# zkonduit/ezkl

Hardware: NVIDIA H100
Metric: prove_time_s (lower is better)
Workload: dtype u32 limbs (254-bit Montgomery integers mod BN254 r/p)

## Files before the change

### ezkl_b200/csrc/debug.cu

```cuda
#include "debug.h"
#include "ec_coop.cuh"
#include "msm.cuh"
#include "ntt.cuh"

namespace b200 {
template <class Tag>
HD Fp<Tag> dbg_field(int op, const Fp<Tag>& x, const Fp<Tag>& y) {
    switch (op) {
        case 0: return x + y;
        case 1: return x - y;
        case 2: return x * y;
        case 3: return fp_inv(x);
        case 4: return fp_from_mont(x);
        case 5: return fp_sqr(x);
        case 6: return fp_neg(x);
        case 7: return fp_dbl(x);
        default: return fp_to_mont(x);
    }
}
template <class Tag>
HD Fp<Tag> dbg_field4(int op, const Fp<Tag>& a, const Fp<Tag>& b, const Fp<Tag>& c, const Fp<Tag>& d) {
    return op == 0 ? fp_muladd2(a, b, c, d) : fp_mulsub2(a, b, c, d);
}
HD G1Affine dbg_g1(int op, const G1Affine& p, const G1Affine& q) {
    G1Xyzz r;
    if (op == 0) r = g1_add_mixed(g1_to_xyzz(p), q);
    else if (op == 1) r = g1_dbl(g1_to_xyzz(p));
    else if (op == 2) r = g1_mul_small(g1_to_xyzz(p), q.x.l[0]);
    else if (op == 3) r = g1_add(g1_to_xyzz(p), g1_dbl_affine(q));
    else r = g1_add_mixed(g1_to_xyzz(p), g1_neg(p));
    return g1_to_affine(r);
}
enum { DBG_XYZZ_COOP = 5 };
HD G1Xyzz dbg_xyzz(int op, const G1Xyzz& a, const G1Xyzz& b, uint32_t k) {
    switch (op) {
        case 0: return g1_add(a, b);
        case 1: return g1_dbl(a);
        case 2: { G1Affine q; q.x = b.x; q.y = b.y; return g1_add_mixed(a, q); }
        case 3: return g1_mul_small(a, k);
        default: {
            const G1Affine q = g1_to_affine(a);
            G1Xyzz r = g1_xyzz_identity(); r.x = q.x; r.y = q.y;
            return r;
        }
    }
}

template <class Tag>
__global__ void k_dbg_field(int op, const Fp<Tag>* a, const Fp<Tag>* b, Fp<Tag>* o, size_t n) {
    size_t i = (size_t)blockIdx.x * blockDim.x + threadIdx.x;
    if (i < n) fp_store(o + i, dbg_field(op, fp_load(a + i), fp_load(b + i)));
}
template <class Tag>
__global__ void k_dbg_field4(int op, const Fp<Tag>* a, const Fp<Tag>* b, const Fp<Tag>* c, const Fp<Tag>* d, Fp<Tag>* o, size_t n) {
    size_t i = (size_t)blockIdx.x * blockDim.x + threadIdx.x;
    if (i < n) fp_store(o + i, dbg_field4(op, fp_load(a + i), fp_load(b + i), fp_load(c + i), fp_load(d + i)));
}
__global__ void k_dbg_g1(int op, const G1Affine* a, const G1Affine* b, G1Affine* o, size_t n) {
    size_t i = (size_t)blockIdx.x * blockDim.x + threadIdx.x;
    if (i < n) o[i] = dbg_g1(op, a[i], b[i]);
}
__global__ void k_dbg_xyzz(int op, const G1Xyzz* a, const G1Xyzz* b, const uint32_t* k, G1Xyzz* o, size_t n) {
    const size_t t = (size_t)blockIdx.x * blockDim.x + threadIdx.x;
    if (op >= DBG_XYZZ_COOP) {
        const size_t i = t >> 2;
        if (i >= n) return;
        const G1Xyzz r = op == DBG_XYZZ_COOP ? g1_add_coop4(a[i], b[i]) : g1_dbl_coop4(a[i]);
        if ((t & 3) == 0) o[i] = r;
        return;
    }
    if (t < n) o[t] = dbg_xyzz(op, a[t], b[t], k[t]);
}
__global__ void k_dbg_xyzz_to_affine(const G1Xyzz* p, G1Affine* o, size_t n) {
    size_t i = (size_t)blockIdx.x * blockDim.x + threadIdx.x;
    if (i < n) o[i] = g1_to_affine(p[i]);
}
template <class Tag> static void host_field_op(int op, const b200_fr* a, const b200_fr* b, b200_fr* out, size_t n) {
    for (size_t i = 0; i < n; ++i) {
        Fp<Tag> x, y; memcpy(&x, &a[i], 32); memcpy(&y, &b[i], 32);
        const Fp<Tag> r = dbg_field(op, x, y); memcpy(&out[i], &r, 32);
    }
}
template <class Tag> static void host_field_op4(int op, const b200_fr* a, const b200_fr* b, const b200_fr* c, const b200_fr* d, b200_fr* out, size_t n) {
    for (size_t i = 0; i < n; ++i) {
        Fp<Tag> w, x, y, z; memcpy(&w, &a[i], 32); memcpy(&x, &b[i], 32); memcpy(&y, &c[i], 32); memcpy(&z, &d[i], 32);
        const Fp<Tag> r = dbg_field4(op, w, x, y, z); memcpy(&out[i], &r, 32);
    }
}
struct DbgStage {
    DevBuf bufs[6];
    int used = 0;
    template <class T> int in(const void* src, size_t bytes, T** d) {
        DevBuf& b = bufs[used++];
        if (b.ensure(bytes ? bytes : 1)) return -2;
        B200_CUDA(cudaMemcpy(b.p, src, bytes, cudaMemcpyHostToDevice));
        *d = b.as<T>();
        return 0;
    }
    template <class T> int out(size_t bytes, T** d) {
        DevBuf& b = bufs[used++];
        if (b.ensure(bytes ? bytes : 1)) return -2;
        *d = b.as<T>();
        return 0;
    }
    ~DbgStage() { for (DevBuf& b : bufs) b.release(); }
};
static Config g_dbg_cfg;
const Config& config() { return g_dbg_cfg; }
int sm_count() {
    int dev = 0, v = 0;
    if (cudaGetDevice(&dev) != cudaSuccess || cudaDeviceGetAttribute(&v, cudaDevAttrMultiProcessorCount, dev) != cudaSuccess || v <= 0) return 132;
    return v;
}
bool prof_enabled() { return false; }
void prof_mark(int, cudaStream_t, bool) {}
__global__ void k_dbg_digits(const Fr* s, int c, int W, int32_t* out, size_t n) {
    size_t i = (size_t)blockIdx.x * blockDim.x + threadIdx.x;
    if (i >= n) return;
    Fr v = fp_from_mont(fp_load(s + i));
    uint32_t carry = 0;
    for (int w = 0; w < W; ++w) out[i * W + w] = msm_next_digit(v.l, c, &carry);
}
template <int VARIANT>
__global__ void __launch_bounds__(256) k_bench_mul(Fq* out, int iters) {
    const uint32_t t = blockIdx.x * blockDim.x + threadIdx.x;
    Fq x = fp_one<FqTag>(), y = fp_one<FqTag>();
    x.l[0] ^= t; y.l[1] ^= (t * 2654435761u);
    if (VARIANT == 0) {
#pragma unroll 1
        for (int i = 0; i < iters; ++i) x = x * y;
    } else if (VARIANT == 1) {
        Fq z = y + y;
#pragma unroll 1
        for (int i = 0; i < iters; i += 2) { x = x * y; z = z * y; }
        x = x + z;
    } else if (VARIANT == 2) {
#pragma unroll 1
        for (int i = 0; i < iters; ++i) { Fq r; fp_mul_portable<FqTag>(r.l, x.l, y.l); x = r; }
    } else if (VARIANT == 3) {
        G1Affine g; g.x = x; g.y = y;
        G1Xyzz acc = g1_dbl_affine(g);
#pragma unroll 1
        for (int i = 0; i < iters; ++i) { acc = g1_add_mixed(acc, g); g.x.l[0] += 1; }
        x = acc.x + acc.y + acc.zz + acc.zzz;
    } else {
#pragma unroll 1
        for (int i = 0; i < iters; ++i) { x = x + y; y = y - x; }
    }
    fp_store(out + t, x);
}
template <int V>
__global__ void __launch_bounds__(256) k_bench_pipe(uint64_t* out, int iters) {
    const uint32_t t = blockIdx.x * blockDim.x + threadIdx.x;
    uint32_t a = t * 2654435761u + 12345u, b = t ^ 0x9e3779b9u;
    if (V == 0) {
        uint64_t c0 = t, c1 = t + 1, c2 = t + 2, c3 = t + 3, c4 = t + 4, c5 = t + 5, c6 = t + 6, c7 = t + 7;
#pragma unroll 1
        for (int i = 0; i < iters; ++i) {
            asm volatile("mad.wide.u32 %0, %8, %9, %0;\n\tmad.wide.u32 %1, %8, %9, %1;\n\tmad.wide.u32 %2, %8, %9, %2;\n\tmad.wide.u32 %3, %8, %9, %3;\n\t"
                         "mad.wide.u32 %4, %8, %9, %4;\n\tmad.wide.u32 %5, %8, %9, %5;\n\tmad.wide.u32 %6, %8, %9, %6;\n\tmad.wide.u32 %7, %8, %9, %7;"
                         : "+l"(c0), "+l"(c1), "+l"(c2), "+l"(c3), "+l"(c4), "+l"(c5), "+l"(c6), "+l"(c7) : "r"(a), "r"(b));
        }
        out[t] = c0 ^ c1 ^ c2 ^ c3 ^ c4 ^ c5 ^ c6 ^ c7;
    } else if (V == 1) {
        uint32_t e0 = t, e1 = 1, e2 = 2, e3 = 3, e4 = 4, e5 = 5, e6 = 6, e7 = 7, o0 = 8, o1 = 9, o2 = 10, o3 = 11, o4 = 12, o5 = 13, o6 = 14, o7 = 15;
#pragma unroll 1
        for (int i = 0; i < iters; ++i) {
            asm volatile("mad.lo.cc.u32 %0, %16, %17, %0;\n\tmadc.hi.cc.u32 %1, %16, %17, %1;\n\tmadc.lo.cc.u32 %2, %16, %17, %2;\n\tmadc.hi.cc.u32 %3, %16, %17, %3;\n\t"
                         "madc.lo.cc.u32 %4, %16, %17, %4;\n\tmadc.hi.cc.u32 %5, %16, %17, %5;\n\tmadc.lo.cc.u32 %6, %16, %17, %6;\n\tmadc.hi.u32 %7, %16, %17, %7;\n\t"
                         "mad.lo.cc.u32 %8, %16, %17, %8;\n\tmadc.hi.cc.u32 %9, %16, %17, %9;\n\tmadc.lo.cc.u32 %10, %16, %17, %10;\n\tmadc.hi.cc.u32 %11, %16, %17, %11;\n\t"
                         "madc.lo.cc.u32 %12, %16, %17, %12;\n\tmadc.hi.cc.u32 %13, %16, %17, %13;\n\tmadc.lo.cc.u32 %14, %16, %17, %14;\n\tmadc.hi.u32 %15, %16, %17, %15;"
                         : "+r"(e0), "+r"(e1), "+r"(e2), "+r"(e3), "+r"(e4), "+r"(e5), "+r"(e6), "+r"(e7), "+r"(o0), "+r"(o1), "+r"(o2), "+r"(o3), "+r"(o4), "+r"(o5), "+r"(o6), "+r"(o7)
                         : "r"(a), "r"(b));
        }
        out[t] = (uint64_t)(e0 ^ e1 ^ e2 ^ e3 ^ e4 ^ e5 ^ e6 ^ e7) << 32 | (o0 ^ o1 ^ o2 ^ o3 ^ o4 ^ o5 ^ o6 ^ o7);
    } else if (V == 2) {
        uint32_t c0 = t, c1 = 1, c2 = 2, c3 = 3, c4 = 4, c5 = 5, c6 = 6, c7 = 7;
#pragma unroll 1
        for (int i = 0; i < iters; ++i) {
            asm volatile("mad.lo.u32 %0, %8, %9, %0;\n\tmad.lo.u32 %1, %8, %9, %1;\n\tmad.lo.u32 %2, %8, %9, %2;\n\tmad.lo.u32 %3, %8, %9, %3;\n\t"
                         "mad.lo.u32 %4, %8, %9, %4;\n\tmad.lo.u32 %5, %8, %9, %5;\n\tmad.lo.u32 %6, %8, %9, %6;\n\tmad.lo.u32 %7, %8, %9, %7;"
                         : "+r"(c0), "+r"(c1), "+r"(c2), "+r"(c3), "+r"(c4), "+r"(c5), "+r"(c6), "+r"(c7) : "r"(a), "r"(b));
        }
        out[t] = c0 ^ c1 ^ c2 ^ c3 ^ c4 ^ c5 ^ c6 ^ c7;
    } else {
        double x = (double)a, y = 1.0 + 1e-9 * (double)(b & 1023), c0 = t, c1 = 1, c2 = 2, c3 = 3, c4 = 4, c5 = 5, c6 = 6, c7 = 7;
#pragma unroll 1
        for (int i = 0; i < iters; ++i) {
            c0 = fma(x, y, c0); c1 = fma(x, y, c1); c2 = fma(x, y, c2); c3 = fma(x, y, c3); c4 = fma(x, y, c4); c5 = fma(x, y, c5); c6 = fma(x, y, c6); c7 = fma(x, y, c7);
        }
        out[t] = (uint64_t)(c0 + c1 + c2 + c3 + c4 + c5 + c6 + c7);
    }
}
}
using namespace b200;

#pragma GCC visibility push(default)
extern "C" {
int b200_debug_field_op(int field, int op, const b200_fr* a, const b200_fr* b, b200_fr* out, size_t n) {
    if (n == 0) return 0;
    DbgStage st;
    Fr *da, *db, *dout;
    if (int rc = st.in(a, 32 * n, &da)) return rc;
    if (int rc = st.in(b, 32 * n, &db)) return rc;
    if (int rc = st.out(32 * n, &dout)) return rc;
    if (field == 0) k_dbg_field<FrTag><<<div_up(n, 128), 128>>>(op, da, db, dout, n);
    else k_dbg_field<FqTag><<<div_up(n, 128), 128>>>(op, (const Fq*)da, (const Fq*)db, (Fq*)dout, n);
    B200_CUDA(cudaGetLastError());
    B200_CUDA(cudaMemcpy(out, dout, 32 * n, cudaMemcpyDeviceToHost));
    return 0;
}
int b200_debug_field_op4(int field, int op, const b200_fr* a, const b200_fr* b, const b200_fr* c, const b200_fr* d, b200_fr* out, size_t n) {
    if (n == 0) return 0;
    DbgStage st;
    Fr *da, *db, *dc, *dd, *dout;
    if (int rc = st.in(a, 32 * n, &da)) return rc;
    if (int rc = st.in(b, 32 * n, &db)) return rc;
    if (int rc = st.in(c, 32 * n, &dc)) return rc;
    if (int rc = st.in(d, 32 * n, &dd)) return rc;
    if (int rc = st.out(32 * n, &dout)) return rc;
    if (field == 0) k_dbg_field4<FrTag><<<div_up(n, 128), 128>>>(op, da, db, dc, dd, dout, n);
    else k_dbg_field4<FqTag><<<div_up(n, 128), 128>>>(op, (const Fq*)da, (const Fq*)db, (const Fq*)dc, (const Fq*)dd, (Fq*)dout, n);
    B200_CUDA(cudaGetLastError());
    B200_CUDA(cudaMemcpy(out, dout, 32 * n, cudaMemcpyDeviceToHost));
    return 0;
}
int b200_debug_g1_op(int op, const b200_g1_affine* a, const b200_g1_affine* b, b200_g1_affine* out, size_t n) {
    if (n == 0) return 0;
    DbgStage st;
    G1Affine *da, *db, *dout;
    if (int rc = st.in(a, 64 * n, &da)) return rc;
    if (int rc = st.in(b, 64 * n, &db)) return rc;
    if (int rc = st.out(64 * n, &dout)) return rc;
    k_dbg_g1<<<div_up(n, 64), 64>>>(op, da, db, dout, n);
    B200_CUDA(cudaGetLastError());
    B200_CUDA(cudaMemcpy(out, dout, 64 * n, cudaMemcpyDeviceToHost));
    return 0;
}
int b200_debug_g1_xyzz_op(int op, const b200_g1_xyzz* a, const b200_g1_xyzz* b, const uint32_t* k, b200_g1_xyzz* out, size_t n) {
    if (op < 0 || op > DBG_XYZZ_COOP + 1) return -1;
    if (n == 0) return 0;
    DbgStage st;
    G1Xyzz *da, *db, *dout;
    uint32_t* dk;
    if (int rc = st.in(a, 128 * n, &da)) return rc;
    if (int rc = st.in(b, 128 * n, &db)) return rc;
    if (int rc = st.in(k, 4 * n, &dk)) return rc;
    if (int rc = st.out(128 * n, &dout)) return rc;
    const size_t threads = op >= DBG_XYZZ_COOP ? 4 * n : n;
    k_dbg_xyzz<<<div_up(threads, 64), 64>>>(op, da, db, dk, dout, n);
    B200_CUDA(cudaGetLastError());
    B200_CUDA(cudaMemcpy(out, dout, 128 * n, cudaMemcpyDeviceToHost));
    return 0;
}
int b200_debug_digits(const b200_fr* s, size_t n, int c, int32_t* out ) {
    const int W = (255 + c - 1) / c;
    void *ds, *dout;
    B200_CUDA(cudaMalloc(&ds, 32 * n)); B200_CUDA(cudaMalloc(&dout, 4 * n * W));
    B200_CUDA(cudaMemcpy(ds, s, 32 * n, cudaMemcpyHostToDevice));
    k_dbg_digits<<<div_up(n, 128), 128>>>((const Fr*)ds, c, W, (int32_t*)dout, n);
    B200_CUDA(cudaGetLastError());
    B200_CUDA(cudaMemcpy(out, dout, 4 * n * W, cudaMemcpyDeviceToHost));
    cudaFree(ds); cudaFree(dout);
    return 0;
}
int b200_debug_bench(int variant, int iters, int blocks, int threads, float* ms) {
    Fq* d; B200_CUDA(cudaMalloc(&d, sizeof(Fq) * (size_t)blocks * threads));
    cudaEvent_t e0, e1; cudaEventCreate(&e0); cudaEventCreate(&e1);
    for (int rep = 0; rep < 2; ++rep) {
        cudaEventRecord(e0);
        switch (variant) {
            case 0: k_bench_mul<0><<<blocks, threads>>>(d, iters); break;
            case 1: k_bench_mul<1><<<blocks, threads>>>(d, iters); break;
            case 2: k_bench_mul<2><<<blocks, threads>>>(d, iters); break;
            case 3: k_bench_mul<3><<<blocks, threads>>>(d, iters); break;
            default: k_bench_mul<4><<<blocks, threads>>>(d, iters); break;
        }
        cudaEventRecord(e1);
        B200_CUDA(cudaEventSynchronize(e1));
    }
    B200_CUDA(cudaEventElapsedTime(ms, e0, e1));
    cudaFree(d); cudaEventDestroy(e0); cudaEventDestroy(e1);
    return 0;
}
int b200_debug_bench_pipe(int variant, int iters, int blocks, int threads, float* ms) {
    uint64_t* d; B200_CUDA(cudaMalloc(&d, 8 * (size_t)blocks * threads));
    cudaEvent_t e0, e1; cudaEventCreate(&e0); cudaEventCreate(&e1);
    for (int rep = 0; rep < 2; ++rep) {
        cudaEventRecord(e0);
        switch (variant) {
            case 0: k_bench_pipe<0><<<blocks, threads>>>(d, iters); break;
            case 1: k_bench_pipe<1><<<blocks, threads>>>(d, iters); break;
            case 2: k_bench_pipe<2><<<blocks, threads>>>(d, iters); break;
            default: k_bench_pipe<3><<<blocks, threads>>>(d, iters); break;
        }
        cudaEventRecord(e1);
        B200_CUDA(cudaEventSynchronize(e1));
    }
    B200_CUDA(cudaEventElapsedTime(ms, e0, e1));
    cudaFree(d); cudaEventDestroy(e0); cudaEventDestroy(e1);
    return 0;
}
int b200_debug_digits_host(const b200_fr* s_canonical, size_t n, int c, int32_t* out) {
    const int W = (255 + c - 1) / c;
    for (size_t i = 0; i < n; ++i) {
        uint32_t v[8]; memcpy(v, &s_canonical[i], 32);
        uint32_t carry = 0;
        for (int w = 0; w < W; ++w) out[i * W + w] = msm_next_digit(v, c, &carry);
    }
    return 0;
}
int b200_debug_digit_slots_host(const b200_fr* s_canonical, size_t n, int c, int wpl, int32_t* out) {
    const int W = (255 + c - 1) / c;
    for (size_t i = 0; i < n; ++i) {
        uint32_t v[8]; memcpy(v, &s_canonical[i], 32);
        uint32_t carry = 0;
        MsmWindowSlot slot;
        for (int w = 0; w < W; ++w) {
            const int32_t d = msm_next_digit(v, c, &carry);
            int32_t* o = out + ((size_t)i * W + w) * 4;
            o[0] = (int32_t)slot.level; o[1] = slot.r;
            o[2] = d ? (int32_t)(slot.set_off + (uint32_t)(d < 0 ? -d : d) - 1u) : -1;
            o[3] = d < 0 ? -1 : (d > 0 ? 1 : 0);
            slot.next(c, wpl);
        }
    }
    return 0;
}
int b200_debug_msm_pick_levels(size_t n, int c, size_t max_table_bytes, int* s, int* L) {
    msm_pick_levels(n, c, max_table_bytes, s, L);
    return 0;
}
int b200_debug_msm_recode_plan(size_t n, int batch, uint32_t nbuckets, int W, int sm_count, uint32_t* out ) {
    const MsmRecodePlan p = msm_pick_recode(n, batch, nbuckets, W, sm_count);
    out[0] = p.tile; out[1] = p.tiles;
    return 0;
}
int b200_debug_msm_base_off(const b200_fr* scalars, size_t n, int batch, const b200_g1_affine* bases, size_t table_n, int c,
                            size_t max_table_bytes, size_t base_off, b200_g1_affine* out) {
    if (n == 0 || batch < 1 || batch > 4096 || base_off + n > table_n || c < 4 || c > 22) return -1;
    MsmTable t;
    MsmWorkspace ws;
    void *d_sc = nullptr, *d_xyzz = nullptr, *d_aff = nullptr;
    auto run = [&]() -> int {
        if (int rc = msm_table_alloc(&t, table_n, c, max_table_bytes ? max_table_bytes : ~(size_t)0)) return rc;
        B200_CUDA(cudaMemcpy(t.d_table, bases, sizeof(G1Affine) * table_n, cudaMemcpyHostToDevice));
        if (int rc = msm_table_build(&t, nullptr, 0)) return rc;
        B200_CUDA(cudaMalloc(&d_sc, sizeof(Fr) * n * batch));
        B200_CUDA(cudaMalloc(&d_xyzz, sizeof(G1Xyzz) * batch));
        B200_CUDA(cudaMalloc(&d_aff, sizeof(G1Affine) * batch));
        B200_CUDA(cudaMemcpy(d_sc, scalars, sizeof(Fr) * n * batch, cudaMemcpyHostToDevice));
        if (int rc = msm_run(t, (const Fr*)d_sc, n, n, batch, (G1Xyzz*)d_xyzz, ws, 0, base_off)) return rc;
        k_dbg_xyzz_to_affine<<<div_up(batch, 32), 32>>>((const G1Xyzz*)d_xyzz, (G1Affine*)d_aff, (size_t)batch);
        B200_CUDA(cudaGetLastError());
        B200_CUDA(cudaMemcpy(out, d_aff, sizeof(G1Affine) * batch, cudaMemcpyDeviceToHost));
        return 0;
    };
    const int rc = run();
    DevBuf* bufs[] = {&ws.counts, &ws.offs, &ws.ents, &ws.subs, &ws.sums, &ws.misc, &ws.tile_counts};
    for (DevBuf* b : bufs) b->release();
    msm_table_free(&t);
    if (d_sc) cudaFree(d_sc);
    if (d_xyzz) cudaFree(d_xyzz);
    if (d_aff) cudaFree(d_aff);
    return rc;
}
int b200_debug_ntt_plan_host(uint32_t log_n, int batch, int sm_count, int64_t* out ) {
    if (log_n < 1 || log_n > 28 || batch < 1 || batch > 65535 || sm_count < 1) return -1;
    int npass, logm[3];
    ntt_choose_passes(log_n, &npass, logm);
    for (int i = 0; i < npass; ++i) {
        const NttPassShape sh = ntt_pass_shape(npass, logm, i);
        const NttPassGeom g = ntt_pass_geometry((uint32_t)logm[i], sh.inner_cnt, sh.lines, batch, sm_count);
        int64_t* o = out + 7 * i;
        o[0] = g.kernel; o[1] = logm[i]; o[2] = g.log_g; o[3] = g.threads; o[4] = (int64_t)g.smem; o[5] = (int64_t)g.grid_x;
        o[6] = i == npass - 1 ? 0 : (g.kernel == 2 && ntt_full_table(log_n, npass) ? 1 : 2);
    }
    return npass;
}
int b200_debug_host_g1_op(int op, const b200_g1_affine* a, const b200_g1_affine* b, b200_g1_affine* out, size_t n) {
    for (size_t i = 0; i < n; ++i) {
        G1Affine p, q; memcpy(&p, &a[i], 64); memcpy(&q, &b[i], 64);
        const G1Affine o = dbg_g1(op, p, q); memcpy(&out[i], &o, 64);
    }
    return 0;
}
int b200_debug_host_g1_xyzz_op(int op, const b200_g1_xyzz* a, const b200_g1_xyzz* b, const uint32_t* k, b200_g1_xyzz* out, size_t n) {
    if (op < 0 || op >= DBG_XYZZ_COOP) return -1;
    for (size_t i = 0; i < n; ++i) {
        G1Xyzz p, q; memcpy(&p, &a[i], 128); memcpy(&q, &b[i], 128);
        const G1Xyzz o = dbg_xyzz(op, p, q, k[i]); memcpy(&out[i], &o, 128);
    }
    return 0;
}
int b200_debug_host_field_op(int field, int op, const b200_fr* a, const b200_fr* b, b200_fr* out, size_t n) {
    if (field == 0) host_field_op<FrTag>(op, a, b, out, n); else host_field_op<FqTag>(op, a, b, out, n);
    return 0;
}
int b200_debug_host_field_op4(int field, int op, const b200_fr* a, const b200_fr* b, const b200_fr* c, const b200_fr* d, b200_fr* out, size_t n) {
    if (field == 0) host_field_op4<FrTag>(op, a, b, c, d, out, n); else host_field_op4<FqTag>(op, a, b, c, d, out, n);
    return 0;
}
}
#pragma GCC visibility pop
```

### ezkl_b200/csrc/ec.cuh

```cuda
#pragma once
#include "field.cuh"

namespace b200 {

struct alignas(16) G1Affine { Fq x, y; };
struct alignas(16) G1Xyzz { Fq x, y, zz, zzz; };
struct alignas(16) G1Jac { Fq x, y, z; };

HD bool g1_is_identity(const G1Affine& p) { return fp_is_zero(p.x) && fp_is_zero(p.y); }
HD bool g1_is_identity(const G1Xyzz& p) { return fp_is_zero(p.zz); }
HD G1Xyzz g1_xyzz_identity() {
    G1Xyzz r; r.x = fp_zero<FqTag>(); r.y = fp_zero<FqTag>(); r.zz = fp_zero<FqTag>(); r.zzz = fp_zero<FqTag>();
    return r;
}
HD G1Xyzz g1_to_xyzz(const G1Affine& p) {
    G1Xyzz r;
    if (g1_is_identity(p)) return g1_xyzz_identity();
    r.x = p.x; r.y = p.y; r.zz = fp_one<FqTag>(); r.zzz = fp_one<FqTag>();
    return r;
}
HD G1Affine g1_neg(const G1Affine& p) {
    G1Affine r; r.x = p.x; r.y = fp_neg(p.y);
    return r;
}
HD G1Xyzz g1_dbl_affine(const G1Affine& p) {
    if (g1_is_identity(p)) return g1_xyzz_identity();
    G1Xyzz r;
    Fq u = fp_dbl(p.y), v = fp_sqr(u), w = u * v, s = p.x * v;
    Fq xx = fp_sqr(p.x), m = fp_dbl(xx) + xx;
    r.x = fp_sqr(m) - fp_dbl(s);
    r.y = fp_mulsub2(m, s - r.x, w, p.y);
    r.zz = v; r.zzz = w;
    return r;
}
HD G1Xyzz g1_dbl(const G1Xyzz& p) {
    if (g1_is_identity(p)) return p;
    G1Xyzz r;
    Fq u = fp_dbl(p.y), v = fp_sqr(u), w = u * v, s = p.x * v;
    Fq xx = fp_sqr(p.x), m = fp_dbl(xx) + xx;
    r.x = fp_sqr(m) - fp_dbl(s);
    r.y = fp_mulsub2(m, s - r.x, w, p.y);
    r.zz = v * p.zz; r.zzz = w * p.zzz;
    return r;
}
HD G1Xyzz g1_add_mixed(const G1Xyzz& a, const G1Affine& q) {
    if (g1_is_identity(q)) return a;
    if (g1_is_identity(a)) return g1_to_xyzz(q);
    Fq u2 = q.x * a.zz, s2 = q.y * a.zzz;
    Fq p = u2 - a.x, r = s2 - a.y;
    if (fp_is_zero(p)) {
        if (fp_is_zero(r)) return g1_dbl_affine(q);
        return g1_xyzz_identity();
    }
    G1Xyzz o;
    Fq pp = fp_sqr(p), ppp = p * pp, qq = a.x * pp;
    o.x = fp_sqr(r) - ppp - fp_dbl(qq);
    o.y = fp_mulsub2(r, qq - o.x, a.y, ppp);
    o.zz = a.zz * pp; o.zzz = a.zzz * ppp;
    return o;
}
HD G1Xyzz g1_add(const G1Xyzz& a, const G1Xyzz& b) {
    if (g1_is_identity(a)) return b;
    if (g1_is_identity(b)) return a;
    Fq u1 = a.x * b.zz, u2 = b.x * a.zz, s1 = a.y * b.zzz, s2 = b.y * a.zzz;
    Fq p = u2 - u1, r = s2 - s1;
    if (fp_is_zero(p)) {
        if (fp_is_zero(r)) return g1_dbl(a);
        return g1_xyzz_identity();
    }
    G1Xyzz o;
    Fq pp = fp_sqr(p), ppp = p * pp, qq = u1 * pp;
    o.x = fp_sqr(r) - ppp - fp_dbl(qq);
    o.y = fp_mulsub2(r, qq - o.x, s1, ppp);
    o.zz = a.zz * b.zz * pp; o.zzz = a.zzz * b.zzz * ppp;
    return o;
}
HD G1Affine g1_to_affine(const G1Xyzz& p) {
    G1Affine r;
    if (g1_is_identity(p)) { r.x = fp_zero<FqTag>(); r.y = fp_zero<FqTag>(); return r; }
    Fq zzz_inv = fp_inv(p.zzz);
    Fq zinv = p.zz * zzz_inv;
    Fq zinv2 = fp_sqr(zinv);
    r.x = p.x * zinv2;
    r.y = p.y * (zinv2 * zinv);
    return r;
}
HD G1Jac g1_affine_to_jac(const G1Affine& p) {
    G1Jac r;
    if (g1_is_identity(p)) { r.x = fp_zero<FqTag>(); r.y = fp_one<FqTag>(); r.z = fp_zero<FqTag>(); return r; }
    r.x = p.x; r.y = p.y; r.z = fp_one<FqTag>();
    return r;
}
HD bool g1_is_on_curve(const G1Affine& p) {
    if (g1_is_identity(p)) return true;
    Fq one = fp_one<FqTag>();
    Fq three = one + one + one;
    return fp_eq(fp_sqr(p.y), fp_sqr(p.x) * p.x + three);
}
HD G1Xyzz g1_mul_small(const G1Xyzz& p, uint32_t k) {
    if (k == 0) return g1_xyzz_identity();
    const G1Xyzz p2 = g1_dbl(p), p3 = g1_add(p2, p);
    int top = 30;
    while (top > 0 && !((k >> top) & 3u)) top -= 2;
    uint32_t d = (k >> top) & 3u;
    G1Xyzz acc = d == 1 ? p : (d == 2 ? p2 : p3);
#pragma unroll 1
    for (int i = top - 2; i >= 0; i -= 2) {
        acc = g1_dbl(g1_dbl(acc));
        d = (k >> i) & 3u;
        if (d) acc = g1_add(acc, d == 1 ? p : (d == 2 ? p2 : p3));
    }
    return acc;
}

}
```

### ezkl_b200/csrc/field.cuh

```cuda
#pragma once
#include <stdint.h>
#include "fp_ptx.cuh"

#if defined(__CUDACC__)
#define HD __host__ __device__ __forceinline__
#define DEV __device__ __forceinline__
#else
#define HD inline
#define DEV inline
#endif

namespace b200 {

struct FrTag {
    static constexpr uint32_t INV = 0xefffffffu;
    HD static uint32_t mod(int i) {
        constexpr uint32_t M[8] = {0xf0000001u, 0x43e1f593u, 0x79b97091u, 0x2833e848u, 0x8181585du, 0xb85045b6u, 0xe131a029u, 0x30644e72u};
        return M[i];
    }
    HD static uint32_t one(int i) {
        constexpr uint32_t V[8] = {0x4ffffffbu, 0xac96341cu, 0x9f60cd29u, 0x36fc7695u, 0x7879462eu, 0x666ea36fu, 0x9a07df2fu, 0x0e0a77c1u};
        return V[i];
    }
    HD static uint32_t r2(int i) {
        constexpr uint32_t V[8] = {0xae216da7u, 0x1bb8e645u, 0xe35c59e3u, 0x53fe3ab1u, 0x53bb8085u, 0x8c49833du, 0x7f4e44a5u, 0x0216d0b1u};
        return V[i];
    }
};
struct FqTag {
    static constexpr uint32_t INV = 0xe4866389u;
    HD static uint32_t mod(int i) {
        constexpr uint32_t M[8] = {0xd87cfd47u, 0x3c208c16u, 0x6871ca8du, 0x97816a91u, 0x8181585du, 0xb85045b6u, 0xe131a029u, 0x30644e72u};
        return M[i];
    }
    HD static uint32_t one(int i) {
        constexpr uint32_t V[8] = {0xc58f0d9du, 0xd35d438du, 0xf5c70b3du, 0x0a78eb28u, 0x7879462cu, 0x666ea36fu, 0x9a07df2fu, 0x0e0a77c1u};
        return V[i];
    }
    HD static uint32_t r2(int i) {
        constexpr uint32_t V[8] = {0x538afa89u, 0xf32cfc5bu, 0xd44501fbu, 0xb5e71911u, 0x0a417ff6u, 0x47ab1effu, 0xcab8351fu, 0x06d89f71u};
        return V[i];
    }
};

template <class Tag>
struct alignas(16) Fp {
    uint32_t l[8];
};
using Fr = Fp<FrTag>;
using Fq = Fp<FqTag>;

template <class Tag>
HD void fp_mul_portable(uint32_t* r, const uint32_t* a, const uint32_t* b) {
    uint32_t t[10];
#pragma unroll
    for (int i = 0; i < 10; ++i) t[i] = 0;
#pragma unroll
    for (int i = 0; i < 8; ++i) {
        uint64_t c = 0, s;
#pragma unroll
        for (int j = 0; j < 8; ++j) { s = (uint64_t)a[j] * b[i] + t[j] + c; t[j] = (uint32_t)s; c = s >> 32; }
        s = (uint64_t)t[8] + c; t[8] = (uint32_t)s; t[9] = (uint32_t)(s >> 32);
        uint32_t m = t[0] * Tag::INV;
        c = ((uint64_t)m * Tag::mod(0) + t[0]) >> 32;
#pragma unroll
        for (int j = 1; j < 8; ++j) { s = (uint64_t)m * Tag::mod(j) + t[j] + c; t[j - 1] = (uint32_t)s; c = s >> 32; }
        s = (uint64_t)t[8] + c; t[7] = (uint32_t)s; t[8] = t[9] + (uint32_t)(s >> 32);
    }
    uint32_t d[8]; uint64_t br = 0;
#pragma unroll
    for (int j = 0; j < 8; ++j) { uint64_t s = (uint64_t)t[j] - Tag::mod(j) - br; d[j] = (uint32_t)s; br = (s >> 32) & 1; }
    bool ge = (t[8] != 0) || (br == 0);
#pragma unroll
    for (int j = 0; j < 8; ++j) r[j] = ge ? d[j] : t[j];
}
template <class Tag>
HD void fp_add_portable(uint32_t* r, const uint32_t* a, const uint32_t* b) {
    uint32_t t[8], d[8]; uint64_t c = 0, br = 0;
#pragma unroll
    for (int j = 0; j < 8; ++j) { uint64_t s = (uint64_t)a[j] + b[j] + c; t[j] = (uint32_t)s; c = s >> 32; }
#pragma unroll
    for (int j = 0; j < 8; ++j) { uint64_t s = (uint64_t)t[j] - Tag::mod(j) - br; d[j] = (uint32_t)s; br = (s >> 32) & 1; }
    bool ge = (br == 0);
#pragma unroll
    for (int j = 0; j < 8; ++j) r[j] = ge ? d[j] : t[j];
}
template <class Tag>
HD void fp_sub_portable(uint32_t* r, const uint32_t* a, const uint32_t* b) {
    uint32_t t[8]; uint64_t br = 0, c = 0;
#pragma unroll
    for (int j = 0; j < 8; ++j) { uint64_t s = (uint64_t)a[j] - b[j] - br; t[j] = (uint32_t)s; br = (s >> 32) & 1; }
    uint32_t mask = br ? 0xffffffffu : 0u;
#pragma unroll
    for (int j = 0; j < 8; ++j) { uint64_t s = (uint64_t)t[j] + (Tag::mod(j) & mask) + c; r[j] = (uint32_t)s; c = s >> 32; }
}

template <class Tag> struct PtxOps;
#if defined(__CUDA_ARCH__)
template <> struct PtxOps<FrTag> {
    DEV static void mul(uint32_t* r, const uint32_t* a, const uint32_t* b) { fr_mul_ptx(r, a, b); }
    DEV static void add(uint32_t* r, const uint32_t* a, const uint32_t* b) { fr_add_ptx(r, a, b); }
    DEV static void sub(uint32_t* r, const uint32_t* a, const uint32_t* b) { fr_sub_ptx(r, a, b); }
    DEV static void mul2(uint32_t* r, const uint32_t* a, const uint32_t* b, const uint32_t* c, const uint32_t* d) { fr_mul2_ptx(r, a, b, c, d); }
    DEV static void sqr(uint32_t* r, const uint32_t* a) { fr_sqr_ptx(r, a); }
};
template <> struct PtxOps<FqTag> {
    DEV static void mul(uint32_t* r, const uint32_t* a, const uint32_t* b) { fq_mul_ptx(r, a, b); }
    DEV static void add(uint32_t* r, const uint32_t* a, const uint32_t* b) { fq_add_ptx(r, a, b); }
    DEV static void sub(uint32_t* r, const uint32_t* a, const uint32_t* b) { fq_sub_ptx(r, a, b); }
    DEV static void mul2(uint32_t* r, const uint32_t* a, const uint32_t* b, const uint32_t* c, const uint32_t* d) { fq_mul2_ptx(r, a, b, c, d); }
    DEV static void sqr(uint32_t* r, const uint32_t* a) { fq_sqr_ptx(r, a); }
};
#endif

template <class Tag> HD Fp<Tag> operator*(const Fp<Tag>& a, const Fp<Tag>& b) {
    Fp<Tag> r;
#if defined(__CUDA_ARCH__)
    PtxOps<Tag>::mul(r.l, a.l, b.l);
#else
    fp_mul_portable<Tag>(r.l, a.l, b.l);
#endif
    return r;
}
template <class Tag> HD Fp<Tag> operator+(const Fp<Tag>& a, const Fp<Tag>& b) {
    Fp<Tag> r;
#if defined(__CUDA_ARCH__)
    PtxOps<Tag>::add(r.l, a.l, b.l);
#else
    fp_add_portable<Tag>(r.l, a.l, b.l);
#endif
    return r;
}
template <class Tag> HD Fp<Tag> operator-(const Fp<Tag>& a, const Fp<Tag>& b) {
    Fp<Tag> r;
#if defined(__CUDA_ARCH__)
    PtxOps<Tag>::sub(r.l, a.l, b.l);
#else
    fp_sub_portable<Tag>(r.l, a.l, b.l);
#endif
    return r;
}
template <class Tag> HD Fp<Tag> fp_sqr(const Fp<Tag>& a) {
#if defined(__CUDA_ARCH__)
    Fp<Tag> r;
    PtxOps<Tag>::sqr(r.l, a.l);
    return r;
#else
    return a * a;
#endif
}
template <class Tag> HD Fp<Tag> fp_dbl(const Fp<Tag>& a) { return a + a; }
template <class Tag> HD Fp<Tag> fp_zero() {
    Fp<Tag> r;
#pragma unroll
    for (int i = 0; i < 8; ++i) r.l[i] = 0;
    return r;
}
template <class Tag> HD Fp<Tag> fp_one() {
    Fp<Tag> r;
#pragma unroll
    for (int i = 0; i < 8; ++i) r.l[i] = Tag::one(i);
    return r;
}
template <class Tag> HD bool fp_is_zero(const Fp<Tag>& a) {
    uint32_t o = 0;
#pragma unroll
    for (int i = 0; i < 8; ++i) o |= a.l[i];
    return o == 0;
}
template <class Tag> HD bool fp_eq(const Fp<Tag>& a, const Fp<Tag>& b) {
    uint32_t o = 0;
#pragma unroll
    for (int i = 0; i < 8; ++i) o |= a.l[i] ^ b.l[i];
    return o == 0;
}
template <class Tag> HD Fp<Tag> fp_neg(const Fp<Tag>& a) { return fp_zero<Tag>() - a; }
template <class Tag> HD Fp<Tag> fp_muladd2(const Fp<Tag>& a, const Fp<Tag>& b, const Fp<Tag>& c, const Fp<Tag>& d) {
#if defined(__CUDA_ARCH__)
    Fp<Tag> r;
    PtxOps<Tag>::mul2(r.l, a.l, b.l, c.l, d.l);
    return r;
#else
    return a * b + c * d;
#endif
}
template <class Tag> HD Fp<Tag> fp_mulsub2(const Fp<Tag>& a, const Fp<Tag>& b, const Fp<Tag>& c, const Fp<Tag>& d) {
#if defined(__CUDA_ARCH__)
    return fp_muladd2(a, b, fp_neg(c), d);
#else
    return a * b - c * d;
#endif
}
template <class Tag> HD Fp<Tag> fp_from_mont(const Fp<Tag>& a) {
    Fp<Tag> one_c = fp_zero<Tag>(); one_c.l[0] = 1;
    return a * one_c;
}
template <class Tag> HD Fp<Tag> fp_to_mont(const Fp<Tag>& a) {
    Fp<Tag> r2;
#pragma unroll
    for (int i = 0; i < 8; ++i) r2.l[i] = Tag::r2(i);
    return a * r2;
}
template <class Tag> HD Fp<Tag> fp_inv(const Fp<Tag>& a) {
    uint32_t e[8];
    {
        uint64_t br = 2;
        for (int i = 0; i < 8; ++i) { uint64_t s = (uint64_t)Tag::mod(i) - br; e[i] = (uint32_t)s; br = (s >> 32) & 1; }
    }
    Fp<Tag> acc = fp_one<Tag>();
#pragma unroll 1
    for (int i = 253; i >= 0; --i) {
        acc = acc * acc;
        if ((e[i >> 5] >> (i & 31)) & 1) acc = acc * a;
    }
    return acc;
}
template <class Tag> HD Fp<Tag> fp_pow_u64(const Fp<Tag>& a, uint64_t e) {
    Fp<Tag> acc = fp_one<Tag>();
#pragma unroll 1
    for (int i = 63; i >= 0; --i) {
        acc = acc * acc;
        if ((e >> i) & 1) acc = acc * a;
    }
    return acc;
}

#if defined(__CUDACC__)
template <class Tag> DEV Fp<Tag> fp_load(const Fp<Tag>* p) {
    Fp<Tag> r;
    const uint4* q = reinterpret_cast<const uint4*>(p);
    uint4 lo = q[0], hi = q[1];
    r.l[0] = lo.x; r.l[1] = lo.y; r.l[2] = lo.z; r.l[3] = lo.w;
    r.l[4] = hi.x; r.l[5] = hi.y; r.l[6] = hi.z; r.l[7] = hi.w;
    return r;
}
template <class Tag> DEV void fp_store(Fp<Tag>* p, const Fp<Tag>& v) {
    uint4* q = reinterpret_cast<uint4*>(p);
    q[0] = make_uint4(v.l[0], v.l[1], v.l[2], v.l[3]);
    q[1] = make_uint4(v.l[4], v.l[5], v.l[6], v.l[7]);
}
#endif

}
```

### ezkl_b200/csrc/fp_gen.py

```python
#!/usr/bin/env python
import random
import sys

M32 = 0xFFFFFFFF
FIELDS = {
    "fr": 0x30644e72e131a029b85045b68181585d2833e84879b9709143e1f593f0000001,
    "fq": 0x30644e72e131a029b85045b68181585d97816a916871ca8d3c208c16d87cfd47,
}


def limbs(x, n=8):
    return [(x >> (32 * i)) & M32 for i in range(n)]


def gen_mul(mod):
    Ml = limbs(mod)
    inv = (-pow(mod, -1, 1 << 32)) & M32
    ins = []
    X = ["x%d" % i for i in range(8)]
    Y = ["y%d" % i for i in range(8)]
    A = ["a%d" % i for i in range(8)]
    B = ["b%d" % i for i in range(8)]

    def imm(v):
        return "0x%08x" % v

    def reduce_row(E, O):
        ins.append(("mul.lo.u32", "m", E[0], imm(inv)))
        for j in range(4):
            ins.append((("mad.lo.cc.u32" if j == 0 else "madc.lo.cc.u32"), O[2 * j], "m", imm(Ml[2 * j + 1]), O[2 * j]))
            ins.append(("madc.hi.cc.u32", O[2 * j + 1], "m", imm(Ml[2 * j + 1]), O[2 * j + 1]))
        for j in range(4):
            ins.append((("mad.lo.cc.u32" if j == 0 else "madc.lo.cc.u32"), E[2 * j], "m", imm(Ml[2 * j]), E[2 * j]))
            ins.append(("madc.hi.cc.u32", E[2 * j + 1], "m", imm(Ml[2 * j]), E[2 * j + 1]))
        ins.append(("addc.u32", O[7], O[7], "0"))

    for j in range(4):
        ins.append(("mul.lo.u32", X[2 * j], A[2 * j], B[0]))
        ins.append(("mul.hi.u32", X[2 * j + 1], A[2 * j], B[0]))
    for j in range(4):
        ins.append(("mul.lo.u32", Y[2 * j], A[2 * j + 1], B[0]))
        ins.append(("mul.hi.u32", Y[2 * j + 1], A[2 * j + 1], B[0]))
    E, O = X, Y
    reduce_row(E, O)
    for i in range(1, 8):
        nE, nO = O, E
        ins.append(("add.cc.u32", nE[0], nE[0], nO[1]))
        for j in range(4):
            c_lo = nO[2 * j + 2] if 2 * j + 2 < 8 else "0"
            c_hi = nO[2 * j + 3] if 2 * j + 3 < 8 else "0"
            ins.append(("madc.lo.cc.u32", nO[2 * j], A[2 * j + 1], B[i], c_lo))
            ins.append(("madc.hi.cc.u32", nO[2 * j + 1], A[2 * j + 1], B[i], c_hi))
        for j in range(4):
            ins.append((("mad.lo.cc.u32" if j == 0 else "madc.lo.cc.u32"), nE[2 * j], A[2 * j], B[i], nE[2 * j]))
            ins.append(("madc.hi.cc.u32", nE[2 * j + 1], A[2 * j], B[i], nE[2 * j + 1]))
        ins.append(("addc.u32", nO[7], nO[7], "0"))
        E, O = nE, nO
        reduce_row(E, O)
    T = ["t%d" % i for i in range(8)]
    for j in range(7):
        ins.append((("add.cc.u32" if j == 0 else "addc.cc.u32"), T[j], O[j], E[j + 1]))
    ins.append(("addc.u32", T[7], O[7], "0"))
    ins += final_sub(T, Ml)
    return ins


def gen_mul2(mod):
    Ml = limbs(mod)
    inv = (-pow(mod, -1, 1 << 32)) & M32
    ins = []
    X = ["x%d" % i for i in range(8)]
    Y = ["y%d" % i for i in range(8)]
    A = ["a%d" % i for i in range(8)]
    B = ["b%d" % i for i in range(8)]
    Cc = ["c%d" % i for i in range(8)]
    D = ["d%d" % i for i in range(8)]

    def imm(v):
        return "0x%08x" % v

    def acc_rows(E, O, P, q):
        def pair(p):
            return (q, p) if p.startswith("0x") else (p, q)
        for j in range(4):
            ins.append((("mad.lo.cc.u32" if j == 0 else "madc.lo.cc.u32"), O[2 * j]) + pair(P[2 * j + 1]) + (O[2 * j],))
            ins.append(("madc.hi.cc.u32", O[2 * j + 1]) + pair(P[2 * j + 1]) + (O[2 * j + 1],))
        for j in range(4):
            ins.append((("mad.lo.cc.u32" if j == 0 else "madc.lo.cc.u32"), E[2 * j]) + pair(P[2 * j]) + (E[2 * j],))
            ins.append(("madc.hi.cc.u32", E[2 * j + 1]) + pair(P[2 * j]) + (E[2 * j + 1],))
        ins.append(("addc.u32", O[7], O[7], "0"))

    def reduce_row(E, O):
        ins.append(("mul.lo.u32", "m", E[0], imm(inv)))
        acc_rows(E, O, [imm(v) for v in Ml], "m")

    for j in range(4):
        ins.append(("mul.lo.u32", X[2 * j], A[2 * j], B[0]))
        ins.append(("mul.hi.u32", X[2 * j + 1], A[2 * j], B[0]))
    for j in range(4):
        ins.append(("mul.lo.u32", Y[2 * j], A[2 * j + 1], B[0]))
        ins.append(("mul.hi.u32", Y[2 * j + 1], A[2 * j + 1], B[0]))
    E, O = X, Y
    acc_rows(E, O, Cc, D[0])
    reduce_row(E, O)
    for i in range(1, 8):
        nE, nO = O, E
        ins.append(("add.cc.u32", nE[0], nE[0], nO[1]))
        for j in range(4):
            c_lo = nO[2 * j + 2] if 2 * j + 2 < 8 else "0"
            c_hi = nO[2 * j + 3] if 2 * j + 3 < 8 else "0"
            ins.append(("madc.lo.cc.u32", nO[2 * j], A[2 * j + 1], B[i], c_lo))
            ins.append(("madc.hi.cc.u32", nO[2 * j + 1], A[2 * j + 1], B[i], c_hi))
        for j in range(4):
            ins.append((("mad.lo.cc.u32" if j == 0 else "madc.lo.cc.u32"), nE[2 * j], A[2 * j], B[i], nE[2 * j]))
            ins.append(("madc.hi.cc.u32", nE[2 * j + 1], A[2 * j], B[i], nE[2 * j + 1]))
        ins.append(("addc.u32", nO[7], nO[7], "0"))
        E, O = nE, nO
        acc_rows(E, O, Cc, D[i])
        reduce_row(E, O)
    T = ["t%d" % i for i in range(8)]
    for j in range(7):
        ins.append((("add.cc.u32" if j == 0 else "addc.cc.u32"), T[j], O[j], E[j + 1]))
    ins.append(("addc.u32", T[7], O[7], "0"))
    ins += final_sub(T, Ml)
    return ins


def gen_sqr(mod):
    Ml = limbs(mod)
    inv = (-pow(mod, -1, 1 << 32)) & M32
    ins = []
    X = ["x%d" % i for i in range(8)]
    Y = ["y%d" % i for i in range(8)]
    A = ["a%d" % i for i in range(8)]
    U = ["u%d" % i for i in range(8)]
    Wl = ["w%d" % i for i in range(8)]

    def imm(v):
        return "0x%08x" % v

    for j in range(1, 8):
        ins.append(("shl.b32", Wl[j], A[j], "1"))
    for j in range(2, 8):
        ins.append(("shf.l.clamp.b32", U[j], A[j - 1], A[j], "1"))

    def operand(i, j):
        return A[j] if j == i else (Wl[j] if j == i + 1 else U[j])

    def reduce_row(E, O):
        ins.append(("mul.lo.u32", "m", E[0], imm(inv)))
        for j in range(4):
            ins.append((("mad.lo.cc.u32" if j == 0 else "madc.lo.cc.u32"), O[2 * j], "m", imm(Ml[2 * j + 1]), O[2 * j]))
            ins.append(("madc.hi.cc.u32", O[2 * j + 1], "m", imm(Ml[2 * j + 1]), O[2 * j + 1]))
        for j in range(4):
            ins.append((("mad.lo.cc.u32" if j == 0 else "madc.lo.cc.u32"), E[2 * j], "m", imm(Ml[2 * j]), E[2 * j]))
            ins.append(("madc.hi.cc.u32", E[2 * j + 1], "m", imm(Ml[2 * j]), E[2 * j + 1]))
        ins.append(("addc.u32", O[7], O[7], "0"))

    for j in range(4):
        ins.append(("mul.lo.u32", X[2 * j], operand(0, 2 * j), A[0]))
        ins.append(("mul.hi.u32", X[2 * j + 1], operand(0, 2 * j), A[0]))
    for j in range(4):
        ins.append(("mul.lo.u32", Y[2 * j], operand(0, 2 * j + 1), A[0]))
        ins.append(("mul.hi.u32", Y[2 * j + 1], operand(0, 2 * j + 1), A[0]))
    E, O = X, Y
    reduce_row(E, O)
    for i in range(1, 8):
        nE, nO = O, E
        ins.append(("add.cc.u32", nE[0], nE[0], nO[1]))
        for j in range(4):
            c_lo = nO[2 * j + 2] if 2 * j + 2 < 8 else "0"
            c_hi = nO[2 * j + 3] if 2 * j + 3 < 8 else "0"
            if 2 * j + 1 >= i:
                ins.append(("madc.lo.cc.u32", nO[2 * j], operand(i, 2 * j + 1), A[i], c_lo))
                ins.append(("madc.hi.cc.u32", nO[2 * j + 1], operand(i, 2 * j + 1), A[i], c_hi))
            else:
                ins.append(("addc.cc.u32", nO[2 * j], c_lo, "0"))
                ins.append(("addc.cc.u32", nO[2 * j + 1], c_hi, "0"))
        first = True
        for j in range(4):
            if 2 * j < i:
                continue
            ins.append((("mad.lo.cc.u32" if first else "madc.lo.cc.u32"), nE[2 * j], operand(i, 2 * j), A[i], nE[2 * j]))
            ins.append(("madc.hi.cc.u32", nE[2 * j + 1], operand(i, 2 * j), A[i], nE[2 * j + 1]))
            first = False
        if not first:
            ins.append(("addc.u32", nO[7], nO[7], "0"))
        E, O = nE, nO
        reduce_row(E, O)
    T = ["t%d" % i for i in range(8)]
    for j in range(7):
        ins.append((("add.cc.u32" if j == 0 else "addc.cc.u32"), T[j], O[j], E[j + 1]))
    ins.append(("addc.u32", T[7], O[7], "0"))
    ins += final_sub(T, Ml)
    return ins


def final_sub(T, Ml, out=None):
    out = out or ["r%d" % i for i in range(8)]
    ins = []
    S = ["s%d" % i for i in range(8)]
    for j in range(8):
        ins.append((("sub.cc.u32" if j == 0 else "subc.cc.u32"), S[j], T[j], "0x%08x" % Ml[j]))
    ins.append(("subc.u32", "brw", "0", "0"))
    ins.append(("setp.eq.u32", "p", "brw", "0"))
    for j in range(8):
        ins.append(("selp.u32", out[j], S[j], T[j], "p"))
    return ins


def gen_add(mod):
    Ml = limbs(mod)
    ins = []
    T = ["t%d" % i for i in range(8)]
    for j in range(8):
        op = "add.cc.u32" if j == 0 else ("addc.cc.u32" if j < 7 else "addc.u32")
        ins.append((op, T[j], "a%d" % j, "b%d" % j))
    return ins + final_sub(T, Ml)


def gen_sub(mod):
    Ml = limbs(mod)
    ins = []
    T = ["t%d" % i for i in range(8)]
    for j in range(8):
        ins.append((("sub.cc.u32" if j == 0 else "subc.cc.u32"), T[j], "a%d" % j, "b%d" % j))
    ins.append(("subc.u32", "brw", "0", "0"))
    for j in range(8):
        ins.append(("and.b32", "s%d" % j, "brw", "0x%08x" % Ml[j]))
    for j in range(8):
        op = "add.cc.u32" if j == 0 else ("addc.cc.u32" if j < 7 else "addc.u32")
        ins.append((op, "r%d" % j, T[j], "s%d" % j))
    return ins


def run(ins, regs):
    cc = 0
    pred = {}

    def val(x):
        if x in regs:
            return regs[x]
        return int(x, 0)

    for it in ins:
        op, d = it[0], it[1]
        s = [val(x) if x not in pred else x for x in it[2:]]
        if op == "mul.lo.u32":
            regs[d] = (s[0] * s[1]) & M32
        elif op == "mul.hi.u32":
            regs[d] = (s[0] * s[1]) >> 32
        elif op in ("mad.lo.cc.u32", "madc.lo.cc.u32", "madc.hi.cc.u32", "mad.hi.cc.u32"):
            p = s[0] * s[1]
            p = (p & M32) if ".lo" in op else (p >> 32)
            t = p + s[2] + (cc if op.startswith("madc") else 0)
            regs[d], cc = t & M32, t >> 32
        elif op in ("add.cc.u32", "addc.cc.u32", "addc.u32"):
            t = s[0] + s[1] + (cc if op.startswith("addc") else 0)
            regs[d] = t & M32
            if ".cc" in op:
                cc = t >> 32
        elif op in ("sub.cc.u32", "subc.cc.u32", "subc.u32"):
            t = s[0] - s[1] - (cc if op.startswith("subc") else 0)
            regs[d] = t & M32
            if ".cc" in op:
                cc = 1 if t < 0 else 0
        elif op == "and.b32":
            regs[d] = s[0] & s[1]
        elif op == "shl.b32":
            regs[d] = (s[0] << s[1]) & M32
        elif op == "shf.l.clamp.b32":
            regs[d] = ((((s[1] << 32) | s[0]) << min(s[2], 32)) >> 32) & M32
        elif op == "setp.eq.u32":
            pred[d] = (s[0] == s[1])
        elif op == "selp.u32":
            regs[d] = s[0] if pred[it[4]] else s[1]
        else:
            raise ValueError(op)
        assert 0 <= regs.get(d, 0) <= M32
    return regs


def check(name, mod, trials=3000):
    rng = random.Random(hash(name) & 0xFFFF)
    mul, add, sub = gen_mul(mod), gen_add(mod), gen_sub(mod)
    Rinv = pow(1 << 256, -1, mod)
    edge = [0, 1, 2, mod - 1, mod - 2, (1 << 254) % mod, (1 << 253), mod >> 1, 0xFFFFFFFF, (1 << 128) - 1]
    pairs = [(x, y) for x in edge for y in edge] + [(rng.randrange(mod), rng.randrange(mod)) for _ in range(trials)]
    for a, b in pairs:
        regs = {}
        for i, v in enumerate(limbs(a)):
            regs["a%d" % i] = v
        for i, v in enumerate(limbs(b)):
            regs["b%d" % i] = v
        for ins, exp in ((mul, a * b * Rinv % mod), (add, (a + b) % mod), (sub, (a - b) % mod)):
            out = run(ins, dict(regs))
            got = sum(out["r%d" % i] << (32 * i) for i in range(8))
            assert got == exp, (name, hex(a), hex(b), hex(got), hex(exp))
    mul2 = gen_mul2(mod)
    edge2 = [0, 1, mod - 1, mod, (1 << 254) % mod, 0xFFFFFFFF, mod >> 1]
    quads = [(a, b, c, d) for a in edge2 for b in edge2 for c in edge2 for d in edge2]
    quads += [tuple(rng.randrange(mod) for _ in range(4)) for _ in range(trials)]
    for a, b, c, d in quads:
        regs = {}
        for nm, v in (("a", a), ("b", b), ("c", c), ("d", d)):
            for i, w in enumerate(limbs(v)):
                regs["%s%d" % (nm, i)] = w
        out = run(mul2, regs)
        got = sum(out["r%d" % i] << (32 * i) for i in range(8))
        exp = (a * b + c * d) * Rinv % mod
        assert got == exp, (name, "mul2", hex(a), hex(b), hex(c), hex(d), hex(got), hex(exp))
    sqr = gen_sqr(mod)
    for a in edge + [mod, (1 << 254) - 1 if (1 << 254) - 1 < mod else mod - 3, 0x80000000, 0xFFFFFFFF << 32, int("80000000" * 8, 16) % mod,
                     int("ffffffff" * 7, 16)] + [rng.randrange(mod) for _ in range(trials)]:
        regs = {"a%d" % i: v for i, v in enumerate(limbs(a))}
        out = run(sqr, regs)
        got = sum(out["r%d" % i] << (32 * i) for i in range(8))
        assert got == a * a * Rinv % mod, (name, "sqr", hex(a), hex(got))
    return len(mul), len(add), len(sub), len(mul2), len(sqr)


def emit_fn(fname, ins, n_in):
    tmp = sorted({x for it in ins for x in it[1:] if x[0] in "xytsmuw" and not x.startswith("0x")} | {"brw"})
    tmp = [t for t in tmp if t != "p"]
    lines = ["    .reg .u32 %s;" % ", ".join(tmp), "    .reg .pred p;"]

    def opnd(x):
        if x[0] == "r" and x[1:].isdigit():
            return "%%%d" % int(x[1:])
        if x[0] == "a" and x[1:].isdigit():
            return "%%%d" % (8 + int(x[1:]))
        if x[0] == "b" and x[1:].isdigit() and x != "brw":
            return "%%%d" % (16 + int(x[1:]))
        if x[0] == "c" and x[1:].isdigit():
            return "%%%d" % (24 + int(x[1:]))
        if x[0] == "d" and x[1:].isdigit():
            return "%%%d" % (32 + int(x[1:]))
        return x

    for it in ins:
        lines.append("    %s %s;" % (it[0], ", ".join(opnd(x) for x in it[1:])))
    body = "\n".join('        "%s\\n\\t"' % ln.strip() for ln in ["{"] + lines + ["}"])
    outs = ", ".join('"=r"(r[%d])' % i for i in range(8))
    inps = ", ".join('"r"(a[%d])' % i for i in range(8))
    args = "uint32_t* r, const uint32_t* a"
    if n_in >= 2:
        inps += ", " + ", ".join('"r"(b[%d])' % i for i in range(8))
        args += ", const uint32_t* b"
    if n_in == 4:
        inps += ", " + ", ".join('"r"(c[%d])' % i for i in range(8)) + ", " + ", ".join('"r"(d[%d])' % i for i in range(8))
        args += ", const uint32_t* c, const uint32_t* d"
    return ("__device__ __forceinline__ void %s(%s) {\n    asm(\n%s\n        : %s\n        : %s);\n}\n"
            % (fname, args, body, outs, inps))


def main():
    out = ["// GENERATED by fp_gen.py -- do not edit.  Every instruction list below was executed by the generator's",
           "// PTX interpreter against Python bigints (edge + random operands) before this file was written.",
           "#pragma once", "#include <stdint.h>", "#if defined(__CUDA_ARCH__)", ""]
    for name, mod in FIELDS.items():
        n = check(name, mod)
        print("%s: verified; instruction counts mul/add/sub/mul2/sqr = %s" % (name, n))
        out.append(emit_fn("%s_mul_ptx" % name, gen_mul(mod), 2))
        out.append(emit_fn("%s_add_ptx" % name, gen_add(mod), 2))
        out.append(emit_fn("%s_sub_ptx" % name, gen_sub(mod), 2))
        out.append(emit_fn("%s_mul2_ptx" % name, gen_mul2(mod), 4))
        out.append(emit_fn("%s_sqr_ptx" % name, gen_sqr(mod), 1))
    out.append("#endif  // __CUDA_ARCH__")
    if "--check" not in sys.argv:
        import os
        with open(os.path.join(os.path.dirname(os.path.abspath(__file__)), "fp_ptx.cuh"), "w") as f:
            f.write("\n".join(out) + "\n")


if __name__ == "__main__":
    main()
```

### ezkl_b200/csrc/fp_ptx.cuh

```cuda
#pragma once
#include <stdint.h>
#if defined(__CUDA_ARCH__)

__device__ __forceinline__ void fr_mul_ptx(uint32_t* r, const uint32_t* a, const uint32_t* b) {
    asm(
        "{\n\t"
        ".reg .u32 brw, m, s0, s1, s2, s3, s4, s5, s6, s7, t0, t1, t2, t3, t4, t5, t6, t7, x0, x1, x2, x3, x4, x5, x6, x7, y0, y1, y2, y3, y4, y5, y6, y7;\n\t"
        ".reg .pred p;\n\t"
        "mul.lo.u32 x0, %8, %16;\n\t"
        "mul.hi.u32 x1, %8, %16;\n\t"
        "mul.lo.u32 x2, %10, %16;\n\t"
        "mul.hi.u32 x3, %10, %16;\n\t"
        "mul.lo.u32 x4, %12, %16;\n\t"
        "mul.hi.u32 x5, %12, %16;\n\t"
        "mul.lo.u32 x6, %14, %16;\n\t"
        "mul.hi.u32 x7, %14, %16;\n\t"
        "mul.lo.u32 y0, %9, %16;\n\t"
        "mul.hi.u32 y1, %9, %16;\n\t"
        "mul.lo.u32 y2, %11, %16;\n\t"
        "mul.hi.u32 y3, %11, %16;\n\t"
        "mul.lo.u32 y4, %13, %16;\n\t"
        "mul.hi.u32 y5, %13, %16;\n\t"
        "mul.lo.u32 y6, %15, %16;\n\t"
        "mul.hi.u32 y7, %15, %16;\n\t"
// ... 1982 lines not shown

__device__ __forceinline__ void fq_sqr_ptx(uint32_t* r, const uint32_t* a) {
    asm(
        "{\n\t"
        ".reg .u32 brw, m, s0, s1, s2, s3, s4, s5, s6, s7, t0, t1, t2, t3, t4, t5, t6, t7, u2, u3, u4, u5, u6, u7, w1, w2, w3, w4, w5, w6, w7, x0, x1, x2, x3, x4, x5, x6, x7, y0, y1, y2, y3, y4, y5, y6, y7;\n\t"
        ".reg .pred p;\n\t"
        "shl.b32 w1, %9, 1;\n\t"
        "shl.b32 w2, %10, 1;\n\t"
        "shl.b32 w3, %11, 1;\n\t"
        "shl.b32 w4, %12, 1;\n\t"
        "shl.b32 w5, %13, 1;\n\t"
        "shl.b32 w6, %14, 1;\n\t"
        "shl.b32 w7, %15, 1;\n\t"
        "shf.l.clamp.b32 u2, %9, %10, 1;\n\t"
        "shf.l.clamp.b32 u3, %10, %11, 1;\n\t"
        "shf.l.clamp.b32 u4, %11, %12, 1;\n\t"
        "shf.l.clamp.b32 u5, %12, %13, 1;\n\t"
        "shf.l.clamp.b32 u6, %13, %14, 1;\n\t"
        "shf.l.clamp.b32 u7, %14, %15, 1;\n\t"
        "mul.lo.u32 x0, %8, %8;\n\t"
        "mul.hi.u32 x1, %8, %8;\n\t"
        "mul.lo.u32 x2, u2, %8;\n\t"
        "mul.hi.u32 x3, u2, %8;\n\t"
        "mul.lo.u32 x4, u4, %8;\n\t"
        "mul.hi.u32 x5, u4, %8;\n\t"
        "mul.lo.u32 x6, u6, %8;\n\t"
        "mul.hi.u32 x7, u6, %8;\n\t"
        "mul.lo.u32 y0, w1, %8;\n\t"
        "mul.hi.u32 y1, w1, %8;\n\t"
        "mul.lo.u32 y2, u3, %8;\n\t"
        "mul.hi.u32 y3, u3, %8;\n\t"
        "mul.lo.u32 y4, u5, %8;\n\t"
        "mul.hi.u32 y5, u5, %8;\n\t"
        "mul.lo.u32 y6, u7, %8;\n\t"
        "mul.hi.u32 y7, u7, %8;\n\t"
        "mul.lo.u32 m, x0, 0xe4866389;\n\t"
        "mad.lo.cc.u32 y0, m, 0x3c208c16, y0;\n\t"
        "madc.hi.cc.u32 y1, m, 0x3c208c16, y1;\n\t"
        "madc.lo.cc.u32 y2, m, 0x97816a91, y2;\n\t"
        "madc.hi.cc.u32 y3, m, 0x97816a91, y3;\n\t"
        "madc.lo.cc.u32 y4, m, 0xb85045b6, y4;\n\t"
        "madc.hi.cc.u32 y5, m, 0xb85045b6, y5;\n\t"
        "madc.lo.cc.u32 y6, m, 0x30644e72, y6;\n\t"
        "madc.hi.cc.u32 y7, m, 0x30644e72, y7;\n\t"
        "mad.lo.cc.u32 x0, m, 0xd87cfd47, x0;\n\t"
        "madc.hi.cc.u32 x1, m, 0xd87cfd47, x1;\n\t"
        "madc.lo.cc.u32 x2, m, 0x6871ca8d, x2;\n\t"
        "madc.hi.cc.u32 x3, m, 0x6871ca8d, x3;\n\t"
        "madc.lo.cc.u32 x4, m, 0x8181585d, x4;\n\t"
        "madc.hi.cc.u32 x5, m, 0x8181585d, x5;\n\t"
        "madc.lo.cc.u32 x6, m, 0xe131a029, x6;\n\t"
        "madc.hi.cc.u32 x7, m, 0xe131a029, x7;\n\t"
        "addc.u32 y7, y7, 0;\n\t"
        "add.cc.u32 y0, y0, x1;\n\t"
        "madc.lo.cc.u32 x0, %9, %9, x2;\n\t"
        "madc.hi.cc.u32 x1, %9, %9, x3;\n\t"
        "madc.lo.cc.u32 x2, u3, %9, x4;\n\t"
        "madc.hi.cc.u32 x3, u3, %9, x5;\n\t"
        "madc.lo.cc.u32 x4, u5, %9, x6;\n\t"
        "madc.hi.cc.u32 x5, u5, %9, x7;\n\t"
        "madc.lo.cc.u32 x6, u7, %9, 0;\n\t"
        "madc.hi.cc.u32 x7, u7, %9, 0;\n\t"
        "mad.lo.cc.u32 y2, w2, %9, y2;\n\t"
        "madc.hi.cc.u32 y3, w2, %9, y3;\n\t"
        "madc.lo.cc.u32 y4, u4, %9, y4;\n\t"
        "madc.hi.cc.u32 y5, u4, %9, y5;\n\t"
        "madc.lo.cc.u32 y6, u6, %9, y6;\n\t"
        "madc.hi.cc.u32 y7, u6, %9, y7;\n\t"
        "addc.u32 x7, x7, 0;\n\t"
        "mul.lo.u32 m, y0, 0xe4866389;\n\t"
        "mad.lo.cc.u32 x0, m, 0x3c208c16, x0;\n\t"
        "madc.hi.cc.u32 x1, m, 0x3c208c16, x1;\n\t"
        "madc.lo.cc.u32 x2, m, 0x97816a91, x2;\n\t"
        "madc.hi.cc.u32 x3, m, 0x97816a91, x3;\n\t"
        "madc.lo.cc.u32 x4, m, 0xb85045b6, x4;\n\t"
        "madc.hi.cc.u32 x5, m, 0xb85045b6, x5;\n\t"
        "madc.lo.cc.u32 x6, m, 0x30644e72, x6;\n\t"
        "madc.hi.cc.u32 x7, m, 0x30644e72, x7;\n\t"
        "mad.lo.cc.u32 y0, m, 0xd87cfd47, y0;\n\t"
        "madc.hi.cc.u32 y1, m, 0xd87cfd47, y1;\n\t"
        "madc.lo.cc.u32 y2, m, 0x6871ca8d, y2;\n\t"
        "madc.hi.cc.u32 y3, m, 0x6871ca8d, y3;\n\t"
        "madc.lo.cc.u32 y4, m, 0x8181585d, y4;\n\t"
        "madc.hi.cc.u32 y5, m, 0x8181585d, y5;\n\t"
        "madc.lo.cc.u32 y6, m, 0xe131a029, y6;\n\t"
        "madc.hi.cc.u32 y7, m, 0xe131a029, y7;\n\t"
        "addc.u32 x7, x7, 0;\n\t"
        "add.cc.u32 x0, x0, y1;\n\t"
        "addc.cc.u32 y0, y2, 0;\n\t"
        "addc.cc.u32 y1, y3, 0;\n\t"
        "madc.lo.cc.u32 y2, w3, %10, y4;\n\t"
        "madc.hi.cc.u32 y3, w3, %10, y5;\n\t"
        "madc.lo.cc.u32 y4, u5, %10, y6;\n\t"
        "madc.hi.cc.u32 y5, u5, %10, y7;\n\t"
        "madc.lo.cc.u32 y6, u7, %10, 0;\n\t"
        "madc.hi.cc.u32 y7, u7, %10, 0;\n\t"
        "mad.lo.cc.u32 x2, %10, %10, x2;\n\t"
        "madc.hi.cc.u32 x3, %10, %10, x3;\n\t"
        "madc.lo.cc.u32 x4, u4, %10, x4;\n\t"
        "madc.hi.cc.u32 x5, u4, %10, x5;\n\t"
        "madc.lo.cc.u32 x6, u6, %10, x6;\n\t"
        "madc.hi.cc.u32 x7, u6, %10, x7;\n\t"
        "addc.u32 y7, y7, 0;\n\t"
        "mul.lo.u32 m, x0, 0xe4866389;\n\t"
        "mad.lo.cc.u32 y0, m, 0x3c208c16, y0;\n\t"
        "madc.hi.cc.u32 y1, m, 0x3c208c16, y1;\n\t"
        "madc.lo.cc.u32 y2, m, 0x97816a91, y2;\n\t"
        "madc.hi.cc.u32 y3, m, 0x97816a91, y3;\n\t"
        "madc.lo.cc.u32 y4, m, 0xb85045b6, y4;\n\t"
        "madc.hi.cc.u32 y5, m, 0xb85045b6, y5;\n\t"
        "madc.lo.cc.u32 y6, m, 0x30644e72, y6;\n\t"
        "madc.hi.cc.u32 y7, m, 0x30644e72, y7;\n\t"
        "mad.lo.cc.u32 x0, m, 0xd87cfd47, x0;\n\t"
        "madc.hi.cc.u32 x1, m, 0xd87cfd47, x1;\n\t"
        "madc.lo.cc.u32 x2, m, 0x6871ca8d, x2;\n\t"
        "madc.hi.cc.u32 x3, m, 0x6871ca8d, x3;\n\t"
        "madc.lo.cc.u32 x4, m, 0x8181585d, x4;\n\t"
        "madc.hi.cc.u32 x5, m, 0x8181585d, x5;\n\t"
        "madc.lo.cc.u32 x6, m, 0xe131a029, x6;\n\t"
        "madc.hi.cc.u32 x7, m, 0xe131a029, x7;\n\t"
        "addc.u32 y7, y7, 0;\n\t"
        "add.cc.u32 y0, y0, x1;\n\t"
        "addc.cc.u32 x0, x2, 0;\n\t"
        "addc.cc.u32 x1, x3, 0;\n\t"
        "madc.lo.cc.u32 x2, %11, %11, x4;\n\t"
        "madc.hi.cc.u32 x3, %11, %11, x5;\n\t"
        "madc.lo.cc.u32 x4, u5, %11, x6;\n\t"
        "madc.hi.cc.u32 x5, u5, %11, x7;\n\t"
        "madc.lo.cc.u32 x6, u7, %11, 0;\n\t"
        "madc.hi.cc.u32 x7, u7, %11, 0;\n\t"
        "mad.lo.cc.u32 y4, w4, %11, y4;\n\t"
        "madc.hi.cc.u32 y5, w4, %11, y5;\n\t"
        "madc.lo.cc.u32 y6, u6, %11, y6;\n\t"
        "madc.hi.cc.u32 y7, u6, %11, y7;\n\t"
        "addc.u32 x7, x7, 0;\n\t"
        "mul.lo.u32 m, y0, 0xe4866389;\n\t"
        "mad.lo.cc.u32 x0, m, 0x3c208c16, x0;\n\t"
        "madc.hi.cc.u32 x1, m, 0x3c208c16, x1;\n\t"
        "madc.lo.cc.u32 x2, m, 0x97816a91, x2;\n\t"
        "madc.hi.cc.u32 x3, m, 0x97816a91, x3;\n\t"
        "madc.lo.cc.u32 x4, m, 0xb85045b6, x4;\n\t"
        "madc.hi.cc.u32 x5, m, 0xb85045b6, x5;\n\t"
        "madc.lo.cc.u32 x6, m, 0x30644e72, x6;\n\t"
        "madc.hi.cc.u32 x7, m, 0x30644e72, x7;\n\t"
        "mad.lo.cc.u32 y0, m, 0xd87cfd47, y0;\n\t"
        "madc.hi.cc.u32 y1, m, 0xd87cfd47, y1;\n\t"
        "madc.lo.cc.u32 y2, m, 0x6871ca8d, y2;\n\t"
        "madc.hi.cc.u32 y3, m, 0x6871ca8d, y3;\n\t"
        "madc.lo.cc.u32 y4, m, 0x8181585d, y4;\n\t"
        "madc.hi.cc.u32 y5, m, 0x8181585d, y5;\n\t"
        "madc.lo.cc.u32 y6, m, 0xe131a029, y6;\n\t"
        "madc.hi.cc.u32 y7, m, 0xe131a029, y7;\n\t"
        "addc.u32 x7, x7, 0;\n\t"
        "add.cc.u32 x0, x0, y1;\n\t"
        "addc.cc.u32 y0, y2, 0;\n\t"
        "addc.cc.u32 y1, y3, 0;\n\t"
        "addc.cc.u32 y2, y4, 0;\n\t"
        "addc.cc.u32 y3, y5, 0;\n\t"
        "madc.lo.cc.u32 y4, w5, %12, y6;\n\t"
        "madc.hi.cc.u32 y5, w5, %12, y7;\n\t"
        "madc.lo.cc.u32 y6, u7, %12, 0;\n\t"
        "madc.hi.cc.u32 y7, u7, %12, 0;\n\t"
        "mad.lo.cc.u32 x4, %12, %12, x4;\n\t"
        "madc.hi.cc.u32 x5, %12, %12, x5;\n\t"
        "madc.lo.cc.u32 x6, u6, %12, x6;\n\t"
        "madc.hi.cc.u32 x7, u6, %12, x7;\n\t"
        "addc.u32 y7, y7, 0;\n\t"
        "mul.lo.u32 m, x0, 0xe4866389;\n\t"
        "mad.lo.cc.u32 y0, m, 0x3c208c16, y0;\n\t"
        "madc.hi.cc.u32 y1, m, 0x3c208c16, y1;\n\t"
        "madc.lo.cc.u32 y2, m, 0x97816a91, y2;\n\t"
        "madc.hi.cc.u32 y3, m, 0x97816a91, y3;\n\t"
        "madc.lo.cc.u32 y4, m, 0xb85045b6, y4;\n\t"
        "madc.hi.cc.u32 y5, m, 0xb85045b6, y5;\n\t"
        "madc.lo.cc.u32 y6, m, 0x30644e72, y6;\n\t"
        "madc.hi.cc.u32 y7, m, 0x30644e72, y7;\n\t"
        "mad.lo.cc.u32 x0, m, 0xd87cfd47, x0;\n\t"
        "madc.hi.cc.u32 x1, m, 0xd87cfd47, x1;\n\t"
        "madc.lo.cc.u32 x2, m, 0x6871ca8d, x2;\n\t"
        "madc.hi.cc.u32 x3, m, 0x6871ca8d, x3;\n\t"
        "madc.lo.cc.u32 x4, m, 0x8181585d, x4;\n\t"
        "madc.hi.cc.u32 x5, m, 0x8181585d, x5;\n\t"
        "madc.lo.cc.u32 x6, m, 0xe131a029, x6;\n\t"
        "madc.hi.cc.u32 x7, m, 0xe131a029, x7;\n\t"
        "addc.u32 y7, y7, 0;\n\t"
        "add.cc.u32 y0, y0, x1;\n\t"
        "addc.cc.u32 x0, x2, 0;\n\t"
        "addc.cc.u32 x1, x3, 0;\n\t"
        "addc.cc.u32 x2, x4, 0;\n\t"
        "addc.cc.u32 x3, x5, 0;\n\t"
        "madc.lo.cc.u32 x4, %13, %13, x6;\n\t"
        "madc.hi.cc.u32 x5, %13, %13, x7;\n\t"
        "madc.lo.cc.u32 x6, u7, %13, 0;\n\t"
        "madc.hi.cc.u32 x7, u7, %13, 0;\n\t"
        "mad.lo.cc.u32 y6, w6, %13, y6;\n\t"
        "madc.hi.cc.u32 y7, w6, %13, y7;\n\t"
        "addc.u32 x7, x7, 0;\n\t"
        "mul.lo.u32 m, y0, 0xe4866389;\n\t"
        "mad.lo.cc.u32 x0, m, 0x3c208c16, x0;\n\t"
        "madc.hi.cc.u32 x1, m, 0x3c208c16, x1;\n\t"
        "madc.lo.cc.u32 x2, m, 0x97816a91, x2;\n\t"
        "madc.hi.cc.u32 x3, m, 0x97816a91, x3;\n\t"
        "madc.lo.cc.u32 x4, m, 0xb85045b6, x4;\n\t"
        "madc.hi.cc.u32 x5, m, 0xb85045b6, x5;\n\t"
        "madc.lo.cc.u32 x6, m, 0x30644e72, x6;\n\t"
        "madc.hi.cc.u32 x7, m, 0x30644e72, x7;\n\t"
        "mad.lo.cc.u32 y0, m, 0xd87cfd47, y0;\n\t"
        "madc.hi.cc.u32 y1, m, 0xd87cfd47, y1;\n\t"
        "madc.lo.cc.u32 y2, m, 0x6871ca8d, y2;\n\t"
        "madc.hi.cc.u32 y3, m, 0x6871ca8d, y3;\n\t"
        "madc.lo.cc.u32 y4, m, 0x8181585d, y4;\n\t"
        "madc.hi.cc.u32 y5, m, 0x8181585d, y5;\n\t"
        "madc.lo.cc.u32 y6, m, 0xe131a029, y6;\n\t"
        "madc.hi.cc.u32 y7, m, 0xe131a029, y7;\n\t"
        "addc.u32 x7, x7, 0;\n\t"
        "add.cc.u32 x0, x0, y1;\n\t"
        "addc.cc.u32 y0, y2, 0;\n\t"
        "addc.cc.u32 y1, y3, 0;\n\t"
        "addc.cc.u32 y2, y4, 0;\n\t"
        "addc.cc.u32 y3, y5, 0;\n\t"
        "addc.cc.u32 y4, y6, 0;\n\t"
        "addc.cc.u32 y5, y7, 0;\n\t"
        "madc.lo.cc.u32 y6, w7, %14, 0;\n\t"
        "madc.hi.cc.u32 y7, w7, %14, 0;\n\t"
        "mad.lo.cc.u32 x6, %14, %14, x6;\n\t"
        "madc.hi.cc.u32 x7, %14, %14, x7;\n\t"
        "addc.u32 y7, y7, 0;\n\t"
        "mul.lo.u32 m, x0, 0xe4866389;\n\t"
        "mad.lo.cc.u32 y0, m, 0x3c208c16, y0;\n\t"
        "madc.hi.cc.u32 y1, m, 0x3c208c16, y1;\n\t"
        "madc.lo.cc.u32 y2, m, 0x97816a91, y2;\n\t"
        "madc.hi.cc.u32 y3, m, 0x97816a91, y3;\n\t"
        "madc.lo.cc.u32 y4, m, 0xb85045b6, y4;\n\t"
        "madc.hi.cc.u32 y5, m, 0xb85045b6, y5;\n\t"
        "madc.lo.cc.u32 y6, m, 0x30644e72, y6;\n\t"
        "madc.hi.cc.u32 y7, m, 0x30644e72, y7;\n\t"
        "mad.lo.cc.u32 x0, m, 0xd87cfd47, x0;\n\t"
        "madc.hi.cc.u32 x1, m, 0xd87cfd47, x1;\n\t"
        "madc.lo.cc.u32 x2, m, 0x6871ca8d, x2;\n\t"
        "madc.hi.cc.u32 x3, m, 0x6871ca8d, x3;\n\t"
        "madc.lo.cc.u32 x4, m, 0x8181585d, x4;\n\t"
        "madc.hi.cc.u32 x5, m, 0x8181585d, x5;\n\t"
        "madc.lo.cc.u32 x6, m, 0xe131a029, x6;\n\t"
        "madc.hi.cc.u32 x7, m, 0xe131a029, x7;\n\t"
        "addc.u32 y7, y7, 0;\n\t"
        "add.cc.u32 y0, y0, x1;\n\t"
        "addc.cc.u32 x0, x2, 0;\n\t"
        "addc.cc.u32 x1, x3, 0;\n\t"
        "addc.cc.u32 x2, x4, 0;\n\t"
        "addc.cc.u32 x3, x5, 0;\n\t"
        "addc.cc.u32 x4, x6, 0;\n\t"
        "addc.cc.u32 x5, x7, 0;\n\t"
        "madc.lo.cc.u32 x6, %15, %15, 0;\n\t"
        "madc.hi.cc.u32 x7, %15, %15, 0;\n\t"
        "mul.lo.u32 m, y0, 0xe4866389;\n\t"
        "mad.lo.cc.u32 x0, m, 0x3c208c16, x0;\n\t"
        "madc.hi.cc.u32 x1, m, 0x3c208c16, x1;\n\t"
        "madc.lo.cc.u32 x2, m, 0x97816a91, x2;\n\t"
        "madc.hi.cc.u32 x3, m, 0x97816a91, x3;\n\t"
        "madc.lo.cc.u32 x4, m, 0xb85045b6, x4;\n\t"
        "madc.hi.cc.u32 x5, m, 0xb85045b6, x5;\n\t"
        "madc.lo.cc.u32 x6, m, 0x30644e72, x6;\n\t"
        "madc.hi.cc.u32 x7, m, 0x30644e72, x7;\n\t"
        "mad.lo.cc.u32 y0, m, 0xd87cfd47, y0;\n\t"
        "madc.hi.cc.u32 y1, m, 0xd87cfd47, y1;\n\t"
        "madc.lo.cc.u32 y2, m, 0x6871ca8d, y2;\n\t"
        "madc.hi.cc.u32 y3, m, 0x6871ca8d, y3;\n\t"
        "madc.lo.cc.u32 y4, m, 0x8181585d, y4;\n\t"
        "madc.hi.cc.u32 y5, m, 0x8181585d, y5;\n\t"
        "madc.lo.cc.u32 y6, m, 0xe131a029, y6;\n\t"
        "madc.hi.cc.u32 y7, m, 0xe131a029, y7;\n\t"
        "addc.u32 x7, x7, 0;\n\t"
        "add.cc.u32 t0, x0, y1;\n\t"
        "addc.cc.u32 t1, x1, y2;\n\t"
        "addc.cc.u32 t2, x2, y3;\n\t"
        "addc.cc.u32 t3, x3, y4;\n\t"
        "addc.cc.u32 t4, x4, y5;\n\t"
        "addc.cc.u32 t5, x5, y6;\n\t"
        "addc.cc.u32 t6, x6, y7;\n\t"
        "addc.u32 t7, x7, 0;\n\t"
        "sub.cc.u32 s0, t0, 0xd87cfd47;\n\t"
        "subc.cc.u32 s1, t1, 0x3c208c16;\n\t"
        "subc.cc.u32 s2, t2, 0x6871ca8d;\n\t"
        "subc.cc.u32 s3, t3, 0x97816a91;\n\t"
        "subc.cc.u32 s4, t4, 0x8181585d;\n\t"
        "subc.cc.u32 s5, t5, 0xb85045b6;\n\t"
        "subc.cc.u32 s6, t6, 0xe131a029;\n\t"
        "subc.cc.u32 s7, t7, 0x30644e72;\n\t"
        "subc.u32 brw, 0, 0;\n\t"
        "setp.eq.u32 p, brw, 0;\n\t"
        "selp.u32 %0, s0, t0, p;\n\t"
        "selp.u32 %1, s1, t1, p;\n\t"
        "selp.u32 %2, s2, t2, p;\n\t"
        "selp.u32 %3, s3, t3, p;\n\t"
        "selp.u32 %4, s4, t4, p;\n\t"
        "selp.u32 %5, s5, t5, p;\n\t"
        "selp.u32 %6, s6, t6, p;\n\t"
        "selp.u32 %7, s7, t7, p;\n\t"
        "}\n\t"
        : "=r"(r[0]), "=r"(r[1]), "=r"(r[2]), "=r"(r[3]), "=r"(r[4]), "=r"(r[5]), "=r"(r[6]), "=r"(r[7])
        : "r"(a[0]), "r"(a[1]), "r"(a[2]), "r"(a[3]), "r"(a[4]), "r"(a[5]), "r"(a[6]), "r"(a[7]));
}

#endif
```

### ezkl_b200/csrc/msm.cu

```cuda
#include "msm.cuh"
#include "ec_coop.cuh"

namespace b200 {

static constexpr int HEAVY_CHUNKS = 32;
static constexpr int REDUCE_M_MAX = 32;
static constexpr int TREE_THREADS = 256;

int msm_default_window(size_t n) {
    int k = 0;
    while (((size_t)1 << (k + 1)) <= n) ++k;
    int c = k <= 10 ? 8 : (k <= 13 ? k - 2 : (k <= 17 ? k - 1 : (k <= 19 ? 17 : (k <= 21 ? 18 : 20))));
    if (c < 4) c = 4;
    if (c > 22) c = 22;
    return c;
}

__global__ void __launch_bounds__(128) k_table_next_level(const G1Affine* __restrict__ prev, G1Affine* __restrict__ next, size_t n, int c) {
    size_t i = (size_t)blockIdx.x * blockDim.x + threadIdx.x;
    if (i >= n) return;
    G1Affine p = prev[i];
    G1Xyzz a = g1_dbl_affine(p);
#pragma unroll 1
    for (int j = 1; j < c; ++j) a = g1_dbl(a);
    next[i] = g1_to_affine(a);
}

int msm_table_alloc(MsmTable* t, size_t n, int c, size_t max_table_bytes) {
    B200_CHECK(n > 0, -1, "msm_table_build: empty base vector");
    if (c <= 0) c = msm_default_window(n);
    int W = (255 + c - 1) / c, s = 1, L = W;
    msm_pick_levels(n, c, max_table_bytes, &s, &L);
    B200_CHECK((size_t)L * n < ((size_t)1 << 31), -1, "msm_table_build: L*n = %zu exceeds the 31-bit entry index", (size_t)L * n);
    t->n = n; t->c = c; t->W = W; t->s = s; t->L = L;
    B200_CUDA(cudaGetDevice(&t->device));
    const cudaError_t e = cudaMalloc(&t->d_table, t->bytes());
    if (e != cudaSuccess) {
        cudaGetLastError();
        t->d_table = nullptr;
        set_error("msm_table_build: %zu MiB table (%d levels of %zu points): %s", t->bytes() >> 20, L, n, cudaGetErrorString(e));
        return -2;
    }
    return 0;
}

int msm_table_build(MsmTable* t, const G1Affine* d_bases, cudaStream_t st) {
    const size_t n = t->n;
    if (d_bases) B200_CUDA(cudaMemcpyAsync(t->d_table, d_bases, sizeof(G1Affine) * n, cudaMemcpyDeviceToDevice, st));
    for (int j = 1; j < t->L; ++j) {
        k_table_next_level<<<div_up(n, 128), 128, 0, st>>>(t->d_table + (size_t)(j - 1) * n, t->d_table + (size_t)j * n, n, t->c * t->s); count_launch();
    }
    B200_CUDA(cudaGetLastError());
    return 0;
}
void msm_table_free(MsmTable* t) {
    if (t->d_table) cudaFree(t->d_table);
    t->d_table = nullptr;
}

template <bool SCATTER, bool SUBWIN>
__global__ void __launch_bounds__(256) k_digits(const Fr* __restrict__ scalars, size_t stride, uint32_t n, uint32_t table_n, uint32_t base_off, int c, int W,
                                                 uint32_t nbuckets, uint32_t* __restrict__ counters ,
                                                 const uint32_t* __restrict__ offs , uint32_t* __restrict__ ents, size_t ent_stride,
                                                 const uint32_t* __restrict__ skew, int wpl) {
    const uint32_t col = blockIdx.y;
    const bool aggregate = !SCATTER || skew[col] != 0;
    const Fr* sc = scalars + (size_t)col * stride;
    uint32_t* cnt = counters + (size_t)col * nbuckets;
    const uint32_t* off = SCATTER ? offs + (size_t)col * (nbuckets + 1) : nullptr;
    uint32_t* ent = SCATTER ? ents + (size_t)col * ent_stride : nullptr;
    const unsigned lane = threadIdx.x & 31;
    const uint32_t n_up = (n + 31u) & ~31u;
    for (uint32_t i = blockIdx.x * blockDim.x + threadIdx.x; i < n_up; i += gridDim.x * blockDim.x) {
        const bool valid = i < n;
        Fr s = fp_zero<FrTag>();
        if (valid) s = fp_from_mont(fp_load(sc + i));
        uint32_t carry = 0;
        MsmWindowSlot slot;
#pragma unroll 1
        for (int w = 0; w < W; ++w) {
            int32_t d = msm_next_digit(s.l, c, &carry);
            const uint32_t j = SUBWIN ? slot.level : (uint32_t)w;
            const bool nz = d != 0;
            const unsigned act = __ballot_sync(0xffffffffu, nz);
            if (nz && !aggregate) {
                const uint32_t bucket = (SUBWIN ? slot.set_off : 0u) + (uint32_t)(d < 0 ? -d : d) - 1u;
                ent[off[bucket] + atomicAdd(&cnt[bucket], 1u)] = (j * table_n + base_off + i) | (d < 0 ? 0x80000000u : 0u);
            } else if (nz) {
                const uint32_t bucket = (SUBWIN ? slot.set_off : 0u) + (uint32_t)(d < 0 ? -d : d) - 1u;
                const unsigned peers = __match_any_sync(act, bucket);
                const int leader = __ffs(peers) - 1;
                uint32_t base = 0;
                if ((int)lane == leader) base = atomicAdd(&cnt[bucket], (uint32_t)__popc(peers));
                if (SCATTER) {
                    base = __shfl_sync(peers, base, leader);
                    const uint32_t rank = __popc(peers & ((1u << lane) - 1u));
                    ent[off[bucket] + base + rank] = (j * table_n + base_off + i) | (d < 0 ? 0x80000000u : 0u);
                }
            }
            if (SUBWIN) slot.next(c, wpl);
        }
    }
}

template <bool SCATTER, bool SUBWIN>
__global__ void __launch_bounds__(MSM_TILE_THREADS, 1) k_digits_tile(const Fr* __restrict__ scalars, size_t stride, uint32_t n, uint32_t table_n, uint32_t base_off,
                                                                     int c, int W, uint32_t nbuckets, uint32_t tile, uint32_t* __restrict__ tile_counts ,
                                                                     const uint32_t* __restrict__ offs , uint32_t* __restrict__ ents, size_t ent_stride, int wpl) {
    extern __shared__ uint32_t sh_cnt[];
    const uint32_t col = blockIdx.y;
    const Fr* sc = scalars + (size_t)col * stride;
    uint32_t* tc = tile_counts + ((size_t)col * gridDim.x + blockIdx.x) * nbuckets;
    if (SCATTER) {
        const uint32_t* off = offs + (size_t)col * (nbuckets + 1);
        for (uint32_t b = threadIdx.x; b < nbuckets; b += blockDim.x) sh_cnt[b] = off[b] + tc[b];
    } else {
        for (uint32_t b = threadIdx.x; b < nbuckets; b += blockDim.x) sh_cnt[b] = 0;
    }
    __syncthreads();
    uint32_t* ent = SCATTER ? ents + (size_t)col * ent_stride : nullptr;
    const uint32_t lo = blockIdx.x * tile, hi = min(lo + tile, n);
    for (uint32_t i = lo + threadIdx.x; i < hi; i += blockDim.x) {
        Fr s = fp_from_mont(fp_load(sc + i));
        uint32_t carry = 0;
        MsmWindowSlot slot;
#pragma unroll 1
        for (int w = 0; w < W; ++w) {
            const int32_t d = msm_next_digit(s.l, c, &carry);
            if (d != 0) {
                const uint32_t bucket = (SUBWIN ? slot.set_off : 0u) + (uint32_t)(d < 0 ? -d : d) - 1u;
                const uint32_t pos = atomicAdd(&sh_cnt[bucket], 1u);
                if (SCATTER) ent[pos] = ((SUBWIN ? slot.level : (uint32_t)w) * table_n + base_off + i) | (d < 0 ? 0x80000000u : 0u);
            }
            if (SUBWIN) slot.next(c, wpl);
        }
    }
    if (!SCATTER) {
        __syncthreads();
        for (uint32_t b = threadIdx.x; b < nbuckets; b += blockDim.x) tc[b] = sh_cnt[b];
    }
}

__global__ void __launch_bounds__(256) k_tile_prefix(uint32_t* __restrict__ tile_counts, uint32_t tiles, uint32_t nbuckets, uint32_t* __restrict__ hist) {
    const uint32_t col = blockIdx.y;
    const uint32_t b = blockIdx.x * blockDim.x + threadIdx.x;
    if (b >= nbuckets) return;
    uint32_t* tc = tile_counts + (size_t)col * tiles * nbuckets + b;
    uint32_t acc = 0;
    for (uint32_t t0 = 0; t0 < tiles; t0 += 8) {
        uint32_t v[8];
#pragma unroll
        for (int j = 0; j < 8; ++j) v[j] = t0 + j < tiles ? tc[(size_t)(t0 + j) * nbuckets] : 0u;
#pragma unroll
        for (int j = 0; j < 8; ++j) {
            if (t0 + j < tiles) tc[(size_t)(t0 + j) * nbuckets] = acc;
            acc += v[j];
        }
    }
    hist[(size_t)col * nbuckets + b] = acc;
}

__global__ void __launch_bounds__(1024) k_scan_buckets(const uint32_t* __restrict__ counts, uint32_t* __restrict__ offs, uint32_t* __restrict__ chunk_offs,
                                                        uint32_t nbuckets, uint32_t cap, uint32_t* __restrict__ skew ) {
    __shared__ uint32_t sh_max;
    if (threadIdx.x == 0) sh_max = 0;
    __syncthreads();
    const uint32_t col = blockIdx.x;
    const uint32_t lc = 31u - (uint32_t)__clz(cap);
    const uint32_t* cnt = counts + (size_t)col * nbuckets;
    uint32_t* off = offs + (size_t)col * (nbuckets + 1);
    uint32_t* coff = chunk_offs + (size_t)col * (nbuckets + 1);
    const uint32_t ipt = (nbuckets + blockDim.x - 1) / blockDim.x;
    const uint32_t lo = threadIdx.x * ipt, hi = min(lo + ipt, nbuckets);
    uint32_t s = 0, cs = 0;
    uint32_t mx = 0;
    const bool vec = (ipt & 3u) == 0 && lo + ipt <= nbuckets;
    if (vec) {
        const uint4* c4 = reinterpret_cast<const uint4*>(cnt + lo);
#pragma unroll 4
        for (uint32_t q = 0; q < (ipt >> 2); ++q) {
            const uint4 v = c4[q];
            s += v.x + v.y + v.z + v.w;
            cs += ((v.x + cap - 1) >> lc) + ((v.y + cap - 1) >> lc) + ((v.z + cap - 1) >> lc) + ((v.w + cap - 1) >> lc);
            mx = max(max(mx, v.x), max(max(v.y, v.z), v.w));
        }
    } else {
        for (uint32_t b = lo; b < hi; ++b) { uint32_t v = cnt[b]; s += v; cs += ((v + cap - 1) >> lc); mx = max(mx, v); }
    }
    if (mx) atomicMax(&sh_max, mx);
    uint32_t tot, ctot;
    uint32_t ex = block_exclusive_scan(s, &tot);
    uint32_t cex = block_exclusive_scan(cs, &ctot);
    if (vec) {
        const uint4* c4 = reinterpret_cast<const uint4*>(cnt + lo);
#pragma unroll 4
        for (uint32_t q = 0; q < (ipt >> 2); ++q) {
            const uint4 v = c4[q];
            const uint32_t b = lo + 4 * q;
            off[b] = ex; coff[b] = cex; ex += v.x; cex += ((v.x + cap - 1) >> lc);
            off[b + 1] = ex; coff[b + 1] = cex; ex += v.y; cex += ((v.y + cap - 1) >> lc);
            off[b + 2] = ex; coff[b + 2] = cex; ex += v.z; cex += ((v.z + cap - 1) >> lc);
            off[b + 3] = ex; coff[b + 3] = cex; ex += v.w; cex += ((v.w + cap - 1) >> lc);
        }
    } else {
        for (uint32_t b = lo; b < hi; ++b) { uint32_t v = cnt[b]; off[b] = ex; coff[b] = cex; ex += v; cex += ((v + cap - 1) >> lc); }
    }
    if (threadIdx.x == 0) {
        off[nbuckets] = tot; coff[nbuckets] = ctot;
        skew[col] = sh_max > 16u * (tot / nbuckets + 1u) ? 1u : 0u;
    }
}

__global__ void __launch_bounds__(256) k_fill_chunks(const uint32_t* __restrict__ offs, const uint32_t* __restrict__ chunk_offs, uint32_t nbuckets, uint32_t cap,
                                                      uint32_t* __restrict__ chunk_start, uint32_t* __restrict__ chunk_len, size_t chunk_stride,
                                                      uint32_t* __restrict__ len_hist , uint32_t* __restrict__ heavy , uint32_t heavy_stride) {
    extern __shared__ uint32_t sh_hist[];
    const uint32_t col = blockIdx.y;
    for (uint32_t j = threadIdx.x; j <= cap; j += blockDim.x) sh_hist[j] = 0;
    __syncthreads();
    const uint32_t* off = offs + (size_t)col * (nbuckets + 1);
    const uint32_t* coff = chunk_offs + (size_t)col * (nbuckets + 1);
    uint32_t* cs = chunk_start + (size_t)col * chunk_stride;
    uint32_t* cl = chunk_len + (size_t)col * chunk_stride;
    const uint32_t b = blockIdx.x * blockDim.x + threadIdx.x;
    if (b < nbuckets) {
        const uint32_t start = off[b], size = off[b + 1] - start, c0 = coff[b], nch = coff[b + 1] - c0;
        for (uint32_t j = 0; j < nch; ++j) {
            const uint32_t len = min(cap, size - j * cap);
            cs[c0 + j] = start + j * cap;
            cl[c0 + j] = len;
            if (j + 1 == nch) atomicAdd(&sh_hist[len], 1u);
        }
        if (nch > 1) atomicAdd(&sh_hist[cap], nch - 1);
        if (nch > (uint32_t)HEAVY_CHUNKS) {
            uint32_t* hv = heavy + (size_t)col * heavy_stride;
            uint32_t slot = atomicAdd(&hv[0], 1u);
            if (slot + 1 < heavy_stride) hv[1 + slot] = b;
        }
    }
    __syncthreads();
    uint32_t* gh = len_hist + (size_t)col * (cap + 1);
    for (uint32_t j = threadIdx.x; j <= cap; j += blockDim.x) if (sh_hist[j]) atomicAdd(&gh[j], sh_hist[j]);
}

__global__ void k_len_offsets(const uint32_t* __restrict__ len_hist, uint32_t* __restrict__ len_offs, uint32_t cap) {
    const uint32_t col = blockIdx.x;
    if (threadIdx.x != 0) return;
    const uint32_t* h = len_hist + (size_t)col * (cap + 1);
    uint32_t* o = len_offs + (size_t)col * (cap + 1);
    uint32_t acc = 0;
    for (int l = (int)cap; l >= 0; --l) { o[l] = acc; acc += h[l]; }
}

__global__ void __launch_bounds__(256) k_order_chunks(const uint32_t* __restrict__ chunk_len, size_t chunk_stride, const uint32_t* __restrict__ chunk_offs, uint32_t nbuckets,
                                                       const uint32_t* __restrict__ len_offs, uint32_t* __restrict__ len_cursor, uint32_t cap, uint32_t* __restrict__ order) {
    const uint32_t col = blockIdx.y;
    const uint32_t nchunks = chunk_offs[(size_t)col * (nbuckets + 1) + nbuckets];
    const uint32_t* cl = chunk_len + (size_t)col * chunk_stride;
    uint32_t* ord = order + (size_t)col * chunk_stride;
    const uint32_t* lo = len_offs + (size_t)col * (cap + 1);
    uint32_t* lc = len_cursor + (size_t)col * (cap + 1);
    const unsigned lane = threadIdx.x & 31;
    const uint32_t n_up = (nchunks + 31u) & ~31u;
    for (uint32_t i = blockIdx.x * blockDim.x + threadIdx.x; i < n_up; i += gridDim.x * blockDim.x) {
        const bool valid = i < nchunks;
        const uint32_t len = valid ? cl[i] : 0;
        const unsigned act = __ballot_sync(0xffffffffu, valid);
        if (valid) {
            const unsigned peers = __match_any_sync(act, len);
            const int leader = __ffs(peers) - 1;
            uint32_t base = 0;
            if ((int)lane == leader) base = atomicAdd(&lc[len], (uint32_t)__popc(peers));
            base = __shfl_sync(peers, base, leader);
            ord[lo[len] + base + __popc(peers & ((1u << lane) - 1u))] = i;
        }
    }
}

DEV G1Affine load_base(const G1Affine* __restrict__ table, uint32_t e) {
    const uint4* q = reinterpret_cast<const uint4*>(table + (e & 0x7fffffffu));
    uint4 a = __ldg(q), b = __ldg(q + 1), c = __ldg(q + 2), d = __ldg(q + 3);
    G1Affine p;
    p.x.l[0] = a.x; p.x.l[1] = a.y; p.x.l[2] = a.z; p.x.l[3] = a.w; p.x.l[4] = b.x; p.x.l[5] = b.y; p.x.l[6] = b.z; p.x.l[7] = b.w;
    p.y.l[0] = c.x; p.y.l[1] = c.y; p.y.l[2] = c.z; p.y.l[3] = c.w; p.y.l[4] = d.x; p.y.l[5] = d.y; p.y.l[6] = d.z; p.y.l[7] = d.w;
    return p;
}
__global__ void __launch_bounds__(128, 4) k_accumulate(const G1Affine* __restrict__ table, const uint32_t* __restrict__ ents, size_t ent_stride,
                                                        const uint32_t* __restrict__ chunk_start, const uint32_t* __restrict__ chunk_len, const uint32_t* __restrict__ order,
                                                        size_t chunk_stride, const uint32_t* __restrict__ chunk_offs, uint32_t nbuckets, G1Xyzz* __restrict__ chunk_sums) {
    const uint32_t col = blockIdx.y;
    const uint32_t nchunks = chunk_offs[(size_t)col * (nbuckets + 1) + nbuckets];
    const uint32_t* ent = ents + (size_t)col * ent_stride;
    for (uint32_t t = blockIdx.x * blockDim.x + threadIdx.x; t < nchunks; t += gridDim.x * blockDim.x) {
        const uint32_t ch = order[(size_t)col * chunk_stride + t];
        const uint32_t start = chunk_start[(size_t)col * chunk_stride + ch], len = chunk_len[(size_t)col * chunk_stride + ch];
        uint32_t e = ent[start];
        G1Affine p = load_base(table, e);
        if (e >> 31) p = g1_neg(p);
        G1Xyzz acc = g1_to_xyzz(p);
        if (len > 1) {
            uint32_t e_next = ent[start + 1];
            G1Affine nx = load_base(table, e_next);
#pragma unroll 1
            for (uint32_t j = 1; j < len; ++j) {
                p = nx; e = e_next;
                if (j + 1 < len) { e_next = ent[start + j + 1]; nx = load_base(table, e_next); }
                if (e >> 31) p = g1_neg(p);
                acc = g1_add_mixed(acc, p);
            }
        }
        chunk_sums[(size_t)col * chunk_stride + ch] = acc;
    }
}

DEV G1Xyzz block_sum(G1Xyzz v, G1Xyzz* sh) {
    sh[threadIdx.x] = v;
    __syncthreads();
#pragma unroll 1
    for (unsigned s = blockDim.x / 2; s > 0; s >>= 1) {
        if (threadIdx.x < s) { v = g1_add(v, sh[threadIdx.x + s]); sh[threadIdx.x] = v; }
        __syncthreads();
    }
    return v;
}

__global__ void __launch_bounds__(128) k_combine(const uint32_t* __restrict__ chunk_offs, uint32_t nbuckets, const G1Xyzz* __restrict__ chunk_sums, size_t chunk_stride,
                                                  G1Xyzz* __restrict__ bucket_sums) {
    const uint32_t col = blockIdx.y;
    const uint32_t b = blockIdx.x * blockDim.x + threadIdx.x;
    if (b >= nbuckets) return;
    const uint32_t* coff = chunk_offs + (size_t)col * (nbuckets + 1);
    const uint32_t c0 = coff[b], nch = coff[b + 1] - c0;
    if (nch > (uint32_t)HEAVY_CHUNKS) return;
    const G1Xyzz* cs = chunk_sums + (size_t)col * chunk_stride;
    G1Xyzz acc = g1_xyzz_identity();
    if (nch > 0) acc = cs[c0];
#pragma unroll 1
    for (uint32_t j = 1; j < nch; ++j) acc = g1_add(acc, cs[c0 + j]);
    bucket_sums[(size_t)col * nbuckets + b] = acc;
}
__global__ void __launch_bounds__(TREE_THREADS) k_combine_heavy(const uint32_t* __restrict__ heavy, uint32_t heavy_stride, const uint32_t* __restrict__ chunk_offs, uint32_t nbuckets,
                                                                 const G1Xyzz* __restrict__ chunk_sums, size_t chunk_stride, G1Xyzz* __restrict__ bucket_sums) {
    __shared__ G1Xyzz sh[TREE_THREADS];
    const uint32_t col = blockIdx.y;
    const uint32_t* hv = heavy + (size_t)col * heavy_stride;
    const uint32_t nheavy = min(hv[0], heavy_stride - 1);
    const uint32_t* coff = chunk_offs + (size_t)col * (nbuckets + 1);
    const G1Xyzz* cs = chunk_sums + (size_t)col * chunk_stride;
    for (uint32_t h = blockIdx.x; h < nheavy; h += gridDim.x) {
        const uint32_t b = hv[1 + h];
        const uint32_t c0 = coff[b], nch = coff[b + 1] - c0;
        G1Xyzz acc = g1_xyzz_identity();
#pragma unroll 1
        for (uint32_t j = threadIdx.x; j < nch; j += TREE_THREADS) acc = g1_add(acc, cs[c0 + j]);
        acc = block_sum(acc, sh);
        if (threadIdx.x == 0) bucket_sums[(size_t)col * nbuckets + b] = acc;
        __syncthreads();
    }
}

template <int MIN_CTAS>
__global__ void __launch_bounds__(TREE_THREADS, MIN_CTAS) k_reduce(const G1Xyzz* __restrict__ bucket_sums, uint32_t nbuckets, G1Xyzz* __restrict__ partials, uint32_t nparts, uint32_t per_thread) {
    __shared__ G1Xyzz sh[TREE_THREADS];
    const uint32_t col = blockIdx.y;
    const G1Xyzz* bs = bucket_sums + (size_t)col * nbuckets;
    const uint32_t t = blockIdx.x * blockDim.x + threadIdx.x;
    const uint32_t lo = t * per_thread;
    G1Xyzz run = g1_xyzz_identity(), acc = g1_xyzz_identity();
    if (lo < nbuckets) {
        const uint32_t hi = min(lo + per_thread, nbuckets);
#pragma unroll 1
        for (uint32_t b = hi; b-- > lo;) {
            run = g1_add(run, bs[b]);
            acc = g1_add(acc, run);
        }
        if (lo > 0) acc = g1_add(acc, g1_mul_small(run, lo));
    }
    acc = block_sum(acc, sh);
    if (threadIdx.x == 0) partials[(size_t)col * nparts + blockIdx.x] = acc;
}
__global__ void __launch_bounds__(TREE_THREADS) k_final(const G1Xyzz* __restrict__ partials, uint32_t nparts, G1Xyzz* __restrict__ out) {
    __shared__ G1Xyzz sh[TREE_THREADS];
    const uint32_t col = blockIdx.x;
    G1Xyzz acc = g1_xyzz_identity();
#pragma unroll 1
    for (uint32_t j = threadIdx.x; j < nparts; j += blockDim.x) acc = g1_add(acc, partials[(size_t)col * nparts + j]);
    acc = block_sum(acc, sh);
    if (threadIdx.x == 0) out[col] = acc;
}

static constexpr int COOP_LT = TREE_THREADS / 4;
DEV G1Xyzz block_sum_coop(G1Xyzz v, G1Xyzz* sh) {
    const unsigned lt = threadIdx.x >> 2, q = threadIdx.x & 3;
    if (q == 0) sh[lt] = v;
    __syncthreads();
#pragma unroll 1
    for (unsigned s = COOP_LT / 2; s > 0; s >>= 1) {
        if (lt < s) { v = g1_add_coop4(v, sh[lt + s]); if (q == 0) sh[lt] = v; }
        __syncthreads();
    }
    return v;
}
__global__ void __launch_bounds__(TREE_THREADS) k_final_coop(const G1Xyzz* __restrict__ partials, uint32_t nparts, G1Xyzz* __restrict__ out) {
    __shared__ G1Xyzz sh[COOP_LT];
    const uint32_t col = blockIdx.x;
    G1Xyzz acc = g1_xyzz_identity();
#pragma unroll 1
    for (uint32_t j = threadIdx.x >> 2; j < nparts; j += COOP_LT) acc = g1_add_coop4(acc, partials[(size_t)col * nparts + j]);
    acc = block_sum_coop(acc, sh);
    if (threadIdx.x == 0) out[col] = acc;
}

__global__ void __launch_bounds__(32) k_subwindow_fold(const G1Xyzz* __restrict__ set_sums , int s, int c, uint32_t batch, G1Xyzz* __restrict__ out) {
    const uint32_t col = blockIdx.x * blockDim.x + threadIdx.x;
    if (col >= batch) return;
    const G1Xyzz* rs = set_sums + (size_t)col * s;
    G1Xyzz acc = rs[s - 1];
#pragma unroll 1
    for (int r = s - 2; r >= 0; --r) {
#pragma unroll 1
        for (int k = 0; k < c; ++k) acc = g1_dbl(acc);
        acc = g1_add(acc, rs[r]);
    }
    out[col] = acc;
}

__global__ void __launch_bounds__(128) k_g1_generate(uint64_t seed, size_t n, G1Affine* __restrict__ out) {
    const size_t i = (size_t)blockIdx.x * blockDim.x + threadIdx.x;
    if (i >= n) return;
    uint32_t s[8];
    uint64_t z = seed + 0x9e3779b97f4a7c15ull * (uint64_t)(i + 1);
#pragma unroll
    for (int w = 0; w < 4; ++w) {
        z += 0x9e3779b97f4a7c15ull;
        uint64_t x = z; x = (x ^ (x >> 30)) * 0xbf58476d1ce4e5b9ull; x = (x ^ (x >> 27)) * 0x94d049bb133111ebull; x ^= x >> 31;
        s[2 * w] = (uint32_t)x; s[2 * w + 1] = (uint32_t)(x >> 32);
    }
    s[7] &= 0x0fffffffu;
    G1Affine g; g.x = fp_one<FqTag>(); g.y = fp_one<FqTag>() + fp_one<FqTag>();
    G1Xyzz acc = g1_xyzz_identity();
#pragma unroll 1
    for (int b = 251; b >= 0; --b) {
        acc = g1_dbl(acc);
        if ((s[b >> 5] >> (b & 31)) & 1) acc = g1_add_mixed(acc, g);
    }
    out[i] = g1_to_affine(acc);
}
int g1_generate_run(uint64_t seed, size_t n, G1Affine* d_out, cudaStream_t st) {
    if (n == 0) return 0;
    k_g1_generate<<<div_up(n, 128), 128, 0, st>>>(seed, n, d_out); count_launch();
    B200_CUDA(cudaGetLastError());
    return 0;
}

__global__ void __launch_bounds__(128) k_g1_fixed_base_mul(const Fr* __restrict__ scalars, size_t n, G1Affine base, G1Affine* __restrict__ out) {
    const size_t i = (size_t)blockIdx.x * blockDim.x + threadIdx.x;
    if (i >= n) return;
    const Fr s = fp_from_mont(fp_load(scalars + i));
    G1Xyzz acc = g1_xyzz_identity();
#pragma unroll 1
    for (int b = 253; b >= 0; --b) {
        acc = g1_dbl(acc);
        if ((s.l[b >> 5] >> (b & 31)) & 1) acc = g1_add_mixed(acc, base);
    }
    out[i] = g1_to_affine(acc);
}
int g1_fixed_base_mul_run(const Fr* d_scalars, size_t n, const G1Affine& base, G1Affine* d_out, cudaStream_t st) {
    if (n == 0) return 0;
    k_g1_fixed_base_mul<<<div_up(n, 128), 128, 0, st>>>(d_scalars, n, base, d_out); count_launch();
    B200_CUDA(cudaGetLastError());
    return 0;
}

int g1_sum_run(const G1Xyzz* d_points, size_t groups, size_t count, G1Xyzz* d_out, cudaStream_t st) {
    if (groups == 0) return 0;
    B200_CHECK(groups <= 0x7fffffffu && count <= 0xffffffffu, -1, "g1_sum: sizes out of range");
    k_final_coop<<<(unsigned)groups, TREE_THREADS, 0, st>>>(d_points, (uint32_t)count, d_out); count_launch();
    B200_CUDA(cudaGetLastError());
    return 0;
}

static uint32_t pick_cap(size_t total_entries) {
    size_t target = total_entries / ((size_t)sm_count() * 512 * 4);
    uint32_t cap = 16;
    while (cap < 512 && cap < target) cap <<= 1;
    return cap;
}

size_t msm_workspace_per_column(const MsmTable& t, size_t n) {
    const size_t nb = (size_t)t.s << (t.c - 1), ents = n * t.W;
    const size_t chunk_stride = nb + ents / 16 + 1;
    const size_t tile_counts = nb <= MSM_TILE_MAX_BUCKETS ? (ents + nb) * 4 : 0;
    return ents * 4 + chunk_stride * (12 + sizeof(G1Xyzz)) + nb * (sizeof(G1Xyzz) + 24) + 65536 * (size_t)t.s + tile_counts;
}

int msm_run(const MsmTable& t, const Fr* d_scalars, size_t n, size_t stride, int batch, G1Xyzz* d_out, MsmWorkspace& ws, cudaStream_t st, size_t base_off) {
    B200_CHECK(base_off + n <= t.n, -1, "msm: pairs [%zu, %zu) but only %zu bases registered", base_off, base_off + n, t.n);
    B200_CHECK(batch > 0 && batch <= 65535, -1, "msm: batch %d out of range", batch);
    if (n == 0) {
        B200_CUDA(cudaMemsetAsync(d_out, 0, sizeof(G1Xyzz) * batch, st));
        return 0;
    }
    const int c = t.c, W = t.W, s = t.s;
    B200_CHECK((size_t)batch * s <= 65535, -1, "msm: batch %d x %d bucket sets out of range", batch, s);
    const uint32_t half = 1u << (c - 1), nb = half * (uint32_t)s;
    const int vcols = batch * s;
    const size_t ent_stride = (size_t)n * W;
    B200_CHECK(ent_stride < ((size_t)1 << 32), -1, "msm: n*W too large");
    const Config& cfg = config();
    const uint32_t cap = pick_cap(ent_stride * batch);
    const size_t chunk_stride = (size_t)nb + ent_stride / cap + 1;
    const uint32_t heavy_stride = (uint32_t)(ent_stride / ((size_t)cap * HEAVY_CHUNKS)) + 2;
    const size_t all_buckets = (size_t)batch * nb;
    uint32_t reduce_m = REDUCE_M_MAX, reduce_threads = TREE_THREADS;
    if (all_buckets <= ((size_t)1 << 15)) { reduce_m = 4; reduce_threads = 128; }
    else if (all_buckets <= ((size_t)1 << 18)) { reduce_m = 8; reduce_threads = 128; }
    else if (all_buckets <= ((size_t)5 << 17)) { reduce_m = 16; reduce_threads = 256; }
    else if (all_buckets < ((size_t)37 << 15)) { reduce_m = 32; reduce_threads = 128; }
    while (reduce_m > 1 && reduce_m > half) reduce_m >>= 1;
    if (cfg.msm_reduce_m >= 1 && cfg.msm_reduce_m <= 4096) reduce_m = (uint32_t)cfg.msm_reduce_m;
    if (cfg.msm_reduce_threads == 32 || cfg.msm_reduce_threads == 64 || cfg.msm_reduce_threads == 128 || cfg.msm_reduce_threads == 256) reduce_threads = (uint32_t)cfg.msm_reduce_threads;
    const uint32_t nparts = div_up(div_up(half, reduce_m), reduce_threads);
    uint32_t final_threads = 32;
    while (final_threads < (uint32_t)TREE_THREADS && final_threads < nparts) final_threads <<= 1;

    const unsigned sms = (unsigned)sm_count();
    const MsmRecodePlan rp = msm_pick_recode(n, batch, nb, W, (int)sms);
    const size_t n_hist = (size_t)batch * nb, n_len = (size_t)batch * (cap + 1), n_heavy = (size_t)batch * heavy_stride;
    const size_t counts_words = 2 * n_hist + 2 * n_len + n_heavy;
    if (ws.counts.ensure(counts_words * 4)) return -2;
    uint32_t* hist = ws.counts.as<uint32_t>();
    uint32_t* cursor = hist + n_hist;
    uint32_t* len_hist = cursor + n_hist;
    uint32_t* len_cursor = len_hist + n_len;
    uint32_t* heavy = len_cursor + n_len;
    uint32_t* zero_from = rp.tile ? len_hist : hist;
    const size_t zero_words = counts_words - (size_t)(zero_from - hist);
    uint32_t* tile_counts = nullptr;
    const size_t tile_smem = (size_t)nb * 4;
    auto* count_k = s == 1 ? k_digits_tile<false, false> : k_digits_tile<false, true>;
    auto* place_k = s == 1 ? k_digits_tile<true, false> : k_digits_tile<true, true>;
    if (rp.tile) {
        if (ws.tile_counts.ensure((size_t)batch * rp.tiles * nb * 4)) return -2;
        tile_counts = ws.tile_counts.as<uint32_t>();
        const int smem_limit = (int)(MSM_TILE_MAX_BUCKETS * 4);
        B200_CUDA(cudaFuncSetAttribute(count_k, cudaFuncAttributeMaxDynamicSharedMemorySize, smem_limit));
        B200_CUDA(cudaFuncSetAttribute(place_k, cudaFuncAttributeMaxDynamicSharedMemorySize, smem_limit));
    }
    const size_t n_off = (size_t)batch * (nb + 1);
    if (ws.offs.ensure((2 * n_off + n_len + (size_t)batch) * 4)) return -2;
    uint32_t* offs = ws.offs.as<uint32_t>();
    uint32_t* chunk_offs = offs + n_off;
    uint32_t* len_offs = chunk_offs + n_off;
    uint32_t* skew = len_offs + n_len;
    if (ws.ents.ensure((size_t)batch * ent_stride * 4)) return -2;
    uint32_t* ents = ws.ents.as<uint32_t>();
    if (ws.subs.ensure((size_t)batch * chunk_stride * 4 * 3)) return -2;
    uint32_t* chunk_start = ws.subs.as<uint32_t>();
    uint32_t* chunk_len = chunk_start + (size_t)batch * chunk_stride;
    uint32_t* order = chunk_len + (size_t)batch * chunk_stride;
    const size_t n_set = s > 1 ? (size_t)vcols : 0;
    if (ws.sums.ensure(sizeof(G1Xyzz) * ((size_t)batch * chunk_stride + (size_t)batch * nb + (size_t)vcols * nparts + n_set))) return -2;
    G1Xyzz* chunk_sums = ws.sums.as<G1Xyzz>();
    G1Xyzz* bucket_sums = chunk_sums + (size_t)batch * chunk_stride;
    G1Xyzz* partials = bucket_sums + (size_t)batch * nb;
    G1Xyzz* reduced = s > 1 ? partials + (size_t)vcols * nparts : d_out;

    ProfScope ps_total(PROF_MSM_TOTAL, st);
    B200_CUDA(cudaMemsetAsync(zero_from, 0, zero_words * 4, st));
    if (prof_enabled()) prof_mark(PROF_MSM_RECODE, st, true);
    const unsigned dig_blocks = min(div_up(n, 256), sms * 8u);
    const dim3 gd(dig_blocks, batch), gt(rp.tiles, batch);
    if (rp.tile) {
        count_k<<<gt, MSM_TILE_THREADS, tile_smem, st>>>(d_scalars, stride, (uint32_t)n, (uint32_t)t.n, (uint32_t)base_off, c, W, nb, rp.tile, tile_counts, nullptr, nullptr, 0, s);
        count_launch();
        k_tile_prefix<<<dim3(div_up(nb, 256), batch), 256, 0, st>>>(tile_counts, rp.tiles, nb, hist); count_launch();
    } else {
        if (s == 1) k_digits<false, false><<<gd, 256, 0, st>>>(d_scalars, stride, (uint32_t)n, (uint32_t)t.n, (uint32_t)base_off, c, W, nb, hist, nullptr, nullptr, 0, nullptr, 1);
        else k_digits<false, true><<<gd, 256, 0, st>>>(d_scalars, stride, (uint32_t)n, (uint32_t)t.n, (uint32_t)base_off, c, W, nb, hist, nullptr, nullptr, 0, nullptr, s);
        count_launch();
    }
    {
        ProfScope ps(PROF_MSM_SCAN, st);
        k_scan_buckets<<<batch, 1024, 0, st>>>(hist, offs, chunk_offs, nb, cap, skew); count_launch();
    }
    if (rp.tile) {
        place_k<<<gt, MSM_TILE_THREADS, tile_smem, st>>>(d_scalars, stride, (uint32_t)n, (uint32_t)t.n, (uint32_t)base_off, c, W, nb, rp.tile, tile_counts, offs, ents, ent_stride, s);
    } else if (s == 1) {
        k_digits<true, false><<<gd, 256, 0, st>>>(d_scalars, stride, (uint32_t)n, (uint32_t)t.n, (uint32_t)base_off, c, W, nb, cursor, offs, ents, ent_stride, skew, 1);
    } else {
        k_digits<true, true><<<gd, 256, 0, st>>>(d_scalars, stride, (uint32_t)n, (uint32_t)t.n, (uint32_t)base_off, c, W, nb, cursor, offs, ents, ent_stride, skew, s);
    }
    count_launch();
    k_fill_chunks<<<dim3(div_up(nb, 256), batch), 256, (cap + 1) * 4, st>>>(offs, chunk_offs, nb, cap, chunk_start, chunk_len, chunk_stride, len_hist, heavy, heavy_stride); count_launch();
    k_len_offsets<<<batch, 32, 0, st>>>(len_hist, len_offs, cap); count_launch();
    const unsigned ch_blocks = min(div_up(chunk_stride, 256), sms * 8u);
    k_order_chunks<<<dim3(ch_blocks, batch), 256, 0, st>>>(chunk_len, chunk_stride, chunk_offs, nb, len_offs, len_cursor, cap, order); count_launch();
    if (prof_enabled()) prof_mark(PROF_MSM_RECODE, st, false);
    const unsigned acc_blocks = min(div_up(chunk_stride, 128), sms * 16u);
    {
        ProfScope ps(PROF_MSM_ACCUMULATE, st);
        k_accumulate<<<dim3(acc_blocks, batch), 128, 0, st>>>(t.d_table, ents, ent_stride, chunk_start, chunk_len, order, chunk_stride, chunk_offs, nb, chunk_sums); count_launch();
    }
    ProfScope ps_tail(PROF_MSM_TAIL, st);
    k_combine<<<dim3(div_up(nb, 128), batch), 128, 0, st>>>(chunk_offs, nb, chunk_sums, chunk_stride, bucket_sums); count_launch();
    k_combine_heavy<<<dim3(32, batch), TREE_THREADS, 0, st>>>(heavy, heavy_stride, chunk_offs, nb, chunk_sums, chunk_stride, bucket_sums); count_launch();
    {
        ProfScope ps(PROF_MSM_REDUCE, st);
        k_reduce<1><<<dim3(nparts, vcols), reduce_threads, 0, st>>>(bucket_sums, half, partials, nparts, reduce_m); count_launch();
        k_final<<<vcols, final_threads, 0, st>>>(partials, nparts, reduced); count_launch();
    }
    if (s > 1) {
        ProfScope ps(PROF_MSM_FOLD, st);
        k_subwindow_fold<<<div_up((size_t)batch, 32), 32, 0, st>>>(reduced, s, c, (uint32_t)batch, d_out); count_launch();
    }
    B200_CUDA(cudaGetLastError());
    return 0;
}

}
```

Before: 0.08525.

## Use lazy-reduced Fq arithmetic in MSM bucket accumulation and reduction loops

Adds Fq Montgomery multiply, square, add and subtract variants whose results stay in [0, 2p), dropping the final conditional subtraction, plus a reduce helper and lazy XYZZ point additions. The MSM chunk accumulation loop and the bucket running-sum reduction now use these lazy additions and reduce only when storing the result. The aim is to cut per-operation instruction count in the hot elliptic-curve loops. In exchange, correctness depends on the [0, 2p) bounds holding through mul2 and the zero checks, and the debug and benchmark paths gain new ops for testing this.

```diff
diff --git a/ezkl_b200/csrc/debug.cu b/ezkl_b200/csrc/debug.cu
--- a/ezkl_b200/csrc/debug.cu
+++ b/ezkl_b200/csrc/debug.cu
@@ -4,6 +4,18 @@
 #include "ntt.cuh"
 
 namespace b200 {
+template <class Tag> HD Fp<Tag> dbg_field_lazy(int, const Fp<Tag>& x, const Fp<Tag>&) { return x; }
+HD Fq dbg_field_lazy(int op, const Fq& x, const Fq& y) {
+    switch (op) {
+        case 9: return fq_mul_lazy(x, y);
+        case 10: return fq_sqr_lazy(x);
+        case 11: return fq_add_lazy(x, y);
+        case 12: return fq_sub_lazy(x, y);
+        case 13: return fq_reduce(x);
+        case 14: return fq_mulsub2_lazy(x, y, x, x);
+        default: { Fq r = fp_zero<FqTag>(); r.l[0] = fq_is_zero_lazy(x) ? 1u : 0u; return r; }
+    }
+}
 template <class Tag>
 HD Fp<Tag> dbg_field(int op, const Fp<Tag>& x, const Fp<Tag>& y) {
     switch (op) {
@@ -15,7 +27,8 @@
         case 5: return fp_sqr(x);
         case 6: return fp_neg(x);
         case 7: return fp_dbl(x);
-        default: return fp_to_mont(x);
+        case 8: return fp_to_mont(x);
+        default: return dbg_field_lazy(op, x, y);
     }
 }
 template <class Tag>
@@ -31,13 +44,15 @@
     else r = g1_add_mixed(g1_to_xyzz(p), g1_neg(p));
     return g1_to_affine(r);
 }
-enum { DBG_XYZZ_COOP = 5 };
+enum { DBG_XYZZ_COOP = 5, DBG_XYZZ_LAZY = 7 };
 HD G1Xyzz dbg_xyzz(int op, const G1Xyzz& a, const G1Xyzz& b, uint32_t k) {
     switch (op) {
         case 0: return g1_add(a, b);
         case 1: return g1_dbl(a);
         case 2: { G1Affine q; q.x = b.x; q.y = b.y; return g1_add_mixed(a, q); }
         case 3: return g1_mul_small(a, k);
+        case DBG_XYZZ_LAZY: { G1Affine q; q.x = b.x; q.y = b.y; return g1_add_mixed_lazy(a, q); }
+        case DBG_XYZZ_LAZY + 1: return g1_add_lazy(a, b);
         default: {
             const G1Affine q = g1_to_affine(a);
             G1Xyzz r = g1_xyzz_identity(); r.x = q.x; r.y = q.y;
@@ -62,7 +77,7 @@
 }
 __global__ void k_dbg_xyzz(int op, const G1Xyzz* a, const G1Xyzz* b, const uint32_t* k, G1Xyzz* o, size_t n) {
     const size_t t = (size_t)blockIdx.x * blockDim.x + threadIdx.x;
-    if (op >= DBG_XYZZ_COOP) {
+    if (op == DBG_XYZZ_COOP || op == DBG_XYZZ_COOP + 1) {
         const size_t i = t >> 2;
         if (i >= n) return;
         const G1Xyzz r = op == DBG_XYZZ_COOP ? g1_add_coop4(a[i], b[i]) : g1_dbl_coop4(a[i]);
@@ -137,11 +152,12 @@
     } else if (VARIANT == 2) {
 #pragma unroll 1
         for (int i = 0; i < iters; ++i) { Fq r; fp_mul_portable<FqTag>(r.l, x.l, y.l); x = r; }
-    } else if (VARIANT == 3) {
+    } else if (VARIANT == 3 || VARIANT == 5) {
         G1Affine g; g.x = x; g.y = y;
         G1Xyzz acc = g1_dbl_affine(g);
 #pragma unroll 1
-        for (int i = 0; i < iters; ++i) { acc = g1_add_mixed(acc, g); g.x.l[0] += 1; }
+        for (int i = 0; i < iters; ++i) { acc = VARIANT == 3 ? g1_add_mixed(acc, g) : g1_add_mixed_lazy(acc, g); g.x.l[0] += 1; }
+        acc = g1_reduce(acc);
         x = acc.x + acc.y + acc.zz + acc.zzz;
     } else {
 #pragma unroll 1
@@ -238,7 +254,7 @@
     return 0;
 }
 int b200_debug_g1_xyzz_op(int op, const b200_g1_xyzz* a, const b200_g1_xyzz* b, const uint32_t* k, b200_g1_xyzz* out, size_t n) {
-    if (op < 0 || op > DBG_XYZZ_COOP + 1) return -1;
+    if (op < 0 || op > DBG_XYZZ_LAZY + 1) return -1;
     if (n == 0) return 0;
     DbgStage st;
     G1Xyzz *da, *db, *dout;
@@ -247,7 +263,7 @@
     if (int rc = st.in(b, 128 * n, &db)) return rc;
     if (int rc = st.in(k, 4 * n, &dk)) return rc;
     if (int rc = st.out(128 * n, &dout)) return rc;
-    const size_t threads = op >= DBG_XYZZ_COOP ? 4 * n : n;
+    const size_t threads = op == DBG_XYZZ_COOP || op == DBG_XYZZ_COOP + 1 ? 4 * n : n;
     k_dbg_xyzz<<<div_up(threads, 64), 64>>>(op, da, db, dk, dout, n);
     B200_CUDA(cudaGetLastError());
     B200_CUDA(cudaMemcpy(out, dout, 128 * n, cudaMemcpyDeviceToHost));
@@ -274,6 +290,7 @@
             case 1: k_bench_mul<1><<<blocks, threads>>>(d, iters); break;
             case 2: k_bench_mul<2><<<blocks, threads>>>(d, iters); break;
             case 3: k_bench_mul<3><<<blocks, threads>>>(d, iters); break;
+            case 5: k_bench_mul<5><<<blocks, threads>>>(d, iters); break;
             default: k_bench_mul<4><<<blocks, threads>>>(d, iters); break;
         }
         cudaEventRecord(e1);
@@ -386,7 +403,7 @@
     return 0;
 }
 int b200_debug_host_g1_xyzz_op(int op, const b200_g1_xyzz* a, const b200_g1_xyzz* b, const uint32_t* k, b200_g1_xyzz* out, size_t n) {
-    if (op < 0 || op >= DBG_XYZZ_COOP) return -1;
+    if (op < 0 || op > DBG_XYZZ_LAZY + 1 || op == DBG_XYZZ_COOP || op == DBG_XYZZ_COOP + 1) return -1;
     for (size_t i = 0; i < n; ++i) {
         G1Xyzz p, q; memcpy(&p, &a[i], 128); memcpy(&q, &b[i], 128);
         const G1Xyzz o = dbg_xyzz(op, p, q, k[i]); memcpy(&out[i], &o, 128);
diff --git a/ezkl_b200/csrc/ec.cuh b/ezkl_b200/csrc/ec.cuh
--- a/ezkl_b200/csrc/ec.cuh
+++ b/ezkl_b200/csrc/ec.cuh
@@ -59,6 +59,26 @@
     o.zz = a.zz * pp; o.zzz = a.zzz * ppp;
     return o;
 }
+HD G1Xyzz g1_add_mixed_lazy(const G1Xyzz& a, const G1Affine& q) {
+    if (g1_is_identity(q)) return a;
+    if (g1_is_identity(a)) return g1_to_xyzz(q);
+    Fq u2 = fq_mul_lazy(q.x, a.zz), s2 = fq_mul_lazy(q.y, a.zzz);
+    Fq p = fq_sub_lazy(u2, a.x), r = fq_sub_lazy(s2, a.y);
+    if (fq_is_zero_lazy(p)) {
+        if (fq_is_zero_lazy(r)) return g1_dbl_affine(q);
+        return g1_xyzz_identity();
+    }
+    G1Xyzz o;
+    Fq pp = fq_sqr_lazy(p), ppp = fq_mul_lazy(p, pp), qq = fq_mul_lazy(a.x, pp);
+    o.x = fq_sub_lazy(fq_sub_lazy(fq_sqr_lazy(r), ppp), fq_add_lazy(qq, qq));
+    o.y = fq_mulsub2_lazy(r, fq_sub_lazy(qq, o.x), a.y, ppp);
+    o.zz = fq_mul_lazy(a.zz, pp); o.zzz = fq_mul_lazy(a.zzz, ppp);
+    return o;
+}
+HD G1Xyzz g1_reduce(const G1Xyzz& a) {
+    G1Xyzz r; r.x = fq_reduce(a.x); r.y = fq_reduce(a.y); r.zz = fq_reduce(a.zz); r.zzz = fq_reduce(a.zzz);
+    return r;
+}
 HD G1Xyzz g1_add(const G1Xyzz& a, const G1Xyzz& b) {
     if (g1_is_identity(a)) return b;
     if (g1_is_identity(b)) return a;
@@ -73,6 +93,22 @@
     o.x = fp_sqr(r) - ppp - fp_dbl(qq);
     o.y = fp_mulsub2(r, qq - o.x, s1, ppp);
     o.zz = a.zz * b.zz * pp; o.zzz = a.zzz * b.zzz * ppp;
+    return o;
+}
+HD G1Xyzz g1_add_lazy(const G1Xyzz& a, const G1Xyzz& b) {
+    if (g1_is_identity(a)) return b;
+    if (g1_is_identity(b)) return a;
+    Fq u1 = fq_mul_lazy(a.x, b.zz), u2 = fq_mul_lazy(b.x, a.zz), s1 = fq_mul_lazy(a.y, b.zzz), s2 = fq_mul_lazy(b.y, a.zzz);
+    Fq p = fq_sub_lazy(u2, u1), r = fq_sub_lazy(s2, s1);
+    if (fq_is_zero_lazy(p)) {
+        if (fq_is_zero_lazy(r)) return g1_dbl(g1_reduce(a));
+        return g1_xyzz_identity();
+    }
+    G1Xyzz o;
+    Fq pp = fq_sqr_lazy(p), ppp = fq_mul_lazy(p, pp), qq = fq_mul_lazy(u1, pp);
+    o.x = fq_sub_lazy(fq_sub_lazy(fq_sqr_lazy(r), ppp), fq_add_lazy(qq, qq));
+    o.y = fq_mulsub2_lazy(r, fq_sub_lazy(qq, o.x), s1, ppp);
+    o.zz = fq_mul_lazy(fq_mul_lazy(a.zz, b.zz), pp); o.zzz = fq_mul_lazy(fq_mul_lazy(a.zzz, b.zzz), ppp);
     return o;
 }
 HD G1Affine g1_to_affine(const G1Xyzz& p) {
diff --git a/ezkl_b200/csrc/field.cuh b/ezkl_b200/csrc/field.cuh
--- a/ezkl_b200/csrc/field.cuh
+++ b/ezkl_b200/csrc/field.cuh
@@ -191,6 +191,42 @@
     return a * b - c * d;
 #endif
 }
+HD Fq fq_reduce(const Fq& a) {
+    Fq r;
+#if defined(__CUDA_ARCH__)
+    fq_reduce_ptx(r.l, a.l);
+#else
+    uint32_t d[8]; uint64_t br = 0;
+    for (int j = 0; j < 8; ++j) { uint64_t s = (uint64_t)a.l[j] - FqTag::mod(j) - br; d[j] = (uint32_t)s; br = (s >> 32) & 1; }
+    for (int j = 0; j < 8; ++j) r.l[j] = br ? a.l[j] : d[j];
+#endif
+    return r;
+}
+HD bool fq_is_zero_lazy(const Fq& a) {
+    uint32_t z = 0, e = 0;
+#pragma unroll
+    for (int i = 0; i < 8; ++i) { z |= a.l[i]; e |= a.l[i] ^ FqTag::mod(i); }
+    return z == 0 || e == 0;
+}
+#if defined(__CUDA_ARCH__)
+DEV Fq fq_mul_lazy(const Fq& a, const Fq& b) { Fq r; fq_mul_lazy_ptx(r.l, a.l, b.l); return r; }
+DEV Fq fq_sqr_lazy(const Fq& a) { Fq r; fq_sqr_lazy_ptx(r.l, a.l); return r; }
+DEV Fq fq_add_lazy(const Fq& a, const Fq& b) { Fq r; fq_add_lazy_ptx(r.l, a.l, b.l); return r; }
+DEV Fq fq_sub_lazy(const Fq& a, const Fq& b) { Fq r; fq_sub_lazy_ptx(r.l, a.l, b.l); return r; }
+DEV Fq fq_mulsub2_lazy(const Fq& a, const Fq& b, const Fq& c, const Fq& d) {
+    const Fq nc = fq_sub_lazy(fp_zero<FqTag>(), c);
+    Fq r;
+    fq_mul2_ptx(r.l, a.l, b.l, nc.l, d.l);
+    return r;
+}
+#else
+HD Fq fq_mul_lazy(const Fq& a, const Fq& b) { return fq_reduce(a) * fq_reduce(b); }
+HD Fq fq_sqr_lazy(const Fq& a) { return fq_reduce(a) * fq_reduce(a); }
+HD Fq fq_add_lazy(const Fq& a, const Fq& b) { return fq_reduce(a) + fq_reduce(b); }
+HD Fq fq_sub_lazy(const Fq& a, const Fq& b) { return fq_reduce(a) - fq_reduce(b); }
+HD Fq fq_mulsub2_lazy(const Fq& a, const Fq& b, const Fq& c, const Fq& d) { return fq_reduce(a) * fq_reduce(b) - fq_reduce(c) * fq_reduce(d); }
+#endif
+
 template <class Tag> HD Fp<Tag> fp_from_mont(const Fp<Tag>& a) {
     Fp<Tag> one_c = fp_zero<Tag>(); one_c.l[0] = 1;
     return a * one_c;
diff --git a/ezkl_b200/csrc/fp_gen.py b/ezkl_b200/csrc/fp_gen.py
--- a/ezkl_b200/csrc/fp_gen.py
+++ b/ezkl_b200/csrc/fp_gen.py
@@ -13,7 +13,7 @@
     return [(x >> (32 * i)) & M32 for i in range(n)]
 
 
-def gen_mul(mod):
+def gen_mul(mod, lazy=False):
     Ml = limbs(mod)
     inv = (-pow(mod, -1, 1 << 32)) & M32
     ins = []
@@ -57,11 +57,12 @@
         ins.append(("addc.u32", nO[7], nO[7], "0"))
         E, O = nE, nO
         reduce_row(E, O)
-    T = ["t%d" % i for i in range(8)]
+    T = ["%s%d" % ("r" if lazy else "t", i) for i in range(8)]
     for j in range(7):
         ins.append((("add.cc.u32" if j == 0 else "addc.cc.u32"), T[j], O[j], E[j + 1]))
     ins.append(("addc.u32", T[7], O[7], "0"))
-    ins += final_sub(T, Ml)
+    if not lazy:
+        ins += final_sub(T, Ml)
     return ins
 
 
@@ -126,7 +127,7 @@
     return ins
 
 
-def gen_sqr(mod):
+def gen_sqr(mod, lazy=False):
     Ml = limbs(mod)
     inv = (-pow(mod, -1, 1 << 32)) & M32
     ins = []
@@ -188,11 +189,12 @@
             ins.append(("addc.u32", nO[7], nO[7], "0"))
         E, O = nE, nO
         reduce_row(E, O)
-    T = ["t%d" % i for i in range(8)]
+    T = ["%s%d" % ("r" if lazy else "t", i) for i in range(8)]
     for j in range(7):
         ins.append((("add.cc.u32" if j == 0 else "addc.cc.u32"), T[j], O[j], E[j + 1]))
     ins.append(("addc.u32", T[7], O[7], "0"))
-    ins += final_sub(T, Ml)
+    if not lazy:
+        ins += final_sub(T, Ml)
     return ins
 
 
@@ -209,8 +211,8 @@
     return ins
 
 
-def gen_add(mod):
-    Ml = limbs(mod)
+def gen_add(mod, lazy=False):
+    Ml = limbs(2 * mod if lazy else mod)
     ins = []
     T = ["t%d" % i for i in range(8)]
     for j in range(8):
@@ -219,8 +221,8 @@
     return ins + final_sub(T, Ml)
 
 
-def gen_sub(mod):
-    Ml = limbs(mod)
+def gen_sub(mod, lazy=False):
+    Ml = limbs(2 * mod if lazy else mod)
     ins = []
     T = ["t%d" % i for i in range(8)]
     for j in range(8):
@@ -232,6 +234,10 @@
         op = "add.cc.u32" if j == 0 else ("addc.cc.u32" if j < 7 else "addc.u32")
         ins.append((op, "r%d" % j, T[j], "s%d" % j))
     return ins
+
+
+def gen_reduce(mod):
+    return final_sub(["a%d" % i for i in range(8)], limbs(mod))
 
 
 def run(ins, regs):
@@ -320,6 +326,43 @@
     return len(mul), len(add), len(sub), len(mul2), len(sqr)
 
 
+def check_lazy(name, mod, trials=3000):
+    rng = random.Random(hash(name + "lazy") & 0xFFFF)
+    mul, sqr, add, sub, red = gen_mul(mod, True), gen_sqr(mod, True), gen_add(mod, True), gen_sub(mod, True), gen_reduce(mod)
+    mul2 = gen_mul2(mod)
+    Rinv = pow(1 << 256, -1, mod)
+    edge = [0, 1, mod - 1, mod, mod + 1, 2 * mod - 2, 2 * mod - 1, mod >> 1, mod + (mod >> 1), 0xFFFFFFFF, (1 << 254) - 1,
+            2 * mod - (1 << 128)]
+    vals = edge + [rng.randrange(mod, 2 * mod) for _ in range(trials)] + [rng.randrange(2 * mod) for _ in range(trials)]
+
+    def regs_of(**kw):
+        return {"%s%d" % (nm, i): w for nm, v in kw.items() for i, w in enumerate(limbs(v))}
+
+    def result(ins, regs, what, exp, *ops):
+        out = run(ins, regs)
+        got = sum(out["r%d" % i] << (32 * i) for i in range(8))
+        assert got < 2 * mod and got % mod == exp % mod, (name, what) + tuple(hex(x) for x in ops) + (hex(got),)
+        return got
+
+    pairs = [(x, y) for x in edge for y in edge] + [(vals[rng.randrange(len(vals))], vals[rng.randrange(len(vals))]) for _ in range(trials)]
+    for a, b in pairs:
+        regs = regs_of(a=a, b=b)
+        result(mul, dict(regs), "mul_lazy", a * b * Rinv, a, b)
+        result(add, dict(regs), "add_lazy", a + b, a, b)
+        result(sub, dict(regs), "sub_lazy", a - b, a, b)
+    for a in vals:
+        regs = regs_of(a=a)
+        result(sqr, dict(regs), "sqr_lazy", a * a * Rinv, a)
+        got = result(red, dict(regs), "reduce", a, a)
+        assert got == a % mod, (name, "reduce", hex(a), hex(got))
+    edge2 = [0, 1, mod - 1, mod, 2 * mod - 1, mod + (mod >> 1)]
+    quads = [(a, b, c, d) for a in edge2 for b in edge2 for c in edge2 for d in edge2]
+    quads += [tuple(vals[rng.randrange(len(vals))] for _ in range(4)) for _ in range(trials)]
+    for a, b, c, d in quads:
+        result(mul2, regs_of(a=a, b=b, c=c, d=d), "mul2 on [0, 2M)", (a * b + c * d) * Rinv, a, b, c, d)
+    return len(mul), len(sqr), len(add), len(sub), len(red)
+
+
 def emit_fn(fname, ins, n_in):
     tmp = sorted({x for it in ins for x in it[1:] if x[0] in "xytsmuw" and not x.startswith("0x")} | {"brw"})
     tmp = [t for t in tmp if t != "p"]
@@ -366,6 +409,14 @@
         out.append(emit_fn("%s_sub_ptx" % name, gen_sub(mod), 2))
         out.append(emit_fn("%s_mul2_ptx" % name, gen_mul2(mod), 4))
         out.append(emit_fn("%s_sqr_ptx" % name, gen_sqr(mod), 1))
+        if name == "fq":
+            n = check_lazy(name, mod)
+            print("%s: verified on [0, 2p); instruction counts mul_lazy/sqr_lazy/add_lazy/sub_lazy/reduce = %s" % (name, n))
+            out.append(emit_fn("%s_mul_lazy_ptx" % name, gen_mul(mod, True), 2))
+            out.append(emit_fn("%s_sqr_lazy_ptx" % name, gen_sqr(mod, True), 1))
+            out.append(emit_fn("%s_add_lazy_ptx" % name, gen_add(mod, True), 2))
+            out.append(emit_fn("%s_sub_lazy_ptx" % name, gen_sub(mod, True), 2))
+            out.append(emit_fn("%s_reduce_ptx" % name, gen_reduce(mod), 1))
     out.append("#endif  // __CUDA_ARCH__")
     if "--check" not in sys.argv:
         import os
diff --git a/ezkl_b200/csrc/fp_ptx.cuh b/ezkl_b200/csrc/fp_ptx.cuh
--- a/ezkl_b200/csrc/fp_ptx.cuh
+++ b/ezkl_b200/csrc/fp_ptx.cuh
@@ -2308,4 +2308,691 @@
         : "r"(a[0]), "r"(a[1]), "r"(a[2]), "r"(a[3]), "r"(a[4]), "r"(a[5]), "r"(a[6]), "r"(a[7]));
 }
 
+__device__ __forceinline__ void fq_mul_lazy_ptx(uint32_t* r, const uint32_t* a, const uint32_t* b) {
+    asm(
+        "{\n\t"
+        ".reg .u32 brw, m, x0, x1, x2, x3, x4, x5, x6, x7, y0, y1, y2, y3, y4, y5, y6, y7;\n\t"
+        ".reg .pred p;\n\t"
+        "mul.lo.u32 x0, %8, %16;\n\t"
+        "mul.hi.u32 x1, %8, %16;\n\t"
+        "mul.lo.u32 x2, %10, %16;\n\t"
+        "mul.hi.u32 x3, %10, %16;\n\t"
+        "mul.lo.u32 x4, %12, %16;\n\t"
+        "mul.hi.u32 x5, %12, %16;\n\t"
+        "mul.lo.u32 x6, %14, %16;\n\t"
+        "mul.hi.u32 x7, %14, %16;\n\t"
+        "mul.lo.u32 y0, %9, %16;\n\t"
+        "mul.hi.u32 y1, %9, %16;\n\t"
+        "mul.lo.u32 y2, %11, %16;\n\t"
+        "mul.hi.u32 y3, %11, %16;\n\t"
+        "mul.lo.u32 y4, %13, %16;\n\t"
+        "mul.hi.u32 y5, %13, %16;\n\t"
+        "mul.lo.u32 y6, %15, %16;\n\t"
+        "mul.hi.u32 y7, %15, %16;\n\t"
+        "mul.lo.u32 m, x0, 0xe4866389;\n\t"
+        "mad.lo.cc.u32 y0, m, 0x3c208c16, y0;\n\t"
+        "madc.hi.cc.u32 y1, m, 0x3c208c16, y1;\n\t"
+        "madc.lo.cc.u32 y2, m, 0x97816a91, y2;\n\t"
+        "madc.hi.cc.u32 y3, m, 0x97816a91, y3;\n\t"
+        "madc.lo.cc.u32 y4, m, 0xb85045b6, y4;\n\t"
+        "madc.hi.cc.u32 y5, m, 0xb85045b6, y5;\n\t"
+        "madc.lo.cc.u32 y6, m, 0x30644e72, y6;\n\t"
+        "madc.hi.cc.u32 y7, m, 0x30644e72, y7;\n\t"
+        "mad.lo.cc.u32 x0, m, 0xd87cfd47, x0;\n\t"
+        "madc.hi.cc.u32 x1, m, 0xd87cfd47, x1;\n\t"
+        "madc.lo.cc.u32 x2, m, 0x6871ca8d, x2;\n\t"
+        "madc.hi.cc.u32 x3, m, 0x6871ca8d, x3;\n\t"
+        "madc.lo.cc.u32 x4, m, 0x8181585d, x4;\n\t"
+        "madc.hi.cc.u32 x5, m, 0x8181585d, x5;\n\t"
+        "madc.lo.cc.u32 x6, m, 0xe131a029, x6;\n\t"
+        "madc.hi.cc.u32 x7, m, 0xe131a029, x7;\n\t"
+        "addc.u32 y7, y7, 0;\n\t"
+        "add.cc.u32 y0, y0, x1;\n\t"
+        "madc.lo.cc.u32 x0, %9, %17, x2;\n\t"
+        "madc.hi.cc.u32 x1, %9, %17, x3;\n\t"
+        "madc.lo.cc.u32 x2, %11, %17, x4;\n\t"
+        "madc.hi.cc.u32 x3, %11, %17, x5;\n\t"
+        "madc.lo.cc.u32 x4, %13, %17, x6;\n\t"
+        "madc.hi.cc.u32 x5, %13, %17, x7;\n\t"
+        "madc.lo.cc.u32 x6, %15, %17, 0;\n\t"
+        "madc.hi.cc.u32 x7, %15, %17, 0;\n\t"
+        "mad.lo.cc.u32 y0, %8, %17, y0;\n\t"
+        "madc.hi.cc.u32 y1, %8, %17, y1;\n\t"
+        "madc.lo.cc.u32 y2, %10, %17, y2;\n\t"
+        "madc.hi.cc.u32 y3, %10, %17, y3;\n\t"
+        "madc.lo.cc.u32 y4, %12, %17, y4;\n\t"
+        "madc.hi.cc.u32 y5, %12, %17, y5;\n\t"
+        "madc.lo.cc.u32 y6, %14, %17, y6;\n\t"
+        "madc.hi.cc.u32 y7, %14, %17, y7;\n\t"
+        "addc.u32 x7, x7, 0;\n\t"
+        "mul.lo.u32 m, y0, 0xe4866389;\n\t"
+        "mad.lo.cc.u32 x0, m, 0x3c208c16, x0;\n\t"
+        "madc.hi.cc.u32 x1, m, 0x3c208c16, x1;\n\t"
+        "madc.lo.cc.u32 x2, m, 0x97816a91, x2;\n\t"
+        "madc.hi.cc.u32 x3, m, 0x97816a91, x3;\n\t"
+        "madc.lo.cc.u32 x4, m, 0xb85045b6, x4;\n\t"
+        "madc.hi.cc.u32 x5, m, 0xb85045b6, x5;\n\t"
+        "madc.lo.cc.u32 x6, m, 0x30644e72, x6;\n\t"
+        "madc.hi.cc.u32 x7, m, 0x30644e72, x7;\n\t"
+        "mad.lo.cc.u32 y0, m, 0xd87cfd47, y0;\n\t"
+        "madc.hi.cc.u32 y1, m, 0xd87cfd47, y1;\n\t"
+        "madc.lo.cc.u32 y2, m, 0x6871ca8d, y2;\n\t"
+        "madc.hi.cc.u32 y3, m, 0x6871ca8d, y3;\n\t"
+        "madc.lo.cc.u32 y4, m, 0x8181585d, y4;\n\t"
+        "madc.hi.cc.u32 y5, m, 0x8181585d, y5;\n\t"
+        "madc.lo.cc.u32 y6, m, 0xe131a029, y6;\n\t"
+        "madc.hi.cc.u32 y7, m, 0xe131a029, y7;\n\t"
+        "addc.u32 x7, x7, 0;\n\t"
+        "add.cc.u32 x0, x0, y1;\n\t"
+        "madc.lo.cc.u32 y0, %9, %18, y2;\n\t"
+        "madc.hi.cc.u32 y1, %9, %18, y3;\n\t"
+        "madc.lo.cc.u32 y2, %11, %18, y4;\n\t"
+        "madc.hi.cc.u32 y3, %11, %18, y5;\n\t"
+        "madc.lo.cc.u32 y4, %13, %18, y6;\n\t"
+        "madc.hi.cc.u32 y5, %13, %18, y7;\n\t"
+        "madc.lo.cc.u32 y6, %15, %18, 0;\n\t"
+        "madc.hi.cc.u32 y7, %15, %18, 0;\n\t"
+        "mad.lo.cc.u32 x0, %8, %18, x0;\n\t"
+        "madc.hi.cc.u32 x1, %8, %18, x1;\n\t"
+        "madc.lo.cc.u32 x2, %10, %18, x2;\n\t"
+        "madc.hi.cc.u32 x3, %10, %18, x3;\n\t"
+        "madc.lo.cc.u32 x4, %12, %18, x4;\n\t"
+        "madc.hi.cc.u32 x5, %12, %18, x5;\n\t"
+        "madc.lo.cc.u32 x6, %14, %18, x6;\n\t"
+        "madc.hi.cc.u32 x7, %14, %18, x7;\n\t"
+        "addc.u32 y7, y7, 0;\n\t"
+        "mul.lo.u32 m, x0, 0xe4866389;\n\t"
+        "mad.lo.cc.u32 y0, m, 0x3c208c16, y0;\n\t"
+        "madc.hi.cc.u32 y1, m, 0x3c208c16, y1;\n\t"
+        "madc.lo.cc.u32 y2, m, 0x97816a91, y2;\n\t"
+        "madc.hi.cc.u32 y3, m, 0x97816a91, y3;\n\t"
+        "madc.lo.cc.u32 y4, m, 0xb85045b6, y4;\n\t"
+        "madc.hi.cc.u32 y5, m, 0xb85045b6, y5;\n\t"
+        "madc.lo.cc.u32 y6, m, 0x30644e72, y6;\n\t"
+        "madc.hi.cc.u32 y7, m, 0x30644e72, y7;\n\t"
+        "mad.lo.cc.u32 x0, m, 0xd87cfd47, x0;\n\t"
+        "madc.hi.cc.u32 x1, m, 0xd87cfd47, x1;\n\t"
+        "madc.lo.cc.u32 x2, m, 0x6871ca8d, x2;\n\t"
+        "madc.hi.cc.u32 x3, m, 0x6871ca8d, x3;\n\t"
+        "madc.lo.cc.u32 x4, m, 0x8181585d, x4;\n\t"
+        "madc.hi.cc.u32 x5, m, 0x8181585d, x5;\n\t"
+        "madc.lo.cc.u32 x6, m, 0xe131a029, x6;\n\t"
+        "madc.hi.cc.u32 x7, m, 0xe131a029, x7;\n\t"
+        "addc.u32 y7, y7, 0;\n\t"
+        "add.cc.u32 y0, y0, x1;\n\t"
+        "madc.lo.cc.u32 x0, %9, %19, x2;\n\t"
+        "madc.hi.cc.u32 x1, %9, %19, x3;\n\t"
+        "madc.lo.cc.u32 x2, %11, %19, x4;\n\t"
+        "madc.hi.cc.u32 x3, %11, %19, x5;\n\t"
+        "madc.lo.cc.u32 x4, %13, %19, x6;\n\t"
+        "madc.hi.cc.u32 x5, %13, %19, x7;\n\t"
+        "madc.lo.cc.u32 x6, %15, %19, 0;\n\t"
+        "madc.hi.cc.u32 x7, %15, %19, 0;\n\t"
+        "mad.lo.cc.u32 y0, %8, %19, y0;\n\t"
+        "madc.hi.cc.u32 y1, %8, %19, y1;\n\t"
+        "madc.lo.cc.u32 y2, %10, %19, y2;\n\t"
+        "madc.hi.cc.u32 y3, %10, %19, y3;\n\t"
+        "madc.lo.cc.u32 y4, %12, %19, y4;\n\t"
+        "madc.hi.cc.u32 y5, %12, %19, y5;\n\t"
+        "madc.lo.cc.u32 y6, %14, %19, y6;\n\t"
+        "madc.hi.cc.u32 y7, %14, %19, y7;\n\t"
+        "addc.u32 x7, x7, 0;\n\t"
+        "mul.lo.u32 m, y0, 0xe4866389;\n\t"
+        "mad.lo.cc.u32 x0, m, 0x3c208c16, x0;\n\t"
+        "madc.hi.cc.u32 x1, m, 0x3c208c16, x1;\n\t"
+        "madc.lo.cc.u32 x2, m, 0x97816a91, x2;\n\t"
+        "madc.hi.cc.u32 x3, m, 0x97816a91, x3;\n\t"
+        "madc.lo.cc.u32 x4, m, 0xb85045b6, x4;\n\t"
+        "madc.hi.cc.u32 x5, m, 0xb85045b6, x5;\n\t"
+        "madc.lo.cc.u32 x6, m, 0x30644e72, x6;\n\t"
+        "madc.hi.cc.u32 x7, m, 0x30644e72, x7;\n\t"
+        "mad.lo.cc.u32 y0, m, 0xd87cfd47, y0;\n\t"
+        "madc.hi.cc.u32 y1, m, 0xd87cfd47, y1;\n\t"
+        "madc.lo.cc.u32 y2, m, 0x6871ca8d, y2;\n\t"
+        "madc.hi.cc.u32 y3, m, 0x6871ca8d, y3;\n\t"
+        "madc.lo.cc.u32 y4, m, 0x8181585d, y4;\n\t"
+        "madc.hi.cc.u32 y5, m, 0x8181585d, y5;\n\t"
+        "madc.lo.cc.u32 y6, m, 0xe131a029, y6;\n\t"
+        "madc.hi.cc.u32 y7, m, 0xe131a029, y7;\n\t"
+        "addc.u32 x7, x7, 0;\n\t"
+        "add.cc.u32 x0, x0, y1;\n\t"
+        "madc.lo.cc.u32 y0, %9, %20, y2;\n\t"
+        "madc.hi.cc.u32 y1, %9, %20, y3;\n\t"
+        "madc.lo.cc.u32 y2, %11, %20, y4;\n\t"
+        "madc.hi.cc.u32 y3, %11, %20, y5;\n\t"
+        "madc.lo.cc.u32 y4, %13, %20, y6;\n\t"
+        "madc.hi.cc.u32 y5, %13, %20, y7;\n\t"
+        "madc.lo.cc.u32 y6, %15, %20, 0;\n\t"
+        "madc.hi.cc.u32 y7, %15, %20, 0;\n\t"
+        "mad.lo.cc.u32 x0, %8, %20, x0;\n\t"
+        "madc.hi.cc.u32 x1, %8, %20, x1;\n\t"
+        "madc.lo.cc.u32 x2, %10, %20, x2;\n\t"
+        "madc.hi.cc.u32 x3, %10, %20, x3;\n\t"
+        "madc.lo.cc.u32 x4, %12, %20, x4;\n\t"
+        "madc.hi.cc.u32 x5, %12, %20, x5;\n\t"
+        "madc.lo.cc.u32 x6, %14, %20, x6;\n\t"
+        "madc.hi.cc.u32 x7, %14, %20, x7;\n\t"
+        "addc.u32 y7, y7, 0;\n\t"
+        "mul.lo.u32 m, x0, 0xe4866389;\n\t"
+        "mad.lo.cc.u32 y0, m, 0x3c208c16, y0;\n\t"
+        "madc.hi.cc.u32 y1, m, 0x3c208c16, y1;\n\t"
+        "madc.lo.cc.u32 y2, m, 0x97816a91, y2;\n\t"
+        "madc.hi.cc.u32 y3, m, 0x97816a91, y3;\n\t"
+        "madc.lo.cc.u32 y4, m, 0xb85045b6, y4;\n\t"
+        "madc.hi.cc.u32 y5, m, 0xb85045b6, y5;\n\t"
+        "madc.lo.cc.u32 y6, m, 0x30644e72, y6;\n\t"
+        "madc.hi.cc.u32 y7, m, 0x30644e72, y7;\n\t"
+        "mad.lo.cc.u32 x0, m, 0xd87cfd47, x0;\n\t"
+        "madc.hi.cc.u32 x1, m, 0xd87cfd47, x1;\n\t"
+        "madc.lo.cc.u32 x2, m, 0x6871ca8d, x2;\n\t"
+        "madc.hi.cc.u32 x3, m, 0x6871ca8d, x3;\n\t"
+        "madc.lo.cc.u32 x4, m, 0x8181585d, x4;\n\t"
+        "madc.hi.cc.u32 x5, m, 0x8181585d, x5;\n\t"
+        "madc.lo.cc.u32 x6, m, 0xe131a029, x6;\n\t"
+        "madc.hi.cc.u32 x7, m, 0xe131a029, x7;\n\t"
+        "addc.u32 y7, y7, 0;\n\t"
+        "add.cc.u32 y0, y0, x1;\n\t"
+        "madc.lo.cc.u32 x0, %9, %21, x2;\n\t"
+        "madc.hi.cc.u32 x1, %9, %21, x3;\n\t"
+        "madc.lo.cc.u32 x2, %11, %21, x4;\n\t"
+        "madc.hi.cc.u32 x3, %11, %21, x5;\n\t"
+        "madc.lo.cc.u32 x4, %13, %21, x6;\n\t"
+        "madc.hi.cc.u32 x5, %13, %21, x7;\n\t"
+        "madc.lo.cc.u32 x6, %15, %21, 0;\n\t"
+        "madc.hi.cc.u32 x7, %15, %21, 0;\n\t"
+        "mad.lo.cc.u32 y0, %8, %21, y0;\n\t"
+        "madc.hi.cc.u32 y1, %8, %21, y1;\n\t"
+        "madc.lo.cc.u32 y2, %10, %21, y2;\n\t"
+        "madc.hi.cc.u32 y3, %10, %21, y3;\n\t"
+        "madc.lo.cc.u32 y4, %12, %21, y4;\n\t"
+        "madc.hi.cc.u32 y5, %12, %21, y5;\n\t"
+        "madc.lo.cc.u32 y6, %14, %21, y6;\n\t"
+        "madc.hi.cc.u32 y7, %14, %21, y7;\n\t"
+        "addc.u32 x7, x7, 0;\n\t"
+        "mul.lo.u32 m, y0, 0xe4866389;\n\t"
+        "mad.lo.cc.u32 x0, m, 0x3c208c16, x0;\n\t"
+        "madc.hi.cc.u32 x1, m, 0x3c208c16, x1;\n\t"
+        "madc.lo.cc.u32 x2, m, 0x97816a91, x2;\n\t"
+        "madc.hi.cc.u32 x3, m, 0x97816a91, x3;\n\t"
+        "madc.lo.cc.u32 x4, m, 0xb85045b6, x4;\n\t"
+        "madc.hi.cc.u32 x5, m, 0xb85045b6, x5;\n\t"
+        "madc.lo.cc.u32 x6, m, 0x30644e72, x6;\n\t"
+        "madc.hi.cc.u32 x7, m, 0x30644e72, x7;\n\t"
+        "mad.lo.cc.u32 y0, m, 0xd87cfd47, y0;\n\t"
+        "madc.hi.cc.u32 y1, m, 0xd87cfd47, y1;\n\t"
+        "madc.lo.cc.u32 y2, m, 0x6871ca8d, y2;\n\t"
+        "madc.hi.cc.u32 y3, m, 0x6871ca8d, y3;\n\t"
+        "madc.lo.cc.u32 y4, m, 0x8181585d, y4;\n\t"
+        "madc.hi.cc.u32 y5, m, 0x8181585d, y5;\n\t"
+        "madc.lo.cc.u32 y6, m, 0xe131a029, y6;\n\t"
+        "madc.hi.cc.u32 y7, m, 0xe131a029, y7;\n\t"
+        "addc.u32 x7, x7, 0;\n\t"
+        "add.cc.u32 x0, x0, y1;\n\t"
+        "madc.lo.cc.u32 y0, %9, %22, y2;\n\t"
+        "madc.hi.cc.u32 y1, %9, %22, y3;\n\t"
+        "madc.lo.cc.u32 y2, %11, %22, y4;\n\t"
+        "madc.hi.cc.u32 y3, %11, %22, y5;\n\t"
+        "madc.lo.cc.u32 y4, %13, %22, y6;\n\t"
+        "madc.hi.cc.u32 y5, %13, %22, y7;\n\t"
+        "madc.lo.cc.u32 y6, %15, %22, 0;\n\t"
+        "madc.hi.cc.u32 y7, %15, %22, 0;\n\t"
+        "mad.lo.cc.u32 x0, %8, %22, x0;\n\t"
+        "madc.hi.cc.u32 x1, %8, %22, x1;\n\t"
+        "madc.lo.cc.u32 x2, %10, %22, x2;\n\t"
+        "madc.hi.cc.u32 x3, %10, %22, x3;\n\t"
+        "madc.lo.cc.u32 x4, %12, %22, x4;\n\t"
+        "madc.hi.cc.u32 x5, %12, %22, x5;\n\t"
+        "madc.lo.cc.u32 x6, %14, %22, x6;\n\t"
+        "madc.hi.cc.u32 x7, %14, %22, x7;\n\t"
+        "addc.u32 y7, y7, 0;\n\t"
+        "mul.lo.u32 m, x0, 0xe4866389;\n\t"
+        "mad.lo.cc.u32 y0, m, 0x3c208c16, y0;\n\t"
+        "madc.hi.cc.u32 y1, m, 0x3c208c16, y1;\n\t"
+        "madc.lo.cc.u32 y2, m, 0x97816a91, y2;\n\t"
+        "madc.hi.cc.u32 y3, m, 0x97816a91, y3;\n\t"
+        "madc.lo.cc.u32 y4, m, 0xb85045b6, y4;\n\t"
+        "madc.hi.cc.u32 y5, m, 0xb85045b6, y5;\n\t"
+        "madc.lo.cc.u32 y6, m, 0x30644e72, y6;\n\t"
+        "madc.hi.cc.u32 y7, m, 0x30644e72, y7;\n\t"
+        "mad.lo.cc.u32 x0, m, 0xd87cfd47, x0;\n\t"
+        "madc.hi.cc.u32 x1, m, 0xd87cfd47, x1;\n\t"
+        "madc.lo.cc.u32 x2, m, 0x6871ca8d, x2;\n\t"
+        "madc.hi.cc.u32 x3, m, 0x6871ca8d, x3;\n\t"
+        "madc.lo.cc.u32 x4, m, 0x8181585d, x4;\n\t"
+        "madc.hi.cc.u32 x5, m, 0x8181585d, x5;\n\t"
+        "madc.lo.cc.u32 x6, m, 0xe131a029, x6;\n\t"
+        "madc.hi.cc.u32 x7, m, 0xe131a029, x7;\n\t"
+        "addc.u32 y7, y7, 0;\n\t"
+        "add.cc.u32 y0, y0, x1;\n\t"
+        "madc.lo.cc.u32 x0, %9, %23, x2;\n\t"
+        "madc.hi.cc.u32 x1, %9, %23, x3;\n\t"
+        "madc.lo.cc.u32 x2, %11, %23, x4;\n\t"
+        "madc.hi.cc.u32 x3, %11, %23, x5;\n\t"
+        "madc.lo.cc.u32 x4, %13, %23, x6;\n\t"
+        "madc.hi.cc.u32 x5, %13, %23, x7;\n\t"
+        "madc.lo.cc.u32 x6, %15, %23, 0;\n\t"
+        "madc.hi.cc.u32 x7, %15, %23, 0;\n\t"
+        "mad.lo.cc.u32 y0, %8, %23, y0;\n\t"
+        "madc.hi.cc.u32 y1, %8, %23, y1;\n\t"
+        "madc.lo.cc.u32 y2, %10, %23, y2;\n\t"
+        "madc.hi.cc.u32 y3, %10, %23, y3;\n\t"
+        "madc.lo.cc.u32 y4, %12, %23, y4;\n\t"
+        "madc.hi.cc.u32 y5, %12, %23, y5;\n\t"
+        "madc.lo.cc.u32 y6, %14, %23, y6;\n\t"
+        "madc.hi.cc.u32 y7, %14, %23, y7;\n\t"
+        "addc.u32 x7, x7, 0;\n\t"
+        "mul.lo.u32 m, y0, 0xe4866389;\n\t"
+        "mad.lo.cc.u32 x0, m, 0x3c208c16, x0;\n\t"
+        "madc.hi.cc.u32 x1, m, 0x3c208c16, x1;\n\t"
+        "madc.lo.cc.u32 x2, m, 0x97816a91, x2;\n\t"
+        "madc.hi.cc.u32 x3, m, 0x97816a91, x3;\n\t"
+        "madc.lo.cc.u32 x4, m, 0xb85045b6, x4;\n\t"
+        "madc.hi.cc.u32 x5, m, 0xb85045b6, x5;\n\t"
+        "madc.lo.cc.u32 x6, m, 0x30644e72, x6;\n\t"
+        "madc.hi.cc.u32 x7, m, 0x30644e72, x7;\n\t"
+        "mad.lo.cc.u32 y0, m, 0xd87cfd47, y0;\n\t"
+        "madc.hi.cc.u32 y1, m, 0xd87cfd47, y1;\n\t"
+        "madc.lo.cc.u32 y2, m, 0x6871ca8d, y2;\n\t"
+        "madc.hi.cc.u32 y3, m, 0x6871ca8d, y3;\n\t"
+        "madc.lo.cc.u32 y4, m, 0x8181585d, y4;\n\t"
+        "madc.hi.cc.u32 y5, m, 0x8181585d, y5;\n\t"
+        "madc.lo.cc.u32 y6, m, 0xe131a029, y6;\n\t"
+        "madc.hi.cc.u32 y7, m, 0xe131a029, y7;\n\t"
+        "addc.u32 x7, x7, 0;\n\t"
+        "add.cc.u32 %0, x0, y1;\n\t"
+        "addc.cc.u32 %1, x1, y2;\n\t"
+        "addc.cc.u32 %2, x2, y3;\n\t"
+        "addc.cc.u32 %3, x3, y4;\n\t"
+        "addc.cc.u32 %4, x4, y5;\n\t"
+        "addc.cc.u32 %5, x5, y6;\n\t"
+        "addc.cc.u32 %6, x6, y7;\n\t"
+        "addc.u32 %7, x7, 0;\n\t"
+        "}\n\t"
+        : "=r"(r[0]), "=r"(r[1]), "=r"(r[2]), "=r"(r[3]), "=r"(r[4]), "=r"(r[5]), "=r"(r[6]), "=r"(r[7])
+        : "r"(a[0]), "r"(a[1]), "r"(a[2]), "r"(a[3]), "r"(a[4]), "r"(a[5]), "r"(a[6]), "r"(a[7]), "r"(b[0]), "r"(b[1]), "r"(b[2]), "r"(b[3]), "r"(b[4]), "r"(b[5]), "r"(b[6]), "r"(b[7]));
+}
+
+__device__ __forceinline__ void fq_sqr_lazy_ptx(uint32_t* r, const uint32_t* a) {
+    asm(
+        "{\n\t"
+        ".reg .u32 brw, m, u2, u3, u4, u5, u6, u7, w1, w2, w3, w4, w5, w6, w7, x0, x1, x2, x3, x4, x5, x6, x7, y0, y1, y2, y3, y4, y5, y6, y7;\n\t"
+        ".reg .pred p;\n\t"
+        "shl.b32 w1, %9, 1;\n\t"
+        "shl.b32 w2, %10, 1;\n\t"
+        "shl.b32 w3, %11, 1;\n\t"
+        "shl.b32 w4, %12, 1;\n\t"
+        "shl.b32 w5, %13, 1;\n\t"
+        "shl.b32 w6, %14, 1;\n\t"
+        "shl.b32 w7, %15, 1;\n\t"
+        "shf.l.clamp.b32 u2, %9, %10, 1;\n\t"
+        "shf.l.clamp.b32 u3, %10, %11, 1;\n\t"
+        "shf.l.clamp.b32 u4, %11, %12, 1;\n\t"
+        "shf.l.clamp.b32 u5, %12, %13, 1;\n\t"
+        "shf.l.clamp.b32 u6, %13, %14, 1;\n\t"
+        "shf.l.clamp.b32 u7, %14, %15, 1;\n\t"
+        "mul.lo.u32 x0, %8, %8;\n\t"
+        "mul.hi.u32 x1, %8, %8;\n\t"
+        "mul.lo.u32 x2, u2, %8;\n\t"
+        "mul.hi.u32 x3, u2, %8;\n\t"
+        "mul.lo.u32 x4, u4, %8;\n\t"
+        "mul.hi.u32 x5, u4, %8;\n\t"
+        "mul.lo.u32 x6, u6, %8;\n\t"
+        "mul.hi.u32 x7, u6, %8;\n\t"
+        "mul.lo.u32 y0, w1, %8;\n\t"
+        "mul.hi.u32 y1, w1, %8;\n\t"
+        "mul.lo.u32 y2, u3, %8;\n\t"
+        "mul.hi.u32 y3, u3, %8;\n\t"
+        "mul.lo.u32 y4, u5, %8;\n\t"
+        "mul.hi.u32 y5, u5, %8;\n\t"
+        "mul.lo.u32 y6, u7, %8;\n\t"
+        "mul.hi.u32 y7, u7, %8;\n\t"
+        "mul.lo.u32 m, x0, 0xe4866389;\n\t"
+        "mad.lo.cc.u32 y0, m, 0x3c208c16, y0;\n\t"
+        "madc.hi.cc.u32 y1, m, 0x3c208c16, y1;\n\t"
+        "madc.lo.cc.u32 y2, m, 0x97816a91, y2;\n\t"
+        "madc.hi.cc.u32 y3, m, 0x97816a91, y3;\n\t"
+        "madc.lo.cc.u32 y4, m, 0xb85045b6, y4;\n\t"
+        "madc.hi.cc.u32 y5, m, 0xb85045b6, y5;\n\t"
+        "madc.lo.cc.u32 y6, m, 0x30644e72, y6;\n\t"
+        "madc.hi.cc.u32 y7, m, 0x30644e72, y7;\n\t"
+        "mad.lo.cc.u32 x0, m, 0xd87cfd47, x0;\n\t"
+        "madc.hi.cc.u32 x1, m, 0xd87cfd47, x1;\n\t"
+        "madc.lo.cc.u32 x2, m, 0x6871ca8d, x2;\n\t"
+        "madc.hi.cc.u32 x3, m, 0x6871ca8d, x3;\n\t"
+        "madc.lo.cc.u32 x4, m, 0x8181585d, x4;\n\t"
+        "madc.hi.cc.u32 x5, m, 0x8181585d, x5;\n\t"
+        "madc.lo.cc.u32 x6, m, 0xe131a029, x6;\n\t"
+        "madc.hi.cc.u32 x7, m, 0xe131a029, x7;\n\t"
+        "addc.u32 y7, y7, 0;\n\t"
+        "add.cc.u32 y0, y0, x1;\n\t"
+        "madc.lo.cc.u32 x0, %9, %9, x2;\n\t"
+        "madc.hi.cc.u32 x1, %9, %9, x3;\n\t"
+        "madc.lo.cc.u32 x2, u3, %9, x4;\n\t"
+        "madc.hi.cc.u32 x3, u3, %9, x5;\n\t"
+        "madc.lo.cc.u32 x4, u5, %9, x6;\n\t"
+        "madc.hi.cc.u32 x5, u5, %9, x7;\n\t"
+        "madc.lo.cc.u32 x6, u7, %9, 0;\n\t"
+        "madc.hi.cc.u32 x7, u7, %9, 0;\n\t"
+        "mad.lo.cc.u32 y2, w2, %9, y2;\n\t"
+        "madc.hi.cc.u32 y3, w2, %9, y3;\n\t"
+        "madc.lo.cc.u32 y4, u4, %9, y4;\n\t"
+        "madc.hi.cc.u32 y5, u4, %9, y5;\n\t"
+        "madc.lo.cc.u32 y6, u6, %9, y6;\n\t"
+        "madc.hi.cc.u32 y7, u6, %9, y7;\n\t"
+        "addc.u32 x7, x7, 0;\n\t"
+        "mul.lo.u32 m, y0, 0xe4866389;\n\t"
+        "mad.lo.cc.u32 x0, m, 0x3c208c16, x0;\n\t"
+        "madc.hi.cc.u32 x1, m, 0x3c208c16, x1;\n\t"
+        "madc.lo.cc.u32 x2, m, 0x97816a91, x2;\n\t"
+        "madc.hi.cc.u32 x3, m, 0x97816a91, x3;\n\t"
+        "madc.lo.cc.u32 x4, m, 0xb85045b6, x4;\n\t"
+        "madc.hi.cc.u32 x5, m, 0xb85045b6, x5;\n\t"
+        "madc.lo.cc.u32 x6, m, 0x30644e72, x6;\n\t"
+        "madc.hi.cc.u32 x7, m, 0x30644e72, x7;\n\t"
+        "mad.lo.cc.u32 y0, m, 0xd87cfd47, y0;\n\t"
+        "madc.hi.cc.u32 y1, m, 0xd87cfd47, y1;\n\t"
+        "madc.lo.cc.u32 y2, m, 0x6871ca8d, y2;\n\t"
+        "madc.hi.cc.u32 y3, m, 0x6871ca8d, y3;\n\t"
+        "madc.lo.cc.u32 y4, m, 0x8181585d, y4;\n\t"
+        "madc.hi.cc.u32 y5, m, 0x8181585d, y5;\n\t"
+        "madc.lo.cc.u32 y6, m, 0xe131a029, y6;\n\t"
+        "madc.hi.cc.u32 y7, m, 0xe131a029, y7;\n\t"
+        "addc.u32 x7, x7, 0;\n\t"
+        "add.cc.u32 x0, x0, y1;\n\t"
+        "addc.cc.u32 y0, y2, 0;\n\t"
+        "addc.cc.u32 y1, y3, 0;\n\t"
+        "madc.lo.cc.u32 y2, w3, %10, y4;\n\t"
+        "madc.hi.cc.u32 y3, w3, %10, y5;\n\t"
+        "madc.lo.cc.u32 y4, u5, %10, y6;\n\t"
+        "madc.hi.cc.u32 y5, u5, %10, y7;\n\t"
+        "madc.lo.cc.u32 y6, u7, %10, 0;\n\t"
+        "madc.hi.cc.u32 y7, u7, %10, 0;\n\t"
+        "mad.lo.cc.u32 x2, %10, %10, x2;\n\t"
+        "madc.hi.cc.u32 x3, %10, %10, x3;\n\t"
+        "madc.lo.cc.u32 x4, u4, %10, x4;\n\t"
+        "madc.hi.cc.u32 x5, u4, %10, x5;\n\t"
+        "madc.lo.cc.u32 x6, u6, %10, x6;\n\t"
+        "madc.hi.cc.u32 x7, u6, %10, x7;\n\t"
+        "addc.u32 y7, y7, 0;\n\t"
+        "mul.lo.u32 m, x0, 0xe4866389;\n\t"
+        "mad.lo.cc.u32 y0, m, 0x3c208c16, y0;\n\t"
+        "madc.hi.cc.u32 y1, m, 0x3c208c16, y1;\n\t"
+        "madc.lo.cc.u32 y2, m, 0x97816a91, y2;\n\t"
+        "madc.hi.cc.u32 y3, m, 0x97816a91, y3;\n\t"
+        "madc.lo.cc.u32 y4, m, 0xb85045b6, y4;\n\t"
+        "madc.hi.cc.u32 y5, m, 0xb85045b6, y5;\n\t"
+        "madc.lo.cc.u32 y6, m, 0x30644e72, y6;\n\t"
+        "madc.hi.cc.u32 y7, m, 0x30644e72, y7;\n\t"
+        "mad.lo.cc.u32 x0, m, 0xd87cfd47, x0;\n\t"
+        "madc.hi.cc.u32 x1, m, 0xd87cfd47, x1;\n\t"
+        "madc.lo.cc.u32 x2, m, 0x6871ca8d, x2;\n\t"
+        "madc.hi.cc.u32 x3, m, 0x6871ca8d, x3;\n\t"
+        "madc.lo.cc.u32 x4, m, 0x8181585d, x4;\n\t"
+        "madc.hi.cc.u32 x5, m, 0x8181585d, x5;\n\t"
+        "madc.lo.cc.u32 x6, m, 0xe131a029, x6;\n\t"
+        "madc.hi.cc.u32 x7, m, 0xe131a029, x7;\n\t"
+        "addc.u32 y7, y7, 0;\n\t"
+        "add.cc.u32 y0, y0, x1;\n\t"
+        "addc.cc.u32 x0, x2, 0;\n\t"
+        "addc.cc.u32 x1, x3, 0;\n\t"
+        "madc.lo.cc.u32 x2, %11, %11, x4;\n\t"
+        "madc.hi.cc.u32 x3, %11, %11, x5;\n\t"
+        "madc.lo.cc.u32 x4, u5, %11, x6;\n\t"
+        "madc.hi.cc.u32 x5, u5, %11, x7;\n\t"
+        "madc.lo.cc.u32 x6, u7, %11, 0;\n\t"
+        "madc.hi.cc.u32 x7, u7, %11, 0;\n\t"
+        "mad.lo.cc.u32 y4, w4, %11, y4;\n\t"
+        "madc.hi.cc.u32 y5, w4, %11, y5;\n\t"
+        "madc.lo.cc.u32 y6, u6, %11, y6;\n\t"
+        "madc.hi.cc.u32 y7, u6, %11, y7;\n\t"
+        "addc.u32 x7, x7, 0;\n\t"
+        "mul.lo.u32 m, y0, 0xe4866389;\n\t"
+        "mad.lo.cc.u32 x0, m, 0x3c208c16, x0;\n\t"
+        "madc.hi.cc.u32 x1, m, 0x3c208c16, x1;\n\t"
+        "madc.lo.cc.u32 x2, m, 0x97816a91, x2;\n\t"
+        "madc.hi.cc.u32 x3, m, 0x97816a91, x3;\n\t"
+        "madc.lo.cc.u32 x4, m, 0xb85045b6, x4;\n\t"
+        "madc.hi.cc.u32 x5, m, 0xb85045b6, x5;\n\t"
+        "madc.lo.cc.u32 x6, m, 0x30644e72, x6;\n\t"
+        "madc.hi.cc.u32 x7, m, 0x30644e72, x7;\n\t"
+        "mad.lo.cc.u32 y0, m, 0xd87cfd47, y0;\n\t"
+        "madc.hi.cc.u32 y1, m, 0xd87cfd47, y1;\n\t"
+        "madc.lo.cc.u32 y2, m, 0x6871ca8d, y2;\n\t"
+        "madc.hi.cc.u32 y3, m, 0x6871ca8d, y3;\n\t"
+        "madc.lo.cc.u32 y4, m, 0x8181585d, y4;\n\t"
+        "madc.hi.cc.u32 y5, m, 0x8181585d, y5;\n\t"
+        "madc.lo.cc.u32 y6, m, 0xe131a029, y6;\n\t"
+        "madc.hi.cc.u32 y7, m, 0xe131a029, y7;\n\t"
+        "addc.u32 x7, x7, 0;\n\t"
+        "add.cc.u32 x0, x0, y1;\n\t"
+        "addc.cc.u32 y0, y2, 0;\n\t"
+        "addc.cc.u32 y1, y3, 0;\n\t"
+        "addc.cc.u32 y2, y4, 0;\n\t"
+        "addc.cc.u32 y3, y5, 0;\n\t"
+        "madc.lo.cc.u32 y4, w5, %12, y6;\n\t"
+        "madc.hi.cc.u32 y5, w5, %12, y7;\n\t"
+        "madc.lo.cc.u32 y6, u7, %12, 0;\n\t"
+        "madc.hi.cc.u32 y7, u7, %12, 0;\n\t"
+        "mad.lo.cc.u32 x4, %12, %12, x4;\n\t"
+        "madc.hi.cc.u32 x5, %12, %12, x5;\n\t"
+        "madc.lo.cc.u32 x6, u6, %12, x6;\n\t"
+        "madc.hi.cc.u32 x7, u6, %12, x7;\n\t"
+        "addc.u32 y7, y7, 0;\n\t"
+        "mul.lo.u32 m, x0, 0xe4866389;\n\t"
+        "mad.lo.cc.u32 y0, m, 0x3c208c16, y0;\n\t"
+        "madc.hi.cc.u32 y1, m, 0x3c208c16, y1;\n\t"
+        "madc.lo.cc.u32 y2, m, 0x97816a91, y2;\n\t"
+        "madc.hi.cc.u32 y3, m, 0x97816a91, y3;\n\t"
+        "madc.lo.cc.u32 y4, m, 0xb85045b6, y4;\n\t"
+        "madc.hi.cc.u32 y5, m, 0xb85045b6, y5;\n\t"
+        "madc.lo.cc.u32 y6, m, 0x30644e72, y6;\n\t"
+        "madc.hi.cc.u32 y7, m, 0x30644e72, y7;\n\t"
+        "mad.lo.cc.u32 x0, m, 0xd87cfd47, x0;\n\t"
+        "madc.hi.cc.u32 x1, m, 0xd87cfd47, x1;\n\t"
+        "madc.lo.cc.u32 x2, m, 0x6871ca8d, x2;\n\t"
+        "madc.hi.cc.u32 x3, m, 0x6871ca8d, x3;\n\t"
+        "madc.lo.cc.u32 x4, m, 0x8181585d, x4;\n\t"
+        "madc.hi.cc.u32 x5, m, 0x8181585d, x5;\n\t"
+        "madc.lo.cc.u32 x6, m, 0xe131a029, x6;\n\t"
+        "madc.hi.cc.u32 x7, m, 0xe131a029, x7;\n\t"
+        "addc.u32 y7, y7, 0;\n\t"
+        "add.cc.u32 y0, y0, x1;\n\t"
+        "addc.cc.u32 x0, x2, 0;\n\t"
+        "addc.cc.u32 x1, x3, 0;\n\t"
+        "addc.cc.u32 x2, x4, 0;\n\t"
+        "addc.cc.u32 x3, x5, 0;\n\t"
+        "madc.lo.cc.u32 x4, %13, %13, x6;\n\t"
+        "madc.hi.cc.u32 x5, %13, %13, x7;\n\t"
+        "madc.lo.cc.u32 x6, u7, %13, 0;\n\t"
+        "madc.hi.cc.u32 x7, u7, %13, 0;\n\t"
+        "mad.lo.cc.u32 y6, w6, %13, y6;\n\t"
+        "madc.hi.cc.u32 y7, w6, %13, y7;\n\t"
+        "addc.u32 x7, x7, 0;\n\t"
+        "mul.lo.u32 m, y0, 0xe4866389;\n\t"
+        "mad.lo.cc.u32 x0, m, 0x3c208c16, x0;\n\t"
+        "madc.hi.cc.u32 x1, m, 0x3c208c16, x1;\n\t"
+        "madc.lo.cc.u32 x2, m, 0x97816a91, x2;\n\t"
+        "madc.hi.cc.u32 x3, m, 0x97816a91, x3;\n\t"
+        "madc.lo.cc.u32 x4, m, 0xb85045b6, x4;\n\t"
+        "madc.hi.cc.u32 x5, m, 0xb85045b6, x5;\n\t"
+        "madc.lo.cc.u32 x6, m, 0x30644e72, x6;\n\t"
+        "madc.hi.cc.u32 x7, m, 0x30644e72, x7;\n\t"
+        "mad.lo.cc.u32 y0, m, 0xd87cfd47, y0;\n\t"
+        "madc.hi.cc.u32 y1, m, 0xd87cfd47, y1;\n\t"
+        "madc.lo.cc.u32 y2, m, 0x6871ca8d, y2;\n\t"
+        "madc.hi.cc.u32 y3, m, 0x6871ca8d, y3;\n\t"
+        "madc.lo.cc.u32 y4, m, 0x8181585d, y4;\n\t"
+        "madc.hi.cc.u32 y5, m, 0x8181585d, y5;\n\t"
+        "madc.lo.cc.u32 y6, m, 0xe131a029, y6;\n\t"
+        "madc.hi.cc.u32 y7, m, 0xe131a029, y7;\n\t"
+        "addc.u32 x7, x7, 0;\n\t"
+        "add.cc.u32 x0, x0, y1;\n\t"
+        "addc.cc.u32 y0, y2, 0;\n\t"
+        "addc.cc.u32 y1, y3, 0;\n\t"
+        "addc.cc.u32 y2, y4, 0;\n\t"
+        "addc.cc.u32 y3, y5, 0;\n\t"
+        "addc.cc.u32 y4, y6, 0;\n\t"
+        "addc.cc.u32 y5, y7, 0;\n\t"
+        "madc.lo.cc.u32 y6, w7, %14, 0;\n\t"
+        "madc.hi.cc.u32 y7, w7, %14, 0;\n\t"
+        "mad.lo.cc.u32 x6, %14, %14, x6;\n\t"
+        "madc.hi.cc.u32 x7, %14, %14, x7;\n\t"
+        "addc.u32 y7, y7, 0;\n\t"
+        "mul.lo.u32 m, x0, 0xe4866389;\n\t"
+        "mad.lo.cc.u32 y0, m, 0x3c208c16, y0;\n\t"
+        "madc.hi.cc.u32 y1, m, 0x3c208c16, y1;\n\t"
+        "madc.lo.cc.u32 y2, m, 0x97816a91, y2;\n\t"
+        "madc.hi.cc.u32 y3, m, 0x97816a91, y3;\n\t"
+        "madc.lo.cc.u32 y4, m, 0xb85045b6, y4;\n\t"
+        "madc.hi.cc.u32 y5, m, 0xb85045b6, y5;\n\t"
+        "madc.lo.cc.u32 y6, m, 0x30644e72, y6;\n\t"
+        "madc.hi.cc.u32 y7, m, 0x30644e72, y7;\n\t"
+        "mad.lo.cc.u32 x0, m, 0xd87cfd47, x0;\n\t"
+        "madc.hi.cc.u32 x1, m, 0xd87cfd47, x1;\n\t"
+        "madc.lo.cc.u32 x2, m, 0x6871ca8d, x2;\n\t"
+        "madc.hi.cc.u32 x3, m, 0x6871ca8d, x3;\n\t"
+        "madc.lo.cc.u32 x4, m, 0x8181585d, x4;\n\t"
+        "madc.hi.cc.u32 x5, m, 0x8181585d, x5;\n\t"
+        "madc.lo.cc.u32 x6, m, 0xe131a029, x6;\n\t"
+        "madc.hi.cc.u32 x7, m, 0xe131a029, x7;\n\t"
+        "addc.u32 y7, y7, 0;\n\t"
+        "add.cc.u32 y0, y0, x1;\n\t"
+        "addc.cc.u32 x0, x2, 0;\n\t"
+        "addc.cc.u32 x1, x3, 0;\n\t"
+        "addc.cc.u32 x2, x4, 0;\n\t"
+        "addc.cc.u32 x3, x5, 0;\n\t"
+        "addc.cc.u32 x4, x6, 0;\n\t"
+        "addc.cc.u32 x5, x7, 0;\n\t"
+        "madc.lo.cc.u32 x6, %15, %15, 0;\n\t"
+        "madc.hi.cc.u32 x7, %15, %15, 0;\n\t"
+        "mul.lo.u32 m, y0, 0xe4866389;\n\t"
+        "mad.lo.cc.u32 x0, m, 0x3c208c16, x0;\n\t"
+        "madc.hi.cc.u32 x1, m, 0x3c208c16, x1;\n\t"
+        "madc.lo.cc.u32 x2, m, 0x97816a91, x2;\n\t"
+        "madc.hi.cc.u32 x3, m, 0x97816a91, x3;\n\t"
+        "madc.lo.cc.u32 x4, m, 0xb85045b6, x4;\n\t"
+        "madc.hi.cc.u32 x5, m, 0xb85045b6, x5;\n\t"
+        "madc.lo.cc.u32 x6, m, 0x30644e72, x6;\n\t"
+        "madc.hi.cc.u32 x7, m, 0x30644e72, x7;\n\t"
+        "mad.lo.cc.u32 y0, m, 0xd87cfd47, y0;\n\t"
+        "madc.hi.cc.u32 y1, m, 0xd87cfd47, y1;\n\t"
+        "madc.lo.cc.u32 y2, m, 0x6871ca8d, y2;\n\t"
+        "madc.hi.cc.u32 y3, m, 0x6871ca8d, y3;\n\t"
+        "madc.lo.cc.u32 y4, m, 0x8181585d, y4;\n\t"
+        "madc.hi.cc.u32 y5, m, 0x8181585d, y5;\n\t"
+        "madc.lo.cc.u32 y6, m, 0xe131a029, y6;\n\t"
+        "madc.hi.cc.u32 y7, m, 0xe131a029, y7;\n\t"
+        "addc.u32 x7, x7, 0;\n\t"
+        "add.cc.u32 %0, x0, y1;\n\t"
+        "addc.cc.u32 %1, x1, y2;\n\t"
+        "addc.cc.u32 %2, x2, y3;\n\t"
+        "addc.cc.u32 %3, x3, y4;\n\t"
+        "addc.cc.u32 %4, x4, y5;\n\t"
+        "addc.cc.u32 %5, x5, y6;\n\t"
+        "addc.cc.u32 %6, x6, y7;\n\t"
+        "addc.u32 %7, x7, 0;\n\t"
+        "}\n\t"
+        : "=r"(r[0]), "=r"(r[1]), "=r"(r[2]), "=r"(r[3]), "=r"(r[4]), "=r"(r[5]), "=r"(r[6]), "=r"(r[7])
+        : "r"(a[0]), "r"(a[1]), "r"(a[2]), "r"(a[3]), "r"(a[4]), "r"(a[5]), "r"(a[6]), "r"(a[7]));
+}
+
+__device__ __forceinline__ void fq_add_lazy_ptx(uint32_t* r, const uint32_t* a, const uint32_t* b) {
+    asm(
+        "{\n\t"
+        ".reg .u32 brw, s0, s1, s2, s3, s4, s5, s6, s7, t0, t1, t2, t3, t4, t5, t6, t7;\n\t"
+        ".reg .pred p;\n\t"
+        "add.cc.u32 t0, %8, %16;\n\t"
+        "addc.cc.u32 t1, %9, %17;\n\t"
+        "addc.cc.u32 t2, %10, %18;\n\t"
+        "addc.cc.u32 t3, %11, %19;\n\t"
+        "addc.cc.u32 t4, %12, %20;\n\t"
+        "addc.cc.u32 t5, %13, %21;\n\t"
+        "addc.cc.u32 t6, %14, %22;\n\t"
+        "addc.u32 t7, %15, %23;\n\t"
+        "sub.cc.u32 s0, t0, 0xb0f9fa8e;\n\t"
+        "subc.cc.u32 s1, t1, 0x7841182d;\n\t"
+        "subc.cc.u32 s2, t2, 0xd0e3951a;\n\t"
+        "subc.cc.u32 s3, t3, 0x2f02d522;\n\t"
+        "subc.cc.u32 s4, t4, 0x0302b0bb;\n\t"
+        "subc.cc.u32 s5, t5, 0x70a08b6d;\n\t"
+        "subc.cc.u32 s6, t6, 0xc2634053;\n\t"
+        "subc.cc.u32 s7, t7, 0x60c89ce5;\n\t"
+        "subc.u32 brw, 0, 0;\n\t"
+        "setp.eq.u32 p, brw, 0;\n\t"
+        "selp.u32 %0, s0, t0, p;\n\t"
+        "selp.u32 %1, s1, t1, p;\n\t"
+        "selp.u32 %2, s2, t2, p;\n\t"
+        "selp.u32 %3, s3, t3, p;\n\t"
+        "selp.u32 %4, s4, t4, p;\n\t"
+        "selp.u32 %5, s5, t5, p;\n\t"
+        "selp.u32 %6, s6, t6, p;\n\t"
+        "selp.u32 %7, s7, t7, p;\n\t"
+        "}\n\t"
+        : "=r"(r[0]), "=r"(r[1]), "=r"(r[2]), "=r"(r[3]), "=r"(r[4]), "=r"(r[5]), "=r"(r[6]), "=r"(r[7])
+        : "r"(a[0]), "r"(a[1]), "r"(a[2]), "r"(a[3]), "r"(a[4]), "r"(a[5]), "r"(a[6]), "r"(a[7]), "r"(b[0]), "r"(b[1]), "r"(b[2]), "r"(b[3]), "r"(b[4]), "r"(b[5]), "r"(b[6]), "r"(b[7]));
+}
+
+__device__ __forceinline__ void fq_sub_lazy_ptx(uint32_t* r, const uint32_t* a, const uint32_t* b) {
+    asm(
+        "{\n\t"
+        ".reg .u32 brw, s0, s1, s2, s3, s4, s5, s6, s7, t0, t1, t2, t3, t4, t5, t6, t7;\n\t"
+        ".reg .pred p;\n\t"
+        "sub.cc.u32 t0, %8, %16;\n\t"
+        "subc.cc.u32 t1, %9, %17;\n\t"
+        "subc.cc.u32 t2, %10, %18;\n\t"
+        "subc.cc.u32 t3, %11, %19;\n\t"
+        "subc.cc.u32 t4, %12, %20;\n\t"
+        "subc.cc.u32 t5, %13, %21;\n\t"
+        "subc.cc.u32 t6, %14, %22;\n\t"
+        "subc.cc.u32 t7, %15, %23;\n\t"
+        "subc.u32 brw, 0, 0;\n\t"
+        "and.b32 s0, brw, 0xb0f9fa8e;\n\t"
+        "and.b32 s1, brw, 0x7841182d;\n\t"
+        "and.b32 s2, brw, 0xd0e3951a;\n\t"
+        "and.b32 s3, brw, 0x2f02d522;\n\t"
+        "and.b32 s4, brw, 0x0302b0bb;\n\t"
+        "and.b32 s5, brw, 0x70a08b6d;\n\t"
+        "and.b32 s6, brw, 0xc2634053;\n\t"
+        "and.b32 s7, brw, 0x60c89ce5;\n\t"
+        "add.cc.u32 %0, t0, s0;\n\t"
+        "addc.cc.u32 %1, t1, s1;\n\t"
+        "addc.cc.u32 %2, t2, s2;\n\t"
+        "addc.cc.u32 %3, t3, s3;\n\t"
+        "addc.cc.u32 %4, t4, s4;\n\t"
+        "addc.cc.u32 %5, t5, s5;\n\t"
+        "addc.cc.u32 %6, t6, s6;\n\t"
+        "addc.u32 %7, t7, s7;\n\t"
+        "}\n\t"
+        : "=r"(r[0]), "=r"(r[1]), "=r"(r[2]), "=r"(r[3]), "=r"(r[4]), "=r"(r[5]), "=r"(r[6]), "=r"(r[7])
+        : "r"(a[0]), "r"(a[1]), "r"(a[2]), "r"(a[3]), "r"(a[4]), "r"(a[5]), "r"(a[6]), "r"(a[7]), "r"(b[0]), "r"(b[1]), "r"(b[2]), "r"(b[3]), "r"(b[4]), "r"(b[5]), "r"(b[6]), "r"(b[7]));
+}
+
+__device__ __forceinline__ void fq_reduce_ptx(uint32_t* r, const uint32_t* a) {
+    asm(
+        "{\n\t"
+        ".reg .u32 brw, s0, s1, s2, s3, s4, s5, s6, s7;\n\t"
+        ".reg .pred p;\n\t"
+        "sub.cc.u32 s0, %8, 0xd87cfd47;\n\t"
+        "subc.cc.u32 s1, %9, 0x3c208c16;\n\t"
+        "subc.cc.u32 s2, %10, 0x6871ca8d;\n\t"
+        "subc.cc.u32 s3, %11, 0x97816a91;\n\t"
+        "subc.cc.u32 s4, %12, 0x8181585d;\n\t"
+        "subc.cc.u32 s5, %13, 0xb85045b6;\n\t"
+        "subc.cc.u32 s6, %14, 0xe131a029;\n\t"
+        "subc.cc.u32 s7, %15, 0x30644e72;\n\t"
+        "subc.u32 brw, 0, 0;\n\t"
+        "setp.eq.u32 p, brw, 0;\n\t"
+        "selp.u32 %0, s0, %8, p;\n\t"
+        "selp.u32 %1, s1, %9, p;\n\t"
+        "selp.u32 %2, s2, %10, p;\n\t"
+        "selp.u32 %3, s3, %11, p;\n\t"
+        "selp.u32 %4, s4, %12, p;\n\t"
+        "selp.u32 %5, s5, %13, p;\n\t"
+        "selp.u32 %6, s6, %14, p;\n\t"
+        "selp.u32 %7, s7, %15, p;\n\t"
+        "}\n\t"
+        : "=r"(r[0]), "=r"(r[1]), "=r"(r[2]), "=r"(r[3]), "=r"(r[4]), "=r"(r[5]), "=r"(r[6]), "=r"(r[7])
+        : "r"(a[0]), "r"(a[1]), "r"(a[2]), "r"(a[3]), "r"(a[4]), "r"(a[5]), "r"(a[6]), "r"(a[7]));
+}
+
 #endif
diff --git a/ezkl_b200/csrc/msm.cu b/ezkl_b200/csrc/msm.cu
--- a/ezkl_b200/csrc/msm.cu
+++ b/ezkl_b200/csrc/msm.cu
@@ -306,10 +306,10 @@
                 p = nx; e = e_next;
                 if (j + 1 < len) { e_next = ent[start + j + 1]; nx = load_base(table, e_next); }
                 if (e >> 31) p = g1_neg(p);
-                acc = g1_add_mixed(acc, p);
+                acc = g1_add_mixed_lazy(acc, p);
             }
         }
-        chunk_sums[(size_t)col * chunk_stride + ch] = acc;
+        chunk_sums[(size_t)col * chunk_stride + ch] = g1_reduce(acc);
     }
 }
 
@@ -371,9 +371,10 @@
         const uint32_t hi = min(lo + per_thread, nbuckets);
 #pragma unroll 1
         for (uint32_t b = hi; b-- > lo;) {
-            run = g1_add(run, bs[b]);
-            acc = g1_add(acc, run);
-        }
+            run = g1_add_lazy(run, bs[b]);
+            acc = g1_add_lazy(acc, run);
+        }
+        run = g1_reduce(run); acc = g1_reduce(acc);
         if (lo > 0) acc = g1_add(acc, g1_mul_small(run, lo));
     }
     acc = block_sum(acc, sh);
```

Result: faster. 0.08390 (median of 6 runs) (-1.6%).
